# zotya701/OpenCL_Path_tracer

Hardware: AMD Instinct MI355X
Metric: Msamples/s (whole node) at 1920x1080, 8-bounce Cornell box (higher is better)
Workload: dtype f32

## Files before the change

### opencl_path_tracer_amd/csrc/pt_context.hpp

```cpp
#pragma once

#include "pt_internal.hpp"

#include <algorithm>
#include <atomic>
#include <chrono>
#include <cmath>
#include <condition_variable>
#include <functional>
#include <mutex>
#include <cstdio>
#include <cstring>
#include <limits>
#include <memory>
#include <numeric>
#include <queue>
#include <thread>

using namespace ptamd;

namespace ptamd {
struct EventPair {
    hipEvent_t a = nullptr, b = nullptr;
};
}

struct pt_context {
    int device = -1;
    bool has_device = false;
    int32_t W = 0, H = 0;
    int32_t rank = 0, world = 1, rows_per_block = 8;
    int32_t local_rows = 0;
    int64_t npix = 0;
    int64_t slab_pix = 0;

    void* comm = nullptr;
    float4* d_gathered = nullptr;
    float4* d_frame = nullptr;
    uint64_t render_epoch = 0;
    uint64_t frame_epoch = ~0ull;

    std::vector<pt_triangle> tris;
    std::vector<int32_t> obj_begin;
    int32_t tri_shift = 0;
    std::vector<pt_material> mats;
    std::vector<int32_t> enc_rank;
    int32_t next_rank = 0;
    bool tris_uploaded = false, mats_uploaded = false;

    std::vector<Node64> nodes;
    std::vector<Node4q> nodes4;
    int wide_pending = 0;
    std::vector<TriPacket> packets;
    bool host_packets_stale = false;
    std::vector<TriMeta> meta;
    std::vector<int32_t> orig;
    int bvh_depth = 0;
    int interior_depth = 0;
    int n_flat = 0;
    int n_fbox = 0;
    uint8_t fbox_rep[32] = {};
    uint32_t fbox_mask[32] = {};

    float4* d_nodes = nullptr;
    float4* d_nodes4 = nullptr;
    uint32_t* d_stack_ovf = nullptr;
    size_t stack_ovf_lanes = 0;
    float4* d_tris = nullptr;
    TriMeta* d_meta = nullptr;
    pt_material* d_mats = nullptr;
    int32_t* d_rnds = nullptr;
    float4* d_colors = nullptr;
    pt_ray* d_rays = nullptr;
    float4* d_ldr = nullptr;
    unsigned long long* d_stats = nullptr;
    float4* d_wf_state = nullptr;
    int32_t* d_wf_queues = nullptr;
    std::vector<float> cost_boxes;
    uint32_t* d_wf_counters = nullptr;
    hipStream_t wf_stream[kWfMaxChains] = {};
    hipEvent_t wf_event[kWfMaxChains] = {};
    int poll_timeout_ms = 10000;
    int debug_stall_tile = -1;
    bool counters_suspect = false;
    bool launched_since_check = false;
    int wf_streams = -1;
    bool own_rnds = true, own_colors = true;
    hipStream_t stream = nullptr;

    int32_t current_sample = 0;

    int variant = 0;
    int lds_scene = 2;
    int treelet = 0;
    int treelet_nodes = 0;
    int timing = 0;
    int count_work = 0;
    int bvh_on_device = 0;
    double bvh_build_ms = 0.0;
    int cu_count = 256;
    int persistent = 1;
    uint32_t* d_tile_counter = nullptr;
    uint32_t* d_tile_done = nullptr;
    uint32_t* d_tile_cost = nullptr;
    float4* d_adapt_snap = nullptr;
    int32_t* d_adapt_spp = nullptr;
    float* d_adapt_err = nullptr;
    uint8_t* d_adapt_active = nullptr;
    int32_t* d_adapt_list = nullptr;
    int32_t* h_adapt_count = nullptr;
    bool adaptive_frame = false;
    float4* d_aov = nullptr;
    float4* d_dn = nullptr;
    float4* d_denoised = nullptr;
    bool aov_valid = false;
    int moments = 0;
    bool moments_valid = false;
    float* d_variance = nullptr;
    uint64_t frame_serial = 0;
    pt_camera frame_cam = {};
    bool frame_cam_same = false;
    uint64_t aov_serial = 0;
    pt_camera aov_cam = {};
    float4* d_temporal = nullptr;
    float* d_temporal_var = nullptr;
    int temporal_out = -1;
    bool temporal_history = false;
    pt_camera temporal_cam = {};
    uint64_t temporal_frame = ~0ull;
    uint64_t temporal_aov = ~0ull;
    std::vector<int32_t> nee_tri;
    std::vector<float> nee_cdf;
    std::vector<float> nee_pdf_area;
    bool nee_valid = false;
    int32_t* d_nee_tri = nullptr;
    float* d_nee_cdf = nullptr;
    float* d_nee_pdf_area = nullptr;
    bool nee_uploaded = false;
    int chunk_taper = -1;
    int chunk_spp = -1;
    int sah_visit_cost = 10;
    int flat_list = 16;
    int schedule = -1;
    int suspend_lanes = -1;
    int migrate_lanes = -1;
    int node_min_lanes = -1, leaf_min_lanes = -1;
    int lbvh_ploc = 16;
    int lbvh_cluster = 64;
    int build_threads = 0;
    int wide_nodes = 1;
    int wide_lds_entries = kWideLdsEntries;
    int lds_block = -1;
    int waves_per_simd = -1;
    int debug_repeat = 0;
    int cost_binning = 1;
    int bvh_policy = 0;
    int sah_grain = 256;
    int wide_on_device = 1;
    int bvh_device = -1;

    std::vector<EventPair> events;
    size_t events_used = 0;
    double kernel_ms_acc = 0.0;
    int64_t kernel_launches = 0;
    size_t last_lds_bytes = 0;
    int last_waves_per_simd = 4;

    std::string err;
    char info[256] = {0};
};

namespace ptamd {

constexpr size_t kLdsPerCu = 160 * 1024;
constexpr size_t kLdsSlack = 32 * 100 + 4096 + 1024 + 256;

int fail(pt_context* ctx, int code, const std::string& msg);
int host_threads(const pt_context* ctx);

#define PT_HIP(ctx, call)                                                                   \
    do {                                                                                    \
        hipError_t e_ = (call);                                                             \
        if (e_ != hipSuccess)                                                               \
            return fail(ctx, PT_EHIP, std::string(#call) + ": " + hipGetErrorString(e_));   \
    } while (0)

inline void note_frame(pt_context* ctx, int32_t first_sample, const pt_camera* cam) {
    ctx->moments_valid = (first_sample == 0 || ctx->moments_valid) && ctx->moments != 0;
    if (first_sample == 0) {
        ++ctx->frame_serial;
        ctx->frame_cam = *cam;
        ctx->frame_cam_same = true;
    } else if (std::memcmp(cam, &ctx->frame_cam, sizeof(pt_camera)) != 0) {
        ctx->frame_cam_same = false;
    }
}

#define PT_NEED_DEVICE(ctx)                                                                 \
    do {                                                                                    \
        if (!(ctx)) return PT_EINVAL;                                                       \
        if (!(ctx)->has_device)                                                             \
            return fail(ctx, PT_ENODEVICE, "context was created without a HIP device (host-only); no CPU render path exists"); \
    } while (0)
class HostPool {
public:
    static HostPool& get() { static HostPool p; return p; }
    template <class F>
    void run(size_t chunks, int threads, F fn) {
        if (chunks == 0) return;
        if (threads <= 1 || chunks == 1) { for (size_t k = 0; k < chunks; ++k) fn(k); return; }
        std::unique_lock<std::mutex> region(region_mu_, std::try_to_lock);
        if (!region.owns_lock()) {
            std::atomic<size_t> next(0);
            auto work = [&]() { for (size_t k = next.fetch_add(1); k < chunks; k = next.fetch_add(1)) fn(k); };
            std::vector<std::thread> th;
            for (int t = 1; t < std::min<int>(threads, (int)chunks); ++t) th.emplace_back(work);
            work();
            for (std::thread& t : th) t.join();
            return;
        }
        grow(std::min<int>(threads, (int)chunks) - 1);
        std::function<void(size_t)> f = fn;
        {
            std::lock_guard<std::mutex> lk(mu_);
            job_ = &f;
            chunks_ = chunks;
            next_.store(0);
            helpers_wanted_ = std::min<int>(threads, (int)chunks) - 1;
            helpers_in_ = 0;
            helpers_done_ = 0;
            ++generation_;
        }
        cv_.notify_all();
        for (size_t k = next_.fetch_add(1); k < chunks; k = next_.fetch_add(1)) fn(k);
        std::unique_lock<std::mutex> lk(mu_);
        job_ = nullptr;
        done_cv_.wait(lk, [&]() { return helpers_done_ == helpers_in_; });
    }
    ~HostPool() {
        {
            std::lock_guard<std::mutex> lk(mu_);
            stop_ = true;
        }
        cv_.notify_all();
        for (std::thread& t : workers_) t.join();
    }

private:
    void grow(int n) {
        while ((int)workers_.size() < n) workers_.emplace_back([this]() { loop(); });
    }
    void loop() {
        unsigned long long seen = 0;
        for (;;) {
            std::function<void(size_t)>* job = nullptr;
            size_t chunks = 0;
            {
                std::unique_lock<std::mutex> lk(mu_);
                cv_.wait(lk, [&]() { return stop_ || (generation_ != seen && job_ != nullptr && helpers_in_ < helpers_wanted_); });
                if (stop_) return;
                seen = generation_;
                job = job_;
                chunks = chunks_;
                ++helpers_in_;
            }
            for (size_t k = next_.fetch_add(1); k < chunks; k = next_.fetch_add(1)) (*job)(k);
            {
                std::lock_guard<std::mutex> lk(mu_);
                ++helpers_done_;
            }
            done_cv_.notify_all();
        }
    }
    std::mutex region_mu_, mu_;
    std::condition_variable cv_, done_cv_;
    std::vector<std::thread> workers_;
    std::function<void(size_t)>* job_ = nullptr;
    size_t chunks_ = 0;
    std::atomic<size_t> next_{0};
    int helpers_wanted_ = 0, helpers_in_ = 0, helpers_done_ = 0;
    unsigned long long generation_ = 0;
    bool stop_ = false;
};

template <class F>
void parallel_for(size_t n, size_t grain, int threads, F fn) {
    const size_t nt = std::min<size_t>((size_t)std::max(threads, 1), (n + grain - 1) / std::max<size_t>(grain, 1));
    if (nt <= 1) { fn((size_t)0, n); return; }
    const size_t per = (n + nt - 1) / nt;
    HostPool::get().run(nt, (int)nt, [&](size_t k) {
        const size_t b = k * per, e = std::min(n, b + per);
        if (b < e) fn(b, e);
    });
}
int deepest_interior_node(const std::vector<Node64>& nodes);
int reindex_treelet(std::vector<Node64>& nodes, int interior_depth, int want);

int32_t count_local_rows(int32_t H, int32_t rank, int32_t world, int32_t rb);
int wide_stack_entries(int pending);
int stack_entries_for(int interior_depth);
bool whole_tree_fits_lds(size_t n_nodes, size_t n_tris, int interior_depth, int n_flat);
int plan_node_placement(pt_context* ctx, const float4* d_bvh2 = nullptr, bool* wide_on_device = nullptr);
int alloc_stack_overflow(pt_context* ctx);
int seed_upload(pt_context* ctx, const int32_t* global_seeds);
void fill_params(const pt_context* ctx, const pt_camera* cam, RenderParams* p);
int check_ready(pt_context* ctx, const pt_camera* cam);
int time_begin(pt_context* ctx, EventPair** ep);
int time_end(pt_context* ctx, EventPair* ep);
int time_collect(pt_context* ctx);
int sync_and_check(pt_context* ctx);
inline int32_t local_tiles(const pt_context* c) { return ((c->W + 7) / 8) * ((c->local_rows + 7) / 8); }
template <class T>
int upload_vec(pt_context* ctx, T** dptr, const void* src, size_t bytes) {
    if (*dptr) { PT_HIP(ctx, hipFree(*dptr)); *dptr = nullptr; }
    PT_HIP(ctx, hipMalloc((void**)dptr, std::max<size_t>(bytes, 64)));
    if (bytes < 64) PT_HIP(ctx, hipMemset(*dptr, 0, 64));
    if (bytes) PT_HIP(ctx, hipMemcpy(*dptr, src, bytes, hipMemcpyHostToDevice));
    return PT_OK;
}


}
```

### opencl_path_tracer_amd/csrc/pt_host.cpp

```cpp
#include "pt_context.hpp"

namespace {
thread_local std::string g_create_error;
}

namespace ptamd {

int fail(pt_context* ctx, int code, const std::string& msg) {
    if (ctx) ctx->err = msg; else g_create_error = msg;
    return code;
}

int host_threads(const pt_context* ctx) {
    const unsigned hw = std::thread::hardware_concurrency();
    return ctx->build_threads > 0 ? ctx->build_threads : (int)std::min(16u, std::max(1u, hw));
}

int fail_ctx(pt_context* ctx, int code, const std::string& msg) { return fail(ctx, code, msg); }
int append_triangles(pt_context* ctx, int64_t n, pt_triangle** tail) {
    if (!ctx || n < 0 || !tail) return PT_EINVAL;
    if ((int64_t)ctx->tris.size() + n > kMaxTriangles) return fail(ctx, PT_EINVAL, "more than 2^26 triangles");
    const size_t old = ctx->tris.size();
    ctx->tris.resize(old + (size_t)n);
    ctx->tris_uploaded = false;
    *tail = ctx->tris.data() + old;
    return PT_OK;
}
hipError_t launch_deinterleave(const float4* gathered, float4* frame, int W, int H, int world, int rb, long long slab_stride, hipStream_t stream);
void gather_source_index(int W, int H, int world, int rb, long long slab_stride, int64_t* out);
int comm_available(std::string* err);
int comm_unique_id(void* id128, std::string* err);
int comm_init(const void* id128, int rank, int world, void** comm_out, std::string* err);
void comm_destroy(void* comm);
int comm_all_gather(void* comm, const void* send, void* recv, size_t floats_per_rank, hipStream_t stream, std::string* err);

}

extern "C" {

void pt_material_init(pt_material* m, const float kd[3], const float ks[3], const float emission[3],
                      const float N[3], const float K[3], float shininess, int32_t type) {
    std::memset(m, 0, sizeof *m);
    for (int i = 0; i < 3; ++i) { m->kd.s[i] = kd[i]; m->ks.s[i] = ks[i]; m->emission.s[i] = emission[i]; }
    m->shininess = shininess;
    m->type = type;
    m->n = (N[0] + N[1] + N[2]) / 3.0f;
    for (int i = 0; i < 3; ++i) {
        float a = (N[i] - 1) * (N[i] - 1);
        float b = (N[i] + 1) * (N[i] + 1);
        m->F0.s[i] = (K[i] * K[i] + a) / (K[i] * K[i] + b);
    }
}

void pt_triangle_init(pt_triangle* t, const float r1[3], const float r2[3], const float r3[3], uint16_t mati) {
    std::memset(t, 0, sizeof *t);
    float v1[3], v2[3], n[3];
    for (int i = 0; i < 3; ++i) {
        t->r1.s[i] = r1[i]; t->r2.s[i] = r2[i]; t->r3.s[i] = r3[i];
        v1[i] = r2[i] - r1[i];
        v2[i] = r3[i] - r1[i];
    }
    t->mati = mati;
    n[0] = v1[1] * v2[2] - v1[2] * v2[1];
    n[1] = v1[2] * v2[0] - v1[0] * v2[2];
    n[2] = v1[0] * v2[1] - v1[1] * v2[0];
    float length = (float)std::sqrt((double)(n[0] * n[0] + n[1] * n[1] + n[2] * n[2]));
    for (int i = 0; i < 3; ++i) t->N.s[i] = n[i] / length;
}

void pt_triangles_init(pt_triangle* out, const float* verts, const uint16_t* mati, int64_t n) {
    for (int64_t i = 0; i < n; ++i) pt_triangle_init(&out[i], verts + 9 * i, verts + 9 * i + 3, verts + 9 * i + 6, mati[i]);
}

static void rotate_x_ref(float v[3], float gamma) {
    gamma = gamma / 180.0f * 3.141593f;
    const double c = std::cos((double)gamma), s = std::sin((double)gamma);
    const float r1 = (float)((double)v[1] * c - (double)v[2] * s);
    const float r2 = (float)((double)v[1] * s + (double)v[2] * c);
    v[1] = r1;
    v[2] = r2;
}
static void rotate_y_ref(float v[3], float beta) {
    beta = beta / 180.0f * 3.141593f;
    const double c = std::cos((double)beta), s = std::sin((double)beta);
    const float r0 = (float)((double)v[0] * c + (double)v[2] * s);
    const float r2 = (float)(-(double)v[0] * s + (double)v[2] * c);
    v[0] = r0;
    v[2] = r2;
}

void pt_camera_init(pt_camera* c, float fov, float yaw, float pitch, const float shift[3], int32_t width, int32_t height) {
    std::memset(c, 0, sizeof *c);
    c->XM = (float)width;
    c->YM = (float)height;
    const float up_length = c->YM / 2.0f;
    const float right_length = c->XM / 2.0f;
    const float ahead_length = (float)((double)right_length / std::tan((double)(fov / 2.0f / 180.0f * 3.141593f)));
    float up[3] = {0.0f, 1.0f, 0.0f}, right[3] = {1.0f, 0.0f, 0.0f}, ahead[3] = {0.0f, 0.0f, 1.0f};
    rotate_x_ref(up, pitch); rotate_y_ref(up, yaw);
    rotate_x_ref(right, pitch); rotate_y_ref(right, yaw);
    rotate_x_ref(ahead, pitch); rotate_y_ref(ahead, yaw);
    for (int i = 0; i < 3; ++i) { up[i] *= up_length; right[i] *= right_length; ahead[i] *= ahead_length; }
    c->eye.s[0] = 500.0f + shift[0];
    c->eye.s[1] = 500.0f + shift[1];
    c->eye.s[2] = -1299.037842f + shift[2];
    for (int i = 0; i < 3; ++i) { c->up.s[i] = up[i]; c->right.s[i] = right[i]; c->lookat.s[i] = c->eye.s[i] + ahead[i]; }
}

void pt_camera_move(float shift[3], float yaw, float pitch, float forward, float rightward, float upward) {
    float up[3] = {0.0f, 1.0f, 0.0f}, right[3] = {1.0f, 0.0f, 0.0f}, ahead[3] = {0.0f, 0.0f, 1.0f};
    rotate_x_ref(up, pitch); rotate_y_ref(up, yaw);
    rotate_x_ref(right, pitch); rotate_y_ref(right, yaw);
    rotate_x_ref(ahead, pitch); rotate_y_ref(ahead, yaw);
    for (int i = 0; i < 3; ++i) {
        const float a = ahead[i] * forward, r = right[i] * rightward, u = up[i] * upward;
        shift[i] = ((shift[i] + a) + r) + u;
    }
}

int pt_create_tiled(int device, int32_t width, int32_t height, int32_t rank, int32_t world, int32_t rows_per_block, pt_context** out) {
    if (!out) return fail(nullptr, PT_EINVAL, "out is NULL");
    *out = nullptr;
    if (width <= 0 || height <= 0 || (int64_t)width * height > (int64_t)1 << 30) return fail(nullptr, PT_EINVAL, "bad frame size");
    if (width > 65535 || height > 65535) return fail(nullptr, PT_EINVAL, "bad frame size: at most 65,535 pixels per side (the kernels pack a pixel's coordinates into 2 x 16 bits)");
    if (world < 1 || rank < 0 || rank >= world || rows_per_block < 1) return fail(nullptr, PT_EINVAL, "bad rank/world/rows_per_block");
    pt_context* ctx = new pt_context();
    ctx->W = width;
    ctx->H = height;
    ctx->rank = rank;
    ctx->world = world;
    ctx->rows_per_block = rows_per_block;
    ctx->local_rows = count_local_rows(height, rank, world, rows_per_block);
    ctx->npix = (int64_t)ctx->local_rows * width;
    for (int32_t r = 0; r < world; ++r) ctx->slab_pix = std::max(ctx->slab_pix, (int64_t)count_local_rows(height, r, world, rows_per_block) * width);
    ctx->device = device;
    if (device < 0) {
        std::snprintf(ctx->info, sizeof ctx->info, "host-only context (no device)");
        *out = ctx;
        return PT_OK;
    }
    int count = 0;
    hipError_t e = hipGetDeviceCount(&count);
    if (e != hipSuccess || count <= 0 || device >= count) {
        delete ctx;
        return fail(nullptr, PT_ENODEVICE, std::string("no usable HIP device: ") + (e != hipSuccess ? hipGetErrorString(e) : "device index out of range"));
    }
    auto bail = [&](const char* what, hipError_t err) {
        std::string msg = std::string(what) + ": " + hipGetErrorString(err);
        pt_destroy(ctx);
        return fail(nullptr, PT_EHIP, msg);
    };
    if ((e = hipSetDevice(device)) != hipSuccess) return bail("hipSetDevice", e);
    hipDeviceProp_t prop;
    if ((e = hipGetDeviceProperties(&prop, device)) != hipSuccess) return bail("hipGetDeviceProperties", e);
    ctx->cu_count = prop.multiProcessorCount;
    std::snprintf(ctx->info, sizeof ctx->info, "%s (%s), %d CUs, %.1f GiB, wave %d", prop.name, prop.gcnArchName,
                  prop.multiProcessorCount, (double)prop.totalGlobalMem / (1024.0 * 1024.0 * 1024.0), prop.warpSize);
    if (std::strncmp(prop.gcnArchName, "gfx950", 6) != 0) {
        std::string msg = std::string("device is ") + prop.gcnArchName + ", this library carries gfx950 code only";
        pt_destroy(ctx);
        return fail(nullptr, PT_ENODEVICE, msg);
    }
    ctx->has_device = true;
    const size_t np = (size_t)std::max<int64_t>(ctx->npix, 1);
    const size_t nslab = (size_t)std::max<int64_t>(ctx->slab_pix, 1);
    if ((e = hipMalloc((void**)&ctx->d_rays, sizeof(pt_ray) * np)) != hipSuccess) return bail("hipMalloc(rays)", e);
    if ((e = hipMalloc((void**)&ctx->d_rnds, sizeof(int32_t) * np)) != hipSuccess) return bail("hipMalloc(rnds)", e);
    if ((e = hipMalloc((void**)&ctx->d_colors, sizeof(float4) * nslab)) != hipSuccess) return bail("hipMalloc(colors)", e);
    if ((e = hipMalloc((void**)&ctx->d_stats, sizeof(unsigned long long) * kStatCols * kStatRows)) != hipSuccess) return bail("hipMalloc(stats)", e);
    if ((e = hipMalloc((void**)&ctx->d_tile_counter, sizeof(uint32_t) * kTileCounterWords)) != hipSuccess) return bail("hipMalloc(tile counter)", e);
    if ((e = hipMemset(ctx->d_tile_counter, 0, sizeof(uint32_t) * kTileCounterWords)) != hipSuccess) return bail("hipMemset", e);
    if ((e = hipMemset(ctx->d_rays, 0, sizeof(pt_ray) * np)) != hipSuccess) return bail("hipMemset", e);
    if ((e = hipMemset(ctx->d_colors, 0, sizeof(float4) * nslab)) != hipSuccess) return bail("hipMemset", e);
    if ((e = hipMemset(ctx->d_stats, 0, sizeof(unsigned long long) * kStatCols * kStatRows)) != hipSuccess) return bail("hipMemset", e);
    int rc = pt_seed_default(ctx);
    if (rc != PT_OK) {
        std::string msg = ctx->err;
        pt_destroy(ctx);
        return fail(nullptr, rc, msg);
    }
    *out = ctx;
    return PT_OK;
}

int pt_create(int device, int32_t width, int32_t height, pt_context** out) {
    return pt_create_tiled(device, width, height, 0, 1, 8, out);
}

void pt_destroy(pt_context* ctx) {
    if (!ctx) return;
    if (ctx->has_device) {
        (void)hipSetDevice(ctx->device);
        (void)hipDeviceSynchronize();
        for (auto& e : ctx->events) { if (e.a) (void)hipEventDestroy(e.a); if (e.b) (void)hipEventDestroy(e.b); }
        if (ctx->d_nodes) (void)hipFree(ctx->d_nodes);
        if (ctx->d_nodes4) (void)hipFree(ctx->d_nodes4);
        if (ctx->d_stack_ovf) (void)hipFree(ctx->d_stack_ovf);
        if (ctx->d_tris) (void)hipFree(ctx->d_tris);
        if (ctx->d_meta) (void)hipFree(ctx->d_meta);
        if (ctx->d_mats) (void)hipFree(ctx->d_mats);
        if (ctx->d_rays) (void)hipFree(ctx->d_rays);
        if (ctx->d_ldr) (void)hipFree(ctx->d_ldr);
        if (ctx->d_stats) (void)hipFree(ctx->d_stats);
        if (ctx->d_tile_counter) (void)hipFree(ctx->d_tile_counter);
        if (ctx->d_tile_done) (void)hipFree(ctx->d_tile_done);
        if (ctx->d_tile_cost) (void)hipFree(ctx->d_tile_cost);
        if (ctx->d_adapt_snap) (void)hipFree(ctx->d_adapt_snap);
        if (ctx->d_adapt_spp) (void)hipFree(ctx->d_adapt_spp);
        if (ctx->d_adapt_err) (void)hipFree(ctx->d_adapt_err);
        if (ctx->d_adapt_active) (void)hipFree(ctx->d_adapt_active);
        if (ctx->d_adapt_list) (void)hipFree(ctx->d_adapt_list);
        if (ctx->h_adapt_count) (void)hipHostFree(ctx->h_adapt_count);
        if (ctx->d_aov) (void)hipFree(ctx->d_aov);
        if (ctx->d_dn) (void)hipFree(ctx->d_dn);
        if (ctx->d_variance) (void)hipFree(ctx->d_variance);
        if (ctx->d_temporal) (void)hipFree(ctx->d_temporal);
        if (ctx->d_temporal_var) (void)hipFree(ctx->d_temporal_var);
        if (ctx->d_nee_tri) (void)hipFree(ctx->d_nee_tri);
        if (ctx->d_nee_cdf) (void)hipFree(ctx->d_nee_cdf);
        if (ctx->d_nee_pdf_area) (void)hipFree(ctx->d_nee_pdf_area);
        if (ctx->d_wf_state) (void)hipFree(ctx->d_wf_state);
        if (ctx->d_wf_queues) (void)hipFree(ctx->d_wf_queues);
        if (ctx->d_wf_counters) (void)hipFree(ctx->d_wf_counters);
        for (int c = 0; c < kWfMaxChains; ++c) {
            if (ctx->wf_stream[c]) (void)hipStreamDestroy(ctx->wf_stream[c]);
            if (ctx->wf_event[c]) (void)hipEventDestroy(ctx->wf_event[c]);
        }
        if (ctx->comm) comm_destroy(ctx->comm);
        if (ctx->d_gathered) (void)hipFree(ctx->d_gathered);
        if (ctx->d_frame) (void)hipFree(ctx->d_frame);
        if (ctx->own_rnds && ctx->d_rnds) (void)hipFree(ctx->d_rnds);
        if (ctx->own_colors && ctx->d_colors) (void)hipFree(ctx->d_colors);
    }
    delete ctx;
}

const char* pt_last_error(const pt_context* ctx) { return ctx ? ctx->err.c_str() : g_create_error.c_str(); }

int pt_device_info(const pt_context* ctx, char* buf, int32_t buflen) {
    if (!ctx || !buf || buflen <= 0) return PT_EINVAL;
    std::snprintf(buf, (size_t)buflen, "%s", ctx->info);
    return PT_OK;
}

int pt_add_material(pt_context* ctx, const pt_material* m) {
    if (!ctx || !m) return PT_EINVAL;
    if (ctx->mats.size() >= 65536) return fail(ctx, PT_EINVAL, "more than 65536 materials (mati is a ushort, prog.cl:20)");
    ctx->mats.push_back(*m);
    ctx->mats_uploaded = false;
    return (int)ctx->mats.size() - 1;
}

int pt_add_triangle(pt_context* ctx, const pt_triangle* t) { return pt_add_triangles(ctx, t, 1); }

int pt_add_triangles(pt_context* ctx, const pt_triangle* t, int64_t n) {
    if (!ctx || (!t && n) || n < 0) return PT_EINVAL;
    if ((int64_t)ctx->tris.size() + n > kMaxTriangles)
        return fail(ctx, PT_EINVAL, "more than 2^26 triangles");
    ctx->tris.insert(ctx->tris.end(), t, t + n);
    ctx->tris_uploaded = false;
    return PT_OK;
}

int pt_upload_materials(pt_context* ctx) {
    if (!ctx) return PT_EINVAL;
    ctx->aov_valid = false;
    ctx->nee_valid = false;
    for (const pt_triangle& t : ctx->tris)
        if (t.mati >= ctx->mats.size()) return fail(ctx, PT_EINVAL, "a triangle references a material index that was never added");
    if (ctx->has_device) {
        PT_HIP(ctx, hipSetDevice(ctx->device));
        std::vector<pt_material> dm(ctx->mats);
        for (pt_material& m : dm)
            m._pad = (m.ks.s[0] == 0.0f && m.ks.s[1] == 0.0f && m.ks.s[2] == 0.0f && std::isfinite(m.shininess) && m.shininess >= 0.0f) ? 1 : 0;
        int rc = upload_vec(ctx, &ctx->d_mats, dm.data(), sizeof(pt_material) * dm.size());
        if (rc != PT_OK) return rc;
    }
    ctx->mats_uploaded = true;
    return PT_OK;
}

int pt_seed_default(pt_context* ctx) {
    PT_NEED_DEVICE(ctx);
    const size_t n = (size_t)ctx->W * (size_t)ctx->H;
    std::vector<int32_t> g(n);
    uint64_t x = 1;
    for (size_t i = 0; i < n; ++i) {
        x = (x * 16807ull) % 2147483647ull;
        g[i] = (int32_t)x;
    }
    return seed_upload(ctx, g.data());
}

int pt_upload_seeds(pt_context* ctx, const int32_t* seeds, int64_t n) {
    PT_NEED_DEVICE(ctx);
    if (!seeds || n != (int64_t)ctx->W * ctx->H) return fail(ctx, PT_EINVAL, "seeds must hold width*height ints (global frame)");
    return seed_upload(ctx, seeds);
}

int pt_local_pixel_count(const pt_context* ctx, int64_t* out) {
    if (!ctx || !out) return PT_EINVAL;
    *out = ctx->npix;
    return PT_OK;
}

int pt_slab_pixel_count(const pt_context* ctx, int64_t* out) {
    if (!ctx || !out) return PT_EINVAL;
    *out = ctx->slab_pix;
    return PT_OK;
}

int pt_frame_size(const pt_context* ctx, int32_t* width, int32_t* height, int64_t* npix) {
    if (!ctx) return PT_EINVAL;
    if (width) *width = ctx->W;
    if (height) *height = ctx->H;
    if (npix) *npix = (int64_t)ctx->W * ctx->H;
    return PT_OK;
}

int pt_comm_available(void) {
    std::string err;
    const int rc = comm_available(&err);
    return rc == PT_OK ? rc : fail(nullptr, rc, err);
}

int pt_comm_unique_id(void* id128) {
    if (!id128) return PT_EINVAL;
    std::string err;
    const int rc = comm_unique_id(id128, &err);
    return rc == PT_OK ? rc : fail(nullptr, rc, err);
}

int pt_comm_init(pt_context* ctx, const void* id128) {
    PT_NEED_DEVICE(ctx);
    if (!id128) return fail(ctx, PT_EINVAL, "id is NULL");
    if (ctx->comm) return fail(ctx, PT_EINVAL, "the context already has a communicator");
    PT_HIP(ctx, hipSetDevice(ctx->device));
    std::string err;
    const int rc = comm_init(id128, ctx->rank, ctx->world, &ctx->comm, &err);
    return rc == PT_OK ? rc : fail(ctx, rc, err);
}

int pt_gather_frame(pt_context* ctx) {
    PT_NEED_DEVICE(ctx);
    if (!ctx->comm) {
        if (ctx->world == 1) return PT_OK;
        return fail(ctx, PT_EINVAL, "pt_comm_init has not been called on this tiled context");
    }
    PT_HIP(ctx, hipSetDevice(ctx->device));
    const size_t slab = (size_t)ctx->slab_pix;
    if (!ctx->d_gathered) PT_HIP(ctx, hipMalloc((void**)&ctx->d_gathered, sizeof(float4) * slab * (size_t)ctx->world));
    if (!ctx->d_frame) PT_HIP(ctx, hipMalloc((void**)&ctx->d_frame, sizeof(float4) * (size_t)ctx->W * (size_t)ctx->H));
    std::string err;
    const int rc = comm_all_gather(ctx->comm, ctx->d_colors, ctx->d_gathered, slab * 4, ctx->stream, &err);
    if (rc != PT_OK) return fail(ctx, rc, err);
    PT_HIP(ctx, launch_deinterleave(ctx->d_gathered, ctx->d_frame, ctx->W, ctx->H, ctx->world, ctx->rows_per_block, (long long)slab, ctx->stream));
    ctx->frame_epoch = ctx->render_epoch;
    return PT_OK;
}

static const float4* current_frame(const pt_context* ctx) {
    if (ctx->d_frame && ctx->frame_epoch == ctx->render_epoch) return ctx->d_frame;
    return ctx->world == 1 ? ctx->d_colors : nullptr;
}

void* pt_device_frame(pt_context* ctx) { return !ctx ? nullptr : (void*)current_frame(ctx); }

int pt_read_frame(pt_context* ctx, float* out, int64_t npix) {
    PT_NEED_DEVICE(ctx);
    if (!out || npix != (int64_t)ctx->W * ctx->H) return fail(ctx, PT_EINVAL, "npix must equal width * height of the global frame");
    const float4* src = current_frame(ctx);
    if (!src) return fail(ctx, PT_EINVAL, ctx->d_frame ? "the gathered frame is older than colors: call pt_gather_frame again" : "pt_gather_frame has not been called");
    PT_HIP(ctx, hipSetDevice(ctx->device));
    PT_HIP(ctx, hipStreamSynchronize(ctx->stream));
    PT_HIP(ctx, hipMemcpy(out, src, sizeof(float4) * (size_t)npix, hipMemcpyDeviceToHost));
    return PT_OK;
}

int pt_debug_gather_index(int32_t width, int32_t height, int32_t world, int32_t rows_per_block, int64_t slab_stride, int64_t* out) {
    if (width <= 0 || height <= 0 || world < 1 || rows_per_block < 1 || !out) return PT_EINVAL;
    gather_source_index(width, height, world, rows_per_block, (long long)slab_stride, out);
    return PT_OK;
}

int pt_local_pixel_ids(const pt_context* ctx, int32_t* out, int64_t n) {
    if (!ctx || !out || n != ctx->npix) return PT_EINVAL;
    for (int32_t lr = 0; lr < ctx->local_rows; ++lr) {
        const int32_t gr = global_row(*ctx, lr);
        for (int32_t x = 0; x < ctx->W; ++x) out[(size_t)lr * ctx->W + x] = gr * ctx->W + x;
    }
    return PT_OK;
}

static int read_back(pt_context* ctx, void* dst, const void* src, size_t bytes) {
    const int rc = sync_and_check(ctx);
    if (rc != PT_OK) return rc;
    if (bytes) PT_HIP(ctx, hipMemcpy(dst, src, bytes, hipMemcpyDeviceToHost));
    return PT_OK;
}

int pt_read_colors(pt_context* ctx, float* out, int64_t npix) {
    PT_NEED_DEVICE(ctx);
    if (!out || npix != ctx->npix) return fail(ctx, PT_EINVAL, "npix must equal the local pixel count");
    return read_back(ctx, out, ctx->d_colors, sizeof(float4) * (size_t)npix);
}
int pt_read_rnds(pt_context* ctx, int32_t* out, int64_t npix) {
    PT_NEED_DEVICE(ctx);
    if (!out || npix != ctx->npix) return fail(ctx, PT_EINVAL, "npix must equal the local pixel count");
    return read_back(ctx, out, ctx->d_rnds, sizeof(int32_t) * (size_t)npix);
}
int pt_read_sample_counts(pt_context* ctx, int32_t* out, int64_t npix) {
    PT_NEED_DEVICE(ctx);
    if (!out || npix != ctx->npix) return fail(ctx, PT_EINVAL, "npix must equal the local pixel count");
    if (!ctx->adaptive_frame) {
        std::fill(out, out + npix, ctx->current_sample);
        return PT_OK;
    }
    std::vector<int32_t> spp((size_t)local_tiles(ctx));
    const int rc = read_back(ctx, spp.data(), ctx->d_adapt_spp, sizeof(int32_t) * spp.size());
    if (rc != PT_OK) return rc;
    const int32_t tiles_x = (ctx->W + 7) / 8;
    for (int64_t i = 0; i < npix; ++i) {
        const int32_t y = (int32_t)(i / ctx->W), x = (int32_t)(i % ctx->W);
        out[i] = spp[(size_t)(y / 8) * tiles_x + x / 8];
    }
    return PT_OK;
}
int pt_read_tile_state(pt_context* ctx, int32_t* spp, float* err, int64_t n_tiles) {
    PT_NEED_DEVICE(ctx);
    if (n_tiles != local_tiles(ctx)) return fail(ctx, PT_EINVAL, "pt_read_tile_state: n_tiles must be the number of 8x8 tiles of the local frame");
    if (!ctx->adaptive_frame) {
        if (spp) std::fill(spp, spp + n_tiles, ctx->current_sample);
        if (err) std::fill(err, err + n_tiles, std::numeric_limits<float>::infinity());
        return PT_OK;
    }
    int rc = PT_OK;
    if (spp && (rc = read_back(ctx, spp, ctx->d_adapt_spp, sizeof(int32_t) * (size_t)n_tiles)) != PT_OK) return rc;
    if (err && (rc = read_back(ctx, err, ctx->d_adapt_err, sizeof(float) * (size_t)n_tiles)) != PT_OK) return rc;
    return PT_OK;
}
int pt_render_aovs(pt_context* ctx, const pt_camera* cam, int32_t subpixels, int32_t specular_depth) {
    if (!ctx) return PT_EINVAL;
    if (subpixels < 1 || subpixels > 8) return fail(ctx, PT_EINVAL, "pt_render_aovs: subpixels must be 1..8");
    if (specular_depth < 0 || specular_depth > 16) return fail(ctx, PT_EINVAL, "pt_render_aovs: specular_depth must be 0..16");
    PT_NEED_DEVICE(ctx);
    int rc = check_ready(ctx, cam);
    if (rc != PT_OK) return rc;
    PT_HIP(ctx, hipSetDevice(ctx->device));
    if (!ctx->d_aov) PT_HIP(ctx, hipMalloc((void**)&ctx->d_aov, 2 * sizeof(float4) * (size_t)std::max<int64_t>(ctx->npix, 1)));
    RenderParams p;
    fill_params(ctx, cam, &p);
    PT_HIP(ctx, launch_aovs(p, subpixels, specular_depth, ctx->npix, ctx->d_aov, ctx->d_aov + ctx->npix, ctx->cu_count, ctx->stream));
    if (!ctx->aov_valid) ctx->temporal_history = false;
    ctx->aov_valid = true;
    ctx->aov_cam = *cam;
    ++ctx->aov_serial;
    return PT_OK;
}
int pt_read_aovs(pt_context* ctx, float* albedo_rgbm, float* normal_depth, int64_t npix) {
    PT_NEED_DEVICE(ctx);
    if (npix != ctx->npix) return fail(ctx, PT_EINVAL, "npix must equal the local pixel count");
    if (!ctx->d_aov) return fail(ctx, PT_EINVAL, "pt_read_aovs: pt_render_aovs has not run");
    int rc = PT_OK;
    if (albedo_rgbm && (rc = read_back(ctx, albedo_rgbm, ctx->d_aov, sizeof(float4) * (size_t)npix)) != PT_OK) return rc;
    if (normal_depth && (rc = read_back(ctx, normal_depth, ctx->d_aov + npix, sizeof(float4) * (size_t)npix)) != PT_OK) return rc;
    return PT_OK;
}
void pt_denoise_defaults(pt_denoise_params* p) {
    if (!p) return;
    p->iterations = 3;
    p->sigma_color = 0.125f;
    p->sigma_normal = 8.0f;
    p->sigma_depth = 0.05f;
    p->demodulate = 1;
}
int pt_denoise(pt_context* ctx, const pt_denoise_params* dp) {
    if (!ctx) return PT_EINVAL;
    if (!dp) return fail(ctx, PT_EINVAL, "pt_denoise: params is NULL");
    if (dp->iterations < 1 || dp->iterations > 10) return fail(ctx, PT_EINVAL, "pt_denoise: iterations must be 1..10");
    if (!(dp->sigma_color >= 0.0f) || !(dp->sigma_normal >= 0.0f) || !(dp->sigma_depth >= 0.0f))
        return fail(ctx, PT_EINVAL, "pt_denoise: sigmas must be >= 0 (and not NaN)");
    if (ctx->world != 1) return fail(ctx, PT_EINVAL, "pt_denoise: contexts of one rank (world == 1) only");
    if (!ctx->aov_valid)
        return fail(ctx, PT_EINVAL, "pt_denoise: no guides (pt_render_aovs has not run since the scene was last uploaded)");
    PT_NEED_DEVICE(ctx);
    PT_HIP(ctx, hipSetDevice(ctx->device));
    const size_t npix = (size_t)ctx->npix;
    if (!ctx->d_dn) PT_HIP(ctx, hipMalloc((void**)&ctx->d_dn, 2 * sizeof(float4) * std::max<size_t>(npix, 1)));
    for (int i = 0; i < dp->iterations; ++i) {
        AtrousStep s;
        s.step = 1 << i;
        s.demodulate = dp->demodulate ? 1 : 0;
        s.color_on = std::isfinite(dp->sigma_color) ? 1 : 0;
        s.normal_on = std::isfinite(dp->sigma_normal) && dp->sigma_normal > 0.0f ? 1 : 0;
        s.depth_on = std::isfinite(dp->sigma_depth) ? 1 : 0;
        s.color_scale = (float)(1 << (2 * i));
        s.sigma_color2 = dp->sigma_color * dp->sigma_color;
        s.sigma_normal = dp->sigma_normal;
        s.sigma_depth = dp->sigma_depth;
        const float4* in = i == 0 ? ctx->d_colors : ctx->d_dn + ((i - 1) & 1) * npix;
        float4* out = ctx->d_dn + (i & 1) * npix;
        PT_HIP(ctx, launch_atrous(in, out, ctx->d_aov, ctx->d_aov + npix, ctx->W, ctx->local_rows, s, i == 0, i == dp->iterations - 1, ctx->stream));
    }
    ctx->d_denoised = ctx->d_dn + ((dp->iterations - 1) & 1) * npix;
    return PT_OK;
}
int pt_read_denoised(pt_context* ctx, float* out, int64_t npix) {
    PT_NEED_DEVICE(ctx);
    if (!out || npix != ctx->npix) return fail(ctx, PT_EINVAL, "npix must equal the local pixel count");
    if (!ctx->d_denoised) return fail(ctx, PT_EINVAL, "pt_read_denoised: pt_denoise has not run");
    return read_back(ctx, out, ctx->d_denoised, sizeof(float4) * (size_t)npix);
}
void* pt_device_denoised(pt_context* ctx) { return ctx ? (void*)ctx->d_denoised : nullptr; }

static int compute_variance(pt_context* ctx, const char* who) {
    if (!ctx->moments_valid) return fail(ctx, PT_EINVAL, std::string(who) + ": the frame was not rendered with option moments = 1 from its first sample");
    if (ctx->current_sample <= 0) return fail(ctx, PT_EINVAL, std::string(who) + ": the frame has no samples");
    PT_HIP(ctx, hipSetDevice(ctx->device));
    if (!ctx->d_variance) PT_HIP(ctx, hipMalloc((void**)&ctx->d_variance, sizeof(float) * (size_t)std::max<int64_t>(ctx->npix, 1)));
    PT_HIP(ctx, launch_variance(ctx->d_colors, ctx->adaptive_frame ? ctx->d_adapt_spp : nullptr, ctx->current_sample, ctx->W, ctx->npix,
                                ctx->d_variance, ctx->stream));
    return PT_OK;
}
int pt_read_variance(pt_context* ctx, float* out, int64_t npix) {
    PT_NEED_DEVICE(ctx);
    if (!out || npix != ctx->npix) return fail(ctx, PT_EINVAL, "npix must equal the local pixel count");
    const int rc = compute_variance(ctx, "pt_read_variance");
    if (rc != PT_OK) return rc;
    return read_back(ctx, out, ctx->d_variance, sizeof(float) * (size_t)npix);
}
void* pt_device_variance(pt_context* ctx) {
    if (!ctx || !ctx->has_device) {
        if (ctx) (void)fail(ctx, PT_ENODEVICE, "context was created without a HIP device (host-only); no CPU render path exists");
        return nullptr;
    }
    return compute_variance(ctx, "pt_device_variance") == PT_OK ? (void*)ctx->d_variance : nullptr;
}

void pt_denoise_variance_defaults(pt_denoise_variance_params* p) {
    if (!p) return;
    p->iterations = 2;
    p->sigma_luminance = 4.0f;
    p->sigma_normal = 8.0f;
    p->sigma_depth = 0.05f;
    p->demodulate = 0;
}
static std::string variance_params_error(const pt_denoise_variance_params* dp) {
    if (!dp) return "params is NULL";
    if (dp->iterations < 1 || dp->iterations > 10) return "iterations must be 1..10";
    if (!(dp->sigma_luminance >= 0.0f) || !(dp->sigma_normal >= 0.0f) || !(dp->sigma_depth >= 0.0f)) return "sigmas must be >= 0 (and not NaN)";
    return "";
}
static int atrous_var_iterations(pt_context* ctx, const pt_denoise_variance_params* dp, const float4* in0, const float* var) {
    const size_t npix = (size_t)ctx->npix;
    if (!ctx->d_dn) PT_HIP(ctx, hipMalloc((void**)&ctx->d_dn, 2 * sizeof(float4) * std::max<size_t>(npix, 1)));
    for (int i = 0; i < dp->iterations; ++i) {
        AtrousVarStep s;
        s.step = 1 << i;
        s.demodulate = dp->demodulate ? 1 : 0;
        s.lum_on = std::isfinite(dp->sigma_luminance) ? 1 : 0;
        s.normal_on = std::isfinite(dp->sigma_normal) && dp->sigma_normal > 0.0f ? 1 : 0;
        s.depth_on = std::isfinite(dp->sigma_depth) ? 1 : 0;
        s.sigma_luminance = dp->sigma_luminance;
        s.sigma_normal = dp->sigma_normal;
        s.sigma_depth = dp->sigma_depth;
        const float4* in = i == 0 ? in0 : ctx->d_dn + ((i - 1) & 1) * npix;
        float4* out = ctx->d_dn + (i & 1) * npix;
        PT_HIP(ctx, launch_atrous_var(in, var, out, ctx->d_aov, ctx->d_aov + npix, ctx->W, ctx->local_rows, s, i == 0,
                                      i == dp->iterations - 1, ctx->stream));
    }
    ctx->d_denoised = ctx->d_dn + ((dp->iterations - 1) & 1) * npix;
    return PT_OK;
}
int pt_denoise_variance(pt_context* ctx, const pt_denoise_variance_params* dp) {
    if (!ctx) return PT_EINVAL;
    const std::string why = variance_params_error(dp);
    if (!why.empty()) return fail(ctx, PT_EINVAL, "pt_denoise_variance: " + why);
    if (ctx->world != 1) return fail(ctx, PT_EINVAL, "pt_denoise_variance: contexts of one rank (world == 1) only");
    if (!ctx->aov_valid)
        return fail(ctx, PT_EINVAL, "pt_denoise_variance: no guides (pt_render_aovs has not run since the scene was last uploaded)");
    PT_NEED_DEVICE(ctx);
    const int rc = compute_variance(ctx, "pt_denoise_variance");
    if (rc != PT_OK) return rc;
    return atrous_var_iterations(ctx, dp, ctx->d_colors, ctx->d_variance);
}

void pt_temporal_defaults(pt_temporal_params* p) {
    if (!p) return;
    p->max_history = 64;
    p->normal_cos = 0.9f;
    p->depth_tolerance = 0.02f;
}
static float4* temporal_colour(const pt_context* ctx, int s) { return ctx->d_temporal + (size_t)s * (size_t)std::max<int64_t>(ctx->npix, 1); }
static float4* temporal_guides(const pt_context* ctx, int s) { return ctx->d_temporal + (size_t)(2 + s) * (size_t)std::max<int64_t>(ctx->npix, 1); }
static float2* temporal_nm(const pt_context* ctx, int s) {
    const size_t np = (size_t)std::max<int64_t>(ctx->npix, 1);
    return reinterpret_cast<float2*>(ctx->d_temporal + 4 * np) + (size_t)s * np;
}
int pt_temporal_accumulate(pt_context* ctx, const pt_temporal_params* tp) {
    if (!ctx) return PT_EINVAL;
    if (!tp) return fail(ctx, PT_EINVAL, "pt_temporal_accumulate: params is NULL");
    if (tp->max_history < 0) return fail(ctx, PT_EINVAL, "pt_temporal_accumulate: max_history must be >= 0");
    if (!(tp->normal_cos >= -1.0f && tp->normal_cos <= 1.0f)) return fail(ctx, PT_EINVAL, "pt_temporal_accumulate: normal_cos must be in [-1, 1]");
    if (!(tp->depth_tolerance >= 0.0f)) return fail(ctx, PT_EINVAL, "pt_temporal_accumulate: depth_tolerance must be >= 0 (and not NaN)");
    if (ctx->world != 1) return fail(ctx, PT_EINVAL, "pt_temporal_accumulate: contexts of one rank (world == 1) only");
    PT_NEED_DEVICE(ctx);
    if (!ctx->aov_valid)
        return fail(ctx, PT_EINVAL, "pt_temporal_accumulate: no guides (pt_render_aovs has not run since the scene was last uploaded)");
    if (!ctx->moments_valid)
        return fail(ctx, PT_EINVAL, "pt_temporal_accumulate: the frame was not rendered with option moments = 1 from its first sample");
    if (ctx->current_sample <= 0) return fail(ctx, PT_EINVAL, "pt_temporal_accumulate: the frame has no samples");
    if (!ctx->frame_cam_same) return fail(ctx, PT_EINVAL, "pt_temporal_accumulate: the launches of the frame used different cameras");
    if (std::memcmp(&ctx->aov_cam, &ctx->frame_cam, sizeof(pt_camera)) != 0)
        return fail(ctx, PT_EINVAL, "pt_temporal_accumulate: the guides were rendered with a different camera from the frame");
    if (ctx->temporal_frame == ctx->frame_serial) return fail(ctx, PT_EINVAL, "pt_temporal_accumulate: this frame was already accumulated");
    PT_HIP(ctx, hipSetDevice(ctx->device));
    const size_t np = (size_t)std::max<int64_t>(ctx->npix, 1);
    if (!ctx->d_temporal) {
        PT_HIP(ctx, hipMalloc((void**)&ctx->d_temporal, (4 * sizeof(float4) + 2 * sizeof(float2)) * np));
        PT_HIP(ctx, hipMalloc((void**)&ctx->d_temporal_var, sizeof(float) * np));
    }
    const int out = ctx->temporal_out == 0 ? 1 : 0, prev = 1 - out;
    TemporalArgs a;
    a.cur = ctx->frame_cam;
    a.prev = ctx->temporal_cam;
    a.colors = ctx->d_colors;
    a.tile_spp = ctx->adaptive_frame ? ctx->d_adapt_spp : nullptr;
    a.n_all = ctx->current_sample;
    a.albedo = ctx->d_aov;
    a.nd = ctx->d_aov + ctx->npix;
    a.prev_c = temporal_colour(ctx, prev);
    a.prev_g = temporal_guides(ctx, prev);
    a.prev_nm = temporal_nm(ctx, prev);
    a.out_c = temporal_colour(ctx, out);
    a.out_g = temporal_guides(ctx, out);
    a.out_nm = temporal_nm(ctx, out);
    a.out_v = ctx->d_temporal_var;
    a.W = ctx->W;
    a.H = ctx->local_rows;
    a.has_prev = ctx->temporal_history ? 1 : 0;
    a.max_history = (float)tp->max_history;
    a.normal_cos = tp->normal_cos;
    a.depth_tolerance = tp->depth_tolerance;
    PT_HIP(ctx, launch_temporal(a, ctx->stream));
    ctx->temporal_out = out;
    ctx->temporal_history = true;
    ctx->temporal_cam = ctx->frame_cam;
    ctx->temporal_frame = ctx->frame_serial;
    ctx->temporal_aov = ctx->aov_serial;
    return PT_OK;
}
int pt_read_temporal(pt_context* ctx, float* rgbv, float* n, int64_t npix) {
    PT_NEED_DEVICE(ctx);
    if (npix != ctx->npix) return fail(ctx, PT_EINVAL, "npix must equal the local pixel count");
    if (ctx->temporal_out < 0) return fail(ctx, PT_EINVAL, "pt_read_temporal: pt_temporal_accumulate has not run");
    int rc = PT_OK;
    if (rgbv) {
        std::vector<float> v((size_t)npix);
        if ((rc = read_back(ctx, rgbv, temporal_colour(ctx, ctx->temporal_out), sizeof(float4) * (size_t)npix)) != PT_OK) return rc;
        if ((rc = read_back(ctx, v.data(), ctx->d_temporal_var, sizeof(float) * (size_t)npix)) != PT_OK) return rc;
        for (int64_t i = 0; i < npix; ++i) rgbv[4 * i + 3] = v[(size_t)i];
    }
    if (n) {
        std::vector<float2> nm((size_t)npix);
        if ((rc = read_back(ctx, nm.data(), temporal_nm(ctx, ctx->temporal_out), sizeof(float2) * (size_t)npix)) != PT_OK) return rc;
        for (int64_t i = 0; i < npix; ++i) n[i] = nm[(size_t)i].x;
    }
    return PT_OK;
}
void* pt_device_temporal(pt_context* ctx) { return ctx && ctx->temporal_out >= 0 ? (void*)temporal_colour(ctx, ctx->temporal_out) : nullptr; }
int pt_denoise_temporal(pt_context* ctx, const pt_denoise_variance_params* dp) {
    if (!ctx) return PT_EINVAL;
    const std::string why = variance_params_error(dp);
    if (!why.empty()) return fail(ctx, PT_EINVAL, "pt_denoise_temporal: " + why);
    if (ctx->world != 1) return fail(ctx, PT_EINVAL, "pt_denoise_temporal: contexts of one rank (world == 1) only");
    PT_NEED_DEVICE(ctx);
    if (!ctx->aov_valid || ctx->temporal_out < 0 || ctx->temporal_aov != ctx->aov_serial)
        return fail(ctx, PT_EINVAL, "pt_denoise_temporal: pt_temporal_accumulate has not run on the current guides");
    PT_HIP(ctx, hipSetDevice(ctx->device));
    return atrous_var_iterations(ctx, dp, temporal_colour(ctx, ctx->temporal_out), ctx->d_temporal_var);
}
int pt_debug_reproject(const pt_camera* cur, const pt_camera* prev, int32_t x, int32_t y, float depth, float out[3]) {
    if (!cur || !prev || !out) return fail(nullptr, PT_EINVAL, "pt_debug_reproject: NULL argument");
    if (!(cur->XM >= 1.0f && cur->XM <= 65535.0f && cur->YM >= 1.0f && cur->YM <= 65535.0f) || x < 0 || y < 0 || x >= (int32_t)cur->XM || y >= (int32_t)cur->YM)
        return fail(nullptr, PT_EINVAL, "pt_debug_reproject: (x, y) must lie in cur's frame");
    if (!reproject(*cur, *prev, y * (int32_t)cur->XM + x, depth, out))
        return fail(nullptr, PT_EINVAL, "pt_debug_reproject: the point is not in front of prev (a <= 0)");
    return PT_OK;
}

uint32_t pt_nee_rand(uint32_t state, int32_t segment, int32_t dim) { return nee_rand(state, segment, dim); }
static int nee_table(pt_context* ctx) {
    if (!ctx->tris_uploaded) return fail(ctx, PT_EINVAL, "pt_upload_triangles has not been called");
    if (!ctx->mats_uploaded) return fail(ctx, PT_EINVAL, "pt_upload_materials has not been called");
    if (ctx->nee_valid) return PT_OK;
    const size_t m = ctx->orig.size();
    std::vector<double> wgt, area;
    ctx->nee_tri.clear();
    ctx->nee_cdf.clear();
    ctx->nee_pdf_area.assign(std::max<size_t>(m, 1), 0.0f);
    for (size_t k = 0; k < m; ++k) {
        const pt_triangle& t = ctx->tris[(size_t)ctx->orig[k]];
        const pt_material& mt = ctx->mats[t.mati];
        if (mt.type != 3) continue;
        const double esum = ((double)mt.emission.s[0] + (double)mt.emission.s[1]) + (double)mt.emission.s[2];
        const double e1[3] = {(double)t.r2.s[0] - t.r1.s[0], (double)t.r2.s[1] - t.r1.s[1], (double)t.r2.s[2] - t.r1.s[2]};
        const double e2[3] = {(double)t.r3.s[0] - t.r1.s[0], (double)t.r3.s[1] - t.r1.s[1], (double)t.r3.s[2] - t.r1.s[2]};
        const double cx = e1[1] * e2[2] - e1[2] * e2[1], cy = e1[2] * e2[0] - e1[0] * e2[2], cz = e1[0] * e2[1] - e1[1] * e2[0];
        const double a = 0.5 * std::sqrt(cx * cx + cy * cy + cz * cz);
        if (!(esum > 0.0) || !(a > 0.0) || !std::isfinite(a * esum)) continue;
        ctx->nee_tri.push_back((int32_t)k);
        wgt.push_back(a * esum);
        area.push_back(a);
    }
    double total = 0.0;
    for (double w : wgt) total += w;
    double run = 0.0;
    for (size_t j = 0; j < wgt.size(); ++j) {
        run += wgt[j];
        ctx->nee_cdf.push_back(j + 1 == wgt.size() ? 1.0f : (float)(run / total));
    }
    double below = 0.0;
    for (size_t j = 0; j < wgt.size(); ++j) {
        const double upto = std::ceil((double)ctx->nee_cdf[j] * 16777216.0);
        ctx->nee_pdf_area[(size_t)ctx->nee_tri[j]] = (float)((upto - below) / 16777216.0 / area[j]);
        below = upto;
    }
    ctx->nee_valid = true;
    ctx->nee_uploaded = false;
    return PT_OK;
}
int pt_debug_light_table(pt_context* ctx, int32_t* orig_tri, float* cdf, int64_t cap, int64_t* n) {
    if (!ctx) return PT_EINVAL;
    if (!n || cap < 0) return fail(ctx, PT_EINVAL, "pt_debug_light_table: n is NULL or cap < 0");
    int rc = nee_table(ctx);
    if (rc != PT_OK) return rc;
    *n = (int64_t)ctx->nee_tri.size();
    const size_t k = (size_t)std::min<int64_t>(cap, *n);
    for (size_t j = 0; j < k; ++j) {
        if (orig_tri) orig_tri[j] = ctx->orig[(size_t)ctx->nee_tri[j]];
        if (cdf) cdf[j] = ctx->nee_cdf[j];
    }
    return PT_OK;
}
int pt_render_nee(pt_context* ctx, const pt_camera* cam, int32_t iterations, int32_t nsamples, int32_t strategy) {
    if (!ctx) return PT_EINVAL;
    if (iterations < 0 || nsamples < 0) return fail(ctx, PT_EINVAL, "pt_render_nee: iterations/nsamples must be >= 0");
    if (strategy < PT_NEE_BSDF || strategy > PT_NEE_MIS) return fail(ctx, PT_EINVAL, "pt_render_nee: strategy must be PT_NEE_BSDF, PT_NEE_LIGHT or PT_NEE_MIS");
    PT_NEED_DEVICE(ctx);
    int rc = check_ready(ctx, cam);
    if (rc != PT_OK) return rc;
    if (ctx->adaptive_frame) return fail(ctx, PT_EINVAL, "pt_render_nee: an adaptive frame is held: pt_set_current_sample(ctx, 0) starts a new frame");
    if ((int64_t)ctx->current_sample + nsamples > INT32_MAX) return fail(ctx, PT_EINVAL, "pt_render_nee: current_sample + nsamples overflows");
    if (nsamples == 0) return PT_OK;
    if ((rc = nee_table(ctx)) != PT_OK) return rc;
    PT_HIP(ctx, hipSetDevice(ctx->device));
    if (!ctx->nee_uploaded) {
        if (ctx->d_nee_tri) PT_HIP(ctx, hipFree(ctx->d_nee_tri));
        if (ctx->d_nee_cdf) PT_HIP(ctx, hipFree(ctx->d_nee_cdf));
        if (ctx->d_nee_pdf_area) PT_HIP(ctx, hipFree(ctx->d_nee_pdf_area));
        ctx->d_nee_tri = nullptr;
        ctx->d_nee_cdf = nullptr;
        ctx->d_nee_pdf_area = nullptr;
        const size_t nl = std::max<size_t>(ctx->nee_tri.size(), 1);
        PT_HIP(ctx, hipMalloc((void**)&ctx->d_nee_tri, sizeof(int32_t) * nl));
        PT_HIP(ctx, hipMalloc((void**)&ctx->d_nee_cdf, sizeof(float) * nl));
        PT_HIP(ctx, hipMalloc((void**)&ctx->d_nee_pdf_area, sizeof(float) * ctx->nee_pdf_area.size()));
        if (!ctx->nee_tri.empty()) {
            PT_HIP(ctx, hipMemcpy(ctx->d_nee_tri, ctx->nee_tri.data(), sizeof(int32_t) * ctx->nee_tri.size(), hipMemcpyHostToDevice));
            PT_HIP(ctx, hipMemcpy(ctx->d_nee_cdf, ctx->nee_cdf.data(), sizeof(float) * ctx->nee_cdf.size(), hipMemcpyHostToDevice));
        }
        PT_HIP(ctx, hipMemcpy(ctx->d_nee_pdf_area, ctx->nee_pdf_area.data(), sizeof(float) * ctx->nee_pdf_area.size(), hipMemcpyHostToDevice));
        ctx->nee_uploaded = true;
    }
    RenderParams p;
    fill_params(ctx, cam, &p);
    p.iterations = iterations;
    p.first_sample = ctx->current_sample;
    p.nsamples = nsamples;
    NeeTable lt;
    lt.tri = ctx->d_nee_tri;
    lt.cdf = ctx->d_nee_cdf;
    lt.pdf_area = ctx->d_nee_pdf_area;
    lt.n = (int32_t)ctx->nee_tri.size();
    lt.strategy = strategy;
    ctx->render_epoch++;
    note_frame(ctx, p.first_sample, cam);
    EventPair* ep;
    if ((rc = time_begin(ctx, &ep)) != PT_OK) return rc;
    PT_HIP(ctx, launch_nee(p, lt, ctx->npix, ctx->cu_count, ctx->stream));
    if ((rc = time_end(ctx, ep)) != PT_OK) return rc;
    ctx->current_sample += nsamples;
    return PT_OK;
}

int pt_read_rays(pt_context* ctx, pt_ray* out, int64_t npix) {
    PT_NEED_DEVICE(ctx);
    if (!out || npix != ctx->npix) return fail(ctx, PT_EINVAL, "npix must equal the local pixel count");
    return read_back(ctx, out, ctx->d_rays, sizeof(pt_ray) * (size_t)npix);
}

int pt_resolve_ldr(pt_context* ctx, int32_t which, float* out, int64_t npix) {
    PT_NEED_DEVICE(ctx);
    if (!out || npix != ctx->npix) return fail(ctx, PT_EINVAL, "npix must equal the local pixel count");
    if (which != 0 && which != 1) return fail(ctx, PT_EINVAL, "which must be 0 (Reinhard) or 1 (filt_im)");
    if (which == 1 && ctx->world != 1) return fail(ctx, PT_EINVAL, "filt_im needs the whole frame on one context (3x3 stencil)");
    PT_HIP(ctx, hipSetDevice(ctx->device));
    if (!ctx->d_ldr) PT_HIP(ctx, hipMalloc((void**)&ctx->d_ldr, sizeof(float4) * (size_t)std::max<int64_t>(npix, 1)));
    if (which == 0) {
        PT_HIP(ctx, launch_resolve_reinhard(ctx->d_colors, ctx->d_ldr, npix, ctx->stream));
    } else {
        PT_HIP(ctx, hipMemsetAsync(ctx->d_ldr, 0, sizeof(float4) * (size_t)npix, ctx->stream));
        PT_HIP(ctx, launch_filt_im(ctx->d_colors, ctx->d_ldr, ctx->W, ctx->H, ctx->stream));
    }
    return read_back(ctx, out, ctx->d_ldr, sizeof(float4) * (size_t)npix);
}

int pt_bind_framebuffer(pt_context* ctx, void* d_colors, void* d_rnds) {
    PT_NEED_DEVICE(ctx);
    PT_HIP(ctx, hipSetDevice(ctx->device));
    PT_HIP(ctx, hipStreamSynchronize(ctx->stream));
    if (d_colors && d_colors != ctx->d_colors) {
        PT_HIP(ctx, hipMemcpy(d_colors, ctx->d_colors, sizeof(float4) * (size_t)ctx->npix, hipMemcpyDeviceToDevice));
        if (ctx->own_colors) PT_HIP(ctx, hipFree(ctx->d_colors));
        ctx->d_colors = (float4*)d_colors;
        ctx->own_colors = false;
    }
    if (d_rnds && d_rnds != ctx->d_rnds) {
        PT_HIP(ctx, hipMemcpy(d_rnds, ctx->d_rnds, sizeof(int32_t) * (size_t)ctx->npix, hipMemcpyDeviceToDevice));
        if (ctx->own_rnds) PT_HIP(ctx, hipFree(ctx->d_rnds));
        ctx->d_rnds = (int32_t*)d_rnds;
        ctx->own_rnds = false;
    }
    return PT_OK;
}

void* pt_device_colors(pt_context* ctx) { return ctx ? (void*)ctx->d_colors : nullptr; }
void* pt_device_rnds(pt_context* ctx) { return ctx ? (void*)ctx->d_rnds : nullptr; }

int pt_set_stream(pt_context* ctx, void* s) {
    PT_NEED_DEVICE(ctx);
    PT_HIP(ctx, hipSetDevice(ctx->device));
    PT_HIP(ctx, hipStreamSynchronize(ctx->stream));
    ctx->stream = (hipStream_t)s;
    return PT_OK;
}

int pt_set_option(pt_context* ctx, const char* key, int64_t value) {
    if (!ctx || !key) return PT_EINVAL;
    std::string k(key);
    if (k == "variant") {
        if (value != 0 && value != 1) return fail(ctx, PT_EINVAL, "variant must be 0 (megakernel) or 1 (wavefront)");
        ctx->variant = (int)value;
    } else if (k == "lds_scene") {
        if (value != 0 && value != 2) return fail(ctx, PT_EINVAL, "lds_scene: 0 every node through L1/L2, 2 stage the tree (or its top) in LDS");
        ctx->lds_scene = (int)value;
    } else if (k == "treelet") {
        if (value < -1 || value > 2048) return fail(ctx, PT_EINVAL, "treelet: 0 off, -1 as many nodes as fit, 2..2048 nodes");
        ctx->treelet = (int)value;
        ctx->tris_uploaded = false;
    } else if (k == "lbvh_cluster") {
        if (value < 0 || value > (1 << 20)) return fail(ctx, PT_EINVAL, "lbvh_cluster: 0 off, 1..2^20 triangles");
        ctx->lbvh_cluster = (int)value;
        ctx->tris_uploaded = false;
    } else if (k == "build_threads") {
        if (value < 0 || value > 256) return fail(ctx, PT_EINVAL, "build_threads: 0 automatic, 1..256");
        ctx->build_threads = (int)value;
    } else if (k == "wide_nodes") {
        if (value < 0 || value > 2) return fail(ctx, PT_EINVAL, "wide_nodes: 0 never, 1 for trees that do not fit LDS, 2 always");
        ctx->wide_nodes = (int)value;
        ctx->tris_uploaded = false;
    } else if (k == "wide_lds_entries") {
        if (value < 4 || value > kWideLdsEntries || (value & 1)) return fail(ctx, PT_EINVAL, "wide_lds_entries: even, 4..20");
        ctx->wide_lds_entries = (int)value;
        ctx->tris_uploaded = false;
    } else if (k == "moments") {
        if (value != 0 && value != 1) return fail(ctx, PT_EINVAL, "moments must be 0 (off) or 1 (second moment of the luminance in colors[].w)");
        ctx->moments = (int)value;
    } else if (k == "timing") {
        ctx->timing = value ? 1 : 0;
    } else if (k == "count_work") {
        ctx->count_work = value ? 1 : 0;
    } else if (k == "chunk_taper") {
        if (value < -1 || value > 1 << 15) return fail(ctx, PT_EINVAL, "chunk_taper: -1 default, 0 off, else the shortest pass");
        ctx->chunk_taper = (int)value;
    } else if (k == "chunk_spp") {
        if (value < -1 || value > 1 << 20) return fail(ctx, PT_EINVAL, "chunk_spp out of range");
        ctx->chunk_spp = (int)value;
    } else if (k == "persistent") {
        ctx->persistent = value ? 1 : 0;
    } else if (k == "sah_visit_cost") {
        if (value < 0 || value > 1000) return fail(ctx, PT_EINVAL, "sah_visit_cost: tenths of a triangle test, 0..1000");
        ctx->sah_visit_cost = (int)value;
    } else if (k == "schedule") {
        if (value < -1 || value > 2) return fail(ctx, PT_EINVAL, "schedule: -1 automatic, 0 lockstep per sample, 1 restart + tail suspension, 2 the same with lanes moving on to the wave's next work item");
        ctx->schedule = (int)value;
    } else if (k == "flat_list") {
        if (value < 0 || value > 32) return fail(ctx, PT_EINVAL, "flat_list: 0..32 big triangles tested before the tree (a 32-bit candidate mask per lane)");
        ctx->flat_list = (int)value;
        ctx->tris_uploaded = false;
    } else if (k == "poll_timeout_ms") {
        if (value < 1 || value > 40000) return fail(ctx, PT_EINVAL, "poll_timeout_ms: 1..40000");
        ctx->poll_timeout_ms = (int)value;
    } else if (k == "debug_stall_tile") {
        if (value < -1 || value > 0x7fffffff) return fail(ctx, PT_EINVAL, "debug_stall_tile: -1 none, or a tile index");
        ctx->debug_stall_tile = (int)value;
    } else if (k == "wf_streams") {
        if (value < -1 || value == 0 || value > kWfMaxChains) return fail(ctx, PT_EINVAL, "wf_streams: -1 default, 1..8");
        ctx->wf_streams = (int)value;
    } else if (k == "node_min_lanes" || k == "leaf_min_lanes") {
        if (value < -1 || value > 63) return fail(ctx, PT_EINVAL, k + ": -1 default, 0..63");
        (k == "node_min_lanes" ? ctx->node_min_lanes : ctx->leaf_min_lanes) = (int)value;
    } else if (k == "migrate_lanes") {
        if (value != -1 && (value < 1 || value > 64)) return fail(ctx, PT_EINVAL, "migrate_lanes: -1 default, 1..64");
        ctx->migrate_lanes = (int)value;
    } else if (k == "suspend_lanes") {
        if (value < -1 || value > 63) return fail(ctx, PT_EINVAL, "suspend_lanes: -1 default, 0..63");
        ctx->suspend_lanes = (int)value;
    } else if (k == "waves_per_simd") {
        if (value != -1 && (value < 4 || value > 8)) return fail(ctx, PT_EINVAL, "waves_per_simd: -1 automatic (at most 7), 4..8 (kernels that read nodes from global memory)");
        ctx->waves_per_simd = (int)value;
    } else if (k == "bvh_device") {
        if (value < -1 || value > 1) return fail(ctx, PT_EINVAL, "bvh_device: -1 (by scene size), 0 (host) or 1 (device)");
        ctx->bvh_device = (int)value;
    } else if (k == "wide_on_device") {
        if (value != 0 && value != 1) return fail(ctx, PT_EINVAL, "wide_on_device: 0 or 1");
        ctx->wide_on_device = (int)value;
    } else if (k == "sah_grain") {
        if (value < 8 || value > (1 << 16)) return fail(ctx, PT_EINVAL, "sah_grain: 8..65536 triangles");
        ctx->sah_grain = (int)value;
    } else if (k == "lbvh_ploc") {
        if (value != 0 && value != 8 && value != 16 && value != 32) return fail(ctx, PT_EINVAL, "lbvh_ploc: 0 (radix tree), 8, 16 or 32 (PLOC search radius)");
        ctx->lbvh_ploc = (int)value;
    } else if (k == "lds_block") {
        if (value != -1 && value != kLdsBlockBase && value != kLdsBlockWide) return fail(ctx, PT_EINVAL, "lds_block: -1 automatic, 512 or 768");
        ctx->lds_block = (int)value;
    } else if (k == "debug_repeat") {
        if (value < 0 || value > 1000) return fail(ctx, PT_EINVAL, "debug_repeat: 0..1000 extra timed launches");
        ctx->debug_repeat = (int)value;
    } else if (k == "cost_binning") {
        ctx->cost_binning = value ? 1 : 0;
    } else if (k == "bvh_policy") {
        if (value < 0 || value > 5) return fail(ctx, PT_EINVAL, "bvh_policy must be 0..5 (4 = device LBVH, 5 = the SAH tree built on the device)");
        ctx->bvh_policy = (int)value;
        ctx->tris_uploaded = false;
    } else if (k == "reset_stats") {
        if (ctx->has_device) {
            PT_HIP(ctx, hipSetDevice(ctx->device));
            PT_HIP(ctx, hipStreamSynchronize(ctx->stream));
            PT_HIP(ctx, hipMemset(ctx->d_stats, 0, sizeof(unsigned long long) * kStatCols * kStatRows));
        }
        int rc = time_collect(ctx);
        if (rc != PT_OK) return rc;
        ctx->kernel_ms_acc = 0.0;
        ctx->kernel_launches = 0;
    } else {
        return fail(ctx, PT_EINVAL, "unknown option: " + k);
    }
    return PT_OK;
}

int pt_get_stat(pt_context* ctx, const char* key, double* out) {
    if (!ctx || !key || !out) return PT_EINVAL;
    std::string k(key);
    if (k == "bvh_nodes") { *out = (double)ctx->nodes.size(); return PT_OK; }
    if (k == "bvh_depth") { *out = (double)ctx->bvh_depth; return PT_OK; }
    if (k == "stack_entries") { *out = (double)stack_entries_for(ctx->interior_depth); return PT_OK; }
    if (k == "bvh_build_ms") { *out = ctx->bvh_build_ms; return PT_OK; }
    if (k == "bvh_on_device") { *out = (double)ctx->bvh_on_device; return PT_OK; }
    if (k == "triangles") { *out = (double)ctx->orig.size(); return PT_OK; }
    if (k == "lds_bytes") { *out = (double)ctx->last_lds_bytes; return PT_OK; }
    if (k == "waves_per_simd") { *out = (double)ctx->last_waves_per_simd; return PT_OK; }
    if (k == "treelet_nodes") { *out = (double)ctx->treelet_nodes; return PT_OK; }
    if (k == "wide_nodes") { *out = (double)ctx->nodes4.size(); return PT_OK; }
    if (k == "wide_pending") { *out = (double)ctx->wide_pending; return PT_OK; }
    if (k == "flat_triangles") { *out = (double)ctx->n_flat; return PT_OK; }
    if (k == "flat_boxes") { *out = (double)ctx->n_fbox; return PT_OK; }
    if (k == "node_mode") {
        pt_camera cam;
        std::memset(&cam, 0, sizeof cam);
        RenderParams p;
        fill_params(ctx, &cam, &p);
        *out = (double)p.node_mode;
        return PT_OK;
    }
    if (k == "kernel_launches") { *out = (double)ctx->kernel_launches; return PT_OK; }
    PT_NEED_DEVICE(ctx);
    PT_HIP(ctx, hipSetDevice(ctx->device));
    if (k == "kernel_ms") {
        int rc = time_collect(ctx);
        if (rc != PT_OK) return rc;
        *out = ctx->kernel_ms_acc;
        return PT_OK;
    }
    if (k == "segments" || k == "samples" || k == "node_visits" || k == "tri_tests" || k == "wave_node_steps" || k == "wave_tri_steps" || k == "tile_lane_steps" ||
        k == "wave_shade_steps" || k == "wave_trips" || k == "wave_rounds" || k.rfind("low_", 0) == 0) {
        std::vector<unsigned long long> rows((size_t)kStatCols * kStatRows);
        unsigned long long h[kStatCols] = {};
        PT_HIP(ctx, hipStreamSynchronize(ctx->stream));
        PT_HIP(ctx, hipMemcpy(rows.data(), ctx->d_stats, sizeof(unsigned long long) * rows.size(), hipMemcpyDeviceToHost));
        for (int r = 0; r < kStatRows; ++r)
            for (int c = 0; c < kStatCols; ++c) h[c] += rows[(size_t)r * kStatCols + c];
        if (k.rfind("low_", 0) == 0 || k == "exact_steps") {
            const int slot = k == "low_node" ? 10 : k == "low_tri" ? 11 : k == "low_exact" ? 12 : k == "low_shade" ? 13 : k == "low_exact_all" ? 15 : -1;
            if (slot < 0) return fail(ctx, PT_EINVAL, "unknown stat " + k);
            *out = (double)h[slot];
            return PT_OK;
        }
        *out = (double)h[k == "segments" ? 0 : k == "samples" ? 1 : k == "node_visits" ? 2 : k == "tri_tests" ? 3 : k == "wave_node_steps" ? 4 : k == "wave_tri_steps" ? 5 : k == "tile_lane_steps" ? 6 : k == "wave_shade_steps" ? 7 : k == "wave_trips" ? 8 : 9];
        return PT_OK;
    }
    return fail(ctx, PT_EINVAL, "unknown stat: " + k);
}

int pt_debug_bvh_sizes(const pt_context* ctx, int64_t* nnodes, int64_t* ntris) {
    if (!ctx) return PT_EINVAL;
    if (nnodes) *nnodes = (int64_t)ctx->nodes.size();
    if (ntris) *ntris = (int64_t)ctx->orig.size();
    return PT_OK;
}

int pt_debug_wide_nodes(const pt_context* ctx, void* out, int64_t capacity, int64_t* count) {
    if (!ctx || !count || capacity < 0) return PT_EINVAL;
    *count = (int64_t)ctx->nodes4.size();
    if (out) std::memcpy(out, ctx->nodes4.data(), sizeof(Node4q) * (size_t)std::min<int64_t>(capacity, *count));
    return PT_OK;
}

int pt_debug_bvh_copy(const pt_context* cctx, float* nodes, float* tris, int32_t* meta, int32_t* orig) {
    if (!cctx || !cctx->tris_uploaded) return PT_EINVAL;
    pt_context* ctx = const_cast<pt_context*>(cctx);
    if (ctx->host_packets_stale && (tris || meta)) {
        const size_t m = ctx->orig.size();
        ctx->packets.resize(m);
        ctx->meta.resize(m);
        PT_HIP(ctx, hipSetDevice(ctx->device));
        PT_HIP(ctx, hipMemcpy(ctx->packets.data(), ctx->d_tris, sizeof(TriPacket) * m, hipMemcpyDeviceToHost));
        PT_HIP(ctx, hipMemcpy(ctx->meta.data(), ctx->d_meta, sizeof(TriMeta) * m, hipMemcpyDeviceToHost));
        ctx->host_packets_stale = false;
    }
    if (nodes) std::memcpy(nodes, ctx->nodes.data(), sizeof(Node64) * ctx->nodes.size());
    if (tris) std::memcpy(tris, ctx->packets.data(), sizeof(TriPacket) * ctx->orig.size());
    if (meta) std::memcpy(meta, ctx->meta.data(), sizeof(TriMeta) * ctx->orig.size());
    if (orig) std::memcpy(orig, ctx->orig.data(), sizeof(int32_t) * ctx->orig.size());
    return PT_OK;
}

namespace {
struct DeviceBuf {
    void* p = nullptr;
    ~DeviceBuf() { if (p) (void)hipFree(p); }
    hipError_t alloc(size_t bytes) { return hipMalloc(&p, std::max<size_t>(bytes, 16)); }
};
struct EventOwner {
    hipEvent_t e = nullptr;
    ~EventOwner() { if (e) (void)hipEventDestroy(e); }
};
}

int pt_debug_math(pt_context* ctx, int32_t fn, int64_t first, int64_t n, int64_t out[3], uint32_t* bad, int64_t bad_cap) {
    PT_NEED_DEVICE(ctx);
    if (fn < PT_MATH_SQRT || fn > PT_MATH_DIV_NORMAL || first < 0 || n < 0 || !out || bad_cap < 0 || (bad_cap > 0 && !bad))
        return fail(ctx, PT_EINVAL, "pt_debug_math: bad arguments");
    PT_HIP(ctx, hipSetDevice(ctx->device));
    DeviceBuf d_out, d_bad;
    PT_HIP(ctx, d_out.alloc(3 * sizeof(unsigned long long)));
    PT_HIP(ctx, d_bad.alloc(2 * sizeof(uint32_t) * (size_t)std::max<int64_t>(bad_cap, 1)));
    PT_HIP(ctx, hipMemsetAsync(d_out.p, 0, 3 * sizeof(unsigned long long), ctx->stream));
    PT_HIP(ctx, launch_debug_math(fn, (unsigned long long)first, (unsigned long long)n, (unsigned long long*)d_out.p, (uint32_t*)d_bad.p, (long long)bad_cap,
                                  ctx->cu_count, ctx->stream));
    PT_HIP(ctx, hipStreamSynchronize(ctx->stream));
    unsigned long long h[3];
    PT_HIP(ctx, hipMemcpy(h, d_out.p, sizeof h, hipMemcpyDeviceToHost));
    for (int i = 0; i < 3; ++i) out[i] = (int64_t)h[i];
    const int64_t k = std::min<int64_t>(out[2], bad_cap);
    if (k > 0) PT_HIP(ctx, hipMemcpy(bad, d_bad.p, 2 * sizeof(uint32_t) * (size_t)k, hipMemcpyDeviceToHost));
    return PT_OK;
}

int pt_debug_closest_hit(pt_context* ctx, const pt_ray* rays, int64_t n, float* out_t, int32_t* out_tri) {
    PT_NEED_DEVICE(ctx);
    if (!rays || !out_t || !out_tri || n < 0) return fail(ctx, PT_EINVAL, "bad arguments");
    if (!ctx->tris_uploaded) return fail(ctx, PT_EINVAL, "pt_upload_triangles has not been called");
    PT_HIP(ctx, hipSetDevice(ctx->device));
    pt_camera cam;
    std::memset(&cam, 0, sizeof cam);
    RenderParams p;
    fill_params(ctx, &cam, &p);
    DeviceBuf d_rays, d_t, d_tri;
    PT_HIP(ctx, d_rays.alloc(sizeof(pt_ray) * (size_t)n));
    PT_HIP(ctx, d_t.alloc(sizeof(float) * (size_t)n));
    PT_HIP(ctx, d_tri.alloc(sizeof(int32_t) * (size_t)n));
    if (n) PT_HIP(ctx, hipMemcpy(d_rays.p, rays, sizeof(pt_ray) * (size_t)n, hipMemcpyHostToDevice));
    ctx->last_lds_bytes = traversal_lds_bytes(p, traversal_block(p.node_mode, false));
    PT_HIP(ctx, launch_debug_closest_hit(p, (const pt_ray*)d_rays.p, n, (float*)d_t.p, (int32_t*)d_tri.p, ctx->cu_count, ctx->stream));
    PT_HIP(ctx, hipStreamSynchronize(ctx->stream));
    if (ctx->debug_repeat > 0) {
        EventOwner e0, e1;
        PT_HIP(ctx, hipEventCreate(&e0.e));
        PT_HIP(ctx, hipEventCreate(&e1.e));
        PT_HIP(ctx, hipEventRecord(e0.e, ctx->stream));
        for (int r = 0; r < ctx->debug_repeat; ++r)
            PT_HIP(ctx, launch_debug_closest_hit(p, (const pt_ray*)d_rays.p, n, (float*)d_t.p, (int32_t*)d_tri.p, ctx->cu_count, ctx->stream));
        PT_HIP(ctx, hipEventRecord(e1.e, ctx->stream));
        PT_HIP(ctx, hipEventSynchronize(e1.e));
        float ms = 0.f;
        PT_HIP(ctx, hipEventElapsedTime(&ms, e0.e, e1.e));
        ctx->kernel_ms_acc += ms;
        ctx->kernel_launches += ctx->debug_repeat;
    }
    if (n) {
        PT_HIP(ctx, hipMemcpy(out_t, d_t.p, sizeof(float) * (size_t)n, hipMemcpyDeviceToHost));
        PT_HIP(ctx, hipMemcpy(out_tri, d_tri.p, sizeof(int32_t) * (size_t)n, hipMemcpyDeviceToHost));
    }
    for (int64_t i = 0; i < n; ++i)
        if (out_tri[i] >= 0) out_tri[i] = ctx->orig[(size_t)out_tri[i]];
    return PT_OK;
}

int pt_debug_deinterleave(pt_context* ctx, const float* gathered, int64_t n_pixels, float* out_frame) {
    PT_NEED_DEVICE(ctx);
    if (!gathered || !out_frame || n_pixels != ctx->slab_pix * ctx->world) return fail(ctx, PT_EINVAL, "gathered must hold world x slab pixels");
    PT_HIP(ctx, hipSetDevice(ctx->device));
    DeviceBuf d_g, d_f;
    const size_t nf = (size_t)ctx->W * (size_t)ctx->H;
    PT_HIP(ctx, d_g.alloc(sizeof(float4) * (size_t)n_pixels));
    PT_HIP(ctx, d_f.alloc(sizeof(float4) * nf));
    PT_HIP(ctx, hipMemcpy(d_g.p, gathered, sizeof(float4) * (size_t)n_pixels, hipMemcpyHostToDevice));
    PT_HIP(ctx, launch_deinterleave((const float4*)d_g.p, (float4*)d_f.p, ctx->W, ctx->H, ctx->world, ctx->rows_per_block, (long long)ctx->slab_pix, ctx->stream));
    PT_HIP(ctx, hipStreamSynchronize(ctx->stream));
    PT_HIP(ctx, hipMemcpy(out_frame, d_f.p, sizeof(float4) * nf, hipMemcpyDeviceToHost));
    return PT_OK;
}

int pt_debug_scene_sizes(const pt_context* ctx, int64_t* ntris, int64_t* nmats, int64_t* nobjs) {
    if (!ctx) return PT_EINVAL;
    if (ntris) *ntris = (int64_t)ctx->tris.size();
    if (nmats) *nmats = (int64_t)ctx->mats.size();
    if (nobjs) *nobjs = (int64_t)ctx->obj_begin.size();
    return PT_OK;
}

int pt_debug_scene_copy(const pt_context* ctx, pt_triangle* tris, pt_material* mats, int32_t* obj_begin) {
    if (!ctx) return PT_EINVAL;
    if (tris && !ctx->tris.empty()) std::memcpy(tris, ctx->tris.data(), sizeof(pt_triangle) * ctx->tris.size());
    if (mats && !ctx->mats.empty()) std::memcpy(mats, ctx->mats.data(), sizeof(pt_material) * ctx->mats.size());
    if (obj_begin && !ctx->obj_begin.empty()) std::memcpy(obj_begin, ctx->obj_begin.data(), sizeof(int32_t) * ctx->obj_begin.size());
    return PT_OK;
}

int pt_debug_tile_cost(pt_context* ctx, uint32_t* out, int64_t n) {
    PT_NEED_DEVICE(ctx);
    const int64_t n_tiles = (int64_t)((ctx->W + 7) / 8) * ((ctx->local_rows + 7) / 8);
    if (!out || n != n_tiles) return fail(ctx, PT_EINVAL, "pt_debug_tile_cost: n must be the number of 8x8 tiles of the local frame");
    if (!ctx->d_tile_cost) return fail(ctx, PT_EINVAL, "pt_debug_tile_cost: no counting launch yet (option count_work, then pt_render)");
    PT_HIP(ctx, hipSetDevice(ctx->device));
    PT_HIP(ctx, hipStreamSynchronize(ctx->stream));
    PT_HIP(ctx, hipMemcpy(out, ctx->d_tile_cost, sizeof(uint32_t) * (size_t)n, hipMemcpyDeviceToHost));
    return PT_OK;
}

int pt_debug_encounter_rank(const pt_context* ctx, int32_t* out, int64_t n) {
    if (!ctx || !out || n != (int64_t)ctx->enc_rank.size()) return PT_EINVAL;
    std::memcpy(out, ctx->enc_rank.data(), sizeof(int32_t) * (size_t)n);
    return PT_OK;
}

}
```

### opencl_path_tracer_amd/csrc/pt_internal.hpp

```cpp
#pragma once

#include <hip/hip_runtime.h>

#include <atomic>
#include <chrono>
#include <cstdint>
#include <cstdio>
#include <cstdlib>
#include <string>
#include <vector>

#include "pt_api.h"

namespace ptamd {

struct Node64 {
    float q[3][4];
    int32_t left, right;
    int32_t pad[2];
};
static_assert(sizeof(Node64) == 64, "Node64 must be 64 B");

struct TriPacket {
    float v[12];
};
static_assert(sizeof(TriPacket) == 48, "TriPacket must be 48 B");

struct TriMeta {
    int32_t rank;
    int32_t mati;
};

struct Node4q {
    float origin[3];
    uint8_t exp[3];
    uint8_t nchild;
    uint32_t qlo_x, qhi_x, qlo_y, qhi_y;
    uint32_t qlo_z, qhi_z;
    uint32_t spare[2];
    int32_t ref[4];
};
static_assert(sizeof(Node4q) == 64, "Node4q must be 64 B");
constexpr int32_t kWideNoChild = ~0;
constexpr int kWideLdsEntries = 20;
bool build_wide_nodes(const std::vector<Node64>& bvh2, std::vector<Node4q>* out, int* max_pending, int threads);

enum : int { kNodesLds = 0, kNodesGlobal = 1, kNodesTreelet = 2, kNodesWide = 3 };

constexpr int64_t kMaxTriangles = (int64_t)1 << 26;

constexpr int64_t kDeviceBuildFrom = 16384;
constexpr int kMaxLeaf = 4;
constexpr int kMaxDepth = 30;
constexpr int kTileCounterError = 16;
constexpr int kMaxTaperPasses = 30;
constexpr int kTileCounterWords = 32;
constexpr int kStatRows = 256;
constexpr int kStatCols = 16;
#ifndef PT_LEAN_FROM_WPS
#define PT_LEAN_FROM_WPS 6
#endif
constexpr int kLeanFromWps = PT_LEAN_FROM_WPS;
constexpr int kLdsBlockWide = 768, kLdsWpsWide = 6;
constexpr int kLdsBlockBase = 512, kLdsWpsBase = 4;
#ifndef PT_LDS_NODE_BYTES
#define PT_LDS_NODE_BYTES 56
#endif
constexpr int kLdsNodeBytes = PT_LDS_NODE_BYTES;
constexpr int kStackEntries = 36;

struct RenderParams {
    const float4* nodes;
    const float4* tris;
    const TriMeta* meta;
    const pt_material* mats;
    int32_t* rnds;
    float4* colors;
    pt_ray* rays;
    unsigned long long* stats;
    pt_camera cam;
    int32_t width, height;
    int32_t local_rows;
    int32_t rank, world, rows_per_block;
    int32_t iterations, first_sample, nsamples;
    int32_t n_nodes, n_tris;
    int32_t n_flat;
    int32_t n_fbox;
    uint8_t fbox_rep[32];
    uint32_t fbox_mask[32];
    int32_t node_mode;
    int32_t treelet_nodes;
    int32_t stack_entries;
    uint32_t* stack_ovf;
    int32_t stack_ovf_lanes;
    uint32_t* tile_counter;
    uint32_t poll_ticks;
    int32_t debug_stall_tile;
    int32_t n_tiles;
    int32_t n_taper;
    uint16_t taper_end[kMaxTaperPasses];
    int32_t chunk_spp;
    uint32_t* tile_done;
    int32_t suspend_lanes;
    int32_t node_min_lanes;
    int32_t leaf_min_lanes;
    int32_t migrate_lanes;
    uint32_t* tile_cost;
    const int32_t* tile_list;
    int32_t moments;
};

template <class P>
__host__ __device__ __forceinline__ int global_row(const P& p, int lrow) {
    return ((lrow / p.rows_per_block) * p.world + p.rank) * p.rows_per_block + lrow % p.rows_per_block;
}

constexpr int kWfCounterStride = 8;
constexpr int kWfMaxBounces = 1023;
constexpr int kWfGenRow = 0;
__host__ __device__ inline int wf_row(int bounce) { return bounce == 0 ? kWfGenRow : bounce + 1; }
constexpr int kWfMaxCostBoxes = 8;
constexpr int kWfMaxChains = 8;
constexpr int kWfDefaultChains = 4;
enum : int { kWfL = 0, kWfB = 1, kWfS = 2, kWfR = 3, kWfC = 4, kWfFields = 5, kWfInsideBit = 1 << 5, kWfBZeroBit = 1 << 6 };
struct WfParams {
    RenderParams rp;
    float* sP;
    float4* rsA[2][2];
    float4* rsB[2][2];
    float4* rsC[2][2];
    float2* hit[2];
    int32_t* q_cls[3];
    uint32_t* counters;
    float cbox[kWfMaxCostBoxes][6];
    int32_t n_cbox;
    int32_t npix;
    int32_t pix0;
    int32_t npix_all;
    int32_t sample;
};

struct LbvhResult {
    float4* d_nodes = nullptr;
    int n_nodes = 0;
    float4* d_tris = nullptr;
    TriMeta* d_meta = nullptr;
    int32_t* d_orig = nullptr;
    int depth = 0;
};
struct DeviceStage {
    char* base = nullptr;
    pt_triangle* d_tris = nullptr;
    int32_t* d_rank = nullptr;
    int32_t* d_sel = nullptr;
    float* d_area = nullptr;
    int* d_misc = nullptr;
    int n = 0;
};
hipError_t stage_upload(const pt_triangle* h_tris, const int32_t* h_rank, int n, hipStream_t stream, DeviceStage* st, float* h_area, int* nonfinite);
hipError_t stage_rest_box(const DeviceStage& st, const int32_t* h_top, int cand, hipStream_t stream, float box[6]);
hipError_t stage_select(const DeviceStage& st, const int32_t* h_flat, int nf, hipStream_t stream);
void stage_free(DeviceStage* st);
hipError_t lbvh_build(const pt_triangle* d_tris, const int32_t* d_rank, int n_all, const int32_t* d_sel, int n, int ploc_radius, hipStream_t stream, LbvhResult* out);
hipError_t sah_device_build(const pt_triangle* d_tris, const int32_t* d_rank, int n_all, const int32_t* d_sel, int n, int max_leaf, bool force_leaf, float visit_cost, int grain,
                            hipStream_t stream, LbvhResult* out, bool* unsupported);

hipError_t wide_device_build(const float4* d_bvh2, int n_nodes, hipStream_t stream, float4** d_out, int* n_out, int* max_pending, bool* failed);

struct LaunchConfig {
    int block = 256;
    size_t lds_bytes = 0;
    int persistent_blocks = 1 << 30;
    int cu_count = 0;
    bool count_work = false;
    int schedule = 0;
    int waves_per_simd = 4;
};

constexpr int kMaxDevicesPerProcess = 16;
struct LdsMark {
    std::atomic<size_t> bytes[kMaxDevicesPerProcess];
};
inline hipError_t ensure_dynamic_lds(const void* kern, LdsMark& mark, size_t lds_bytes) {
    if (lds_bytes <= 64 * 1024) return hipSuccess;
    int dev = 0;
    hipError_t e = hipGetDevice(&dev);
    if (e != hipSuccess) return e;
    if (dev < 0 || dev >= kMaxDevicesPerProcess) return hipFuncSetAttribute(kern, hipFuncAttributeMaxDynamicSharedMemorySize, (int)lds_bytes);
    if (mark.bytes[dev].load(std::memory_order_acquire) >= lds_bytes) return hipSuccess;
    e = hipFuncSetAttribute(kern, hipFuncAttributeMaxDynamicSharedMemorySize, (int)lds_bytes);
    if (e != hipSuccess) return e;
    size_t seen = mark.bytes[dev].load(std::memory_order_relaxed);
    while (seen < lds_bytes && !mark.bytes[dev].compare_exchange_weak(seen, lds_bytes, std::memory_order_release)) {}
    return hipSuccess;
}

struct OccMark {
    std::atomic<long long> key[kMaxDevicesPerProcess];
};
inline int resident_blocks_per_cu(const void* kern, OccMark& mark, int block, size_t lds_bytes) {
    int dev = 0;
    if (hipGetDevice(&dev) != hipSuccess || dev < 0 || dev >= kMaxDevicesPerProcess) return 0;
    const long long seen = mark.key[dev].load(std::memory_order_acquire);
    if (seen != 0 && (size_t)(seen >> 8) == lds_bytes) return (int)(seen & 0xff);
    int n = 0;
    if (hipOccupancyMaxActiveBlocksPerMultiprocessor(&n, kern, block, lds_bytes) != hipSuccess || n <= 0) return 0;
    mark.key[dev].store(((long long)lds_bytes << 8) | (long long)std::min(n, 255), std::memory_order_release);
    return n;
}

struct PhaseClock {
    const char* who;
    const bool on = std::getenv("PTAMD_TRACE") != nullptr;
    std::chrono::steady_clock::time_point t0 = std::chrono::steady_clock::now();
    explicit PhaseClock(const char* w) : who(w) {}
    void lap(const char* what) {
        if (!on) return;
        const auto t1 = std::chrono::steady_clock::now();
        std::fprintf(stderr, "[%s] %-32s %8.1f ms\n", who, what, std::chrono::duration<double, std::milli>(t1 - t0).count());
        t0 = t1;
    }
};

int traversal_block(int node_mode, bool wide_lds_block);
size_t traversal_lds_bytes(const RenderParams& p, int block);
hipError_t launch_gen_ray(const RenderParams& p, hipStream_t stream);
hipError_t launch_trace_ray(const RenderParams& p, const LaunchConfig& lc, hipStream_t stream);
hipError_t launch_render_mega(const RenderParams& p, const LaunchConfig& lc, hipStream_t stream);
hipError_t launch_resolve_reinhard(const float4* colors, float4* out, int64_t n, hipStream_t stream);
hipError_t launch_filt_im(const float4* colors, float4* out, int32_t width, int32_t height, hipStream_t stream);
hipError_t launch_wf_generate(const WfParams& p, hipStream_t stream);
hipError_t launch_wf_intersect(const WfParams& p, int bounce, int cu_count, hipStream_t stream);
hipError_t launch_wf_shade(const WfParams& p, int bounce, hipStream_t stream);
hipError_t launch_adaptive_tiles(const float4* colors, float4* snap, const int32_t* list, int32_t n_list, int32_t width, int32_t rows, int mode,
                                 float threshold, int32_t spp, float* tile_err, int32_t* tile_spp, uint8_t* active, hipStream_t stream);
hipError_t launch_compact_tiles(const uint8_t* active, int32_t n, int32_t* list, int32_t* count, hipStream_t stream);
hipError_t launch_debug_closest_hit(const RenderParams& p, const pt_ray* rays, int64_t n, float* out_t, int32_t* out_tri, int cu_count, hipStream_t stream);
hipError_t launch_debug_math(int fn, unsigned long long first, unsigned long long n, unsigned long long* out, uint32_t* bad, long long bad_cap, int cu_count,
                             hipStream_t stream);
hipError_t launch_aovs(const RenderParams& p, int32_t subpixels, int32_t specular_depth, int64_t npix, float4* albedo_rgbm, float4* normal_depth,
                       int cu_count, hipStream_t stream);
struct AtrousStep {
    int32_t step;
    int32_t demodulate;
    int32_t color_on, normal_on, depth_on;
    float color_scale;
    float sigma_color2, sigma_normal, sigma_depth;
};
hipError_t launch_atrous(const float4* in, float4* out, const float4* albedo, const float4* nd, int32_t W, int32_t H, const AtrousStep& s,
                         bool first, bool last, hipStream_t stream);
struct AtrousVarStep {
    int32_t step;
    int32_t demodulate;
    int32_t lum_on, normal_on, depth_on;
    float sigma_luminance, sigma_normal, sigma_depth;
};
hipError_t launch_atrous_var(const float4* in, const float* var, float4* out, const float4* albedo, const float4* nd, int32_t W, int32_t H,
                             const AtrousVarStep& s, bool first, bool last, hipStream_t stream);
hipError_t launch_variance(const float4* colors, const int32_t* tile_spp, int32_t n_all, int32_t W, int64_t npix, float* out, hipStream_t stream);
struct NeeTable {
    const int32_t* tri;
    const float* cdf;
    const float* pdf_area;
    int32_t n;
    int32_t strategy;
};
hipError_t launch_nee(const RenderParams& p, const NeeTable& lt, int64_t npix, int cu_count, hipStream_t stream);
__host__ __device__ __forceinline__ uint32_t lowbias32(uint32_t x) {
    x ^= x >> 16;
    x *= 0x7feb352du;
    x ^= x >> 15;
    x *= 0x846ca68bu;
    x ^= x >> 16;
    return x;
}
__host__ __device__ __forceinline__ uint32_t nee_rand(uint32_t state, int segment, int dim) {
    return lowbias32(lowbias32(state) + 0x9e3779b9u * (uint32_t)(3 * segment + dim + 1));
}

struct TemporalArgs {
    pt_camera cur, prev;
    const float4* colors;
    const int32_t* tile_spp;
    int32_t n_all;
    const float4* albedo;
    const float4* nd;
    const float4* prev_c;
    const float4* prev_g;
    const float2* prev_nm;
    float4* out_c;
    float4* out_g;
    float2* out_nm;
    float* out_v;
    int32_t W, H;
    int32_t has_prev;
    float max_history, normal_cos, depth_tolerance;
};
hipError_t launch_temporal(const TemporalArgs& a, hipStream_t stream);
__host__ __device__ __forceinline__ float rp_dot(const float* a, const float* b) { return __builtin_fmaf(a[2], b[2], __builtin_fmaf(a[1], b[1], a[0] * b[0])); }
__host__ __device__ __forceinline__ void rp_cross(const float* a, const float* b, float* r) {
    r[0] = __builtin_fmaf(a[1], b[2], -(a[2] * b[1]));
    r[1] = __builtin_fmaf(a[2], b[0], -(a[0] * b[2]));
    r[2] = __builtin_fmaf(a[0], b[1], -(a[1] * b[0]));
}
__host__ __device__ inline bool reproject(const pt_camera& cur, const pt_camera& prev, int gid, float depth, float out[3]) {
    const int X = (int)cur.XM, Y = (int)cur.YM;
    const float sx = (2.0f * ((float)(gid % X) + 0.5f)) / (float)X - 1.0f;
    const float sy = (2.0f * ((float)(gid / X) + 0.5f)) / (float)Y - 1.0f;
    float d[3], v[3], ahead[3];
    for (int i = 0; i < 3; ++i) d[i] = ((cur.lookat.s[i] + cur.right.s[i] * sx) + cur.up.s[i] * sy) - cur.eye.s[i];
    const float inv = 1.0f / __builtin_sqrtf(rp_dot(d, d));
    for (int i = 0; i < 3; ++i) {
        v[i] = __builtin_fmaf(depth, d[i] * inv, cur.eye.s[i]) - prev.eye.s[i];
        ahead[i] = prev.lookat.s[i] - prev.eye.s[i];
    }
    float ru[3], vu[3], rv[3];
    rp_cross(prev.right.s, prev.up.s, ru);
    rp_cross(v, prev.up.s, vu);
    rp_cross(prev.right.s, v, rv);
    const float det = rp_dot(ahead, ru);
    const float a = rp_dot(v, ru) / det;
    if (!(a > 0.0f && a < __builtin_inff())) return false;
    const float u = (rp_dot(ahead, vu) / det) / a, w = (rp_dot(ahead, rv) / det) / a;
    out[0] = ((u + 1.0f) * prev.XM) * 0.5f - 0.5f;
    out[1] = ((w + 1.0f) * prev.YM) * 0.5f - 0.5f;
    out[2] = __builtin_sqrtf(rp_dot(v, v));
    return true;
}

}
```

### opencl_path_tracer_amd/csrc/pt_kernels.hip

```cpp
#include "pt_device.hpp"


#include <algorithm>

namespace ptamd {

__global__ void __launch_bounds__(256) k_gen_ray(RenderParams p) {
    const PixelId px = pixel_of_thread(p);
    if (px.li < 0) return;
    int seed = p.rnds[px.li];
    const float rnd1 = lcg_rand(seed), rnd2 = lcg_rand(seed);
    f3 P, D;
    camera_get_ray(px.gid, p.cam, rnd1, rnd2, &P, &D);
    p.rnds[px.li] = seed;
    float4* r = reinterpret_cast<float4*>(&p.rays[px.li]);
    r[0] = make_float4(P.x, P.y, P.z, 0.0f);
    r[1] = make_float4(D.x, D.y, D.z, 0.0f);
}

enum : int { kSchedLockstep = 0, kSchedSuspend = 1, kSchedMigrate = 2 };


PT_DEV void fold_sample(const RenderParams& p, int li, f3 color, int s) {
    f3 acc = mk(0.0f, 0.0f, 0.0f);
    float m2 = 0.0f;
    if (s != 0) {
        const float4 c = p.colors[li];
        acc = mk(c.x, c.y, c.z);
        m2 = c.w;
    }
    acc = running_mean(acc, color, s);
    m2 = p.moments ? running_moment(m2, color, s) : 0.0f;
    p.colors[li] = make_float4(acc.x, acc.y, acc.z, m2);
}

template <bool SPLIT, int MODE, bool COUNT, bool LEAN, bool SK>
PT_DEV void render_pixel_lockstep(const RenderParams& p, const SceneView& sv, const LaneStack<typename StackOf<MODE>::type> stk, const PixelId px,
                                  int s_begin, int s_end, unsigned* segs, WorkCount* wc) {
    int seed = p.rnds[px.li];
    f3 acc = mk(0.0f, 0.0f, 0.0f);
    float m2 = 0.0f;
    if (!LEAN && s_begin != 0) {
        const float4 c = p.colors[px.li];
        acc = mk(c.x, c.y, c.z);
        if (p.moments) m2 = c.w;
    }
    const int camX = (int)p.cam.XM;
    const int gx = px.gid % camX, gy = px.gid / camX;
    const unsigned pxy = (unsigned)gx | ((unsigned)gy << 16);
    const float pix_x0 = (float)gx, pix_y0 = (float)gy;
    f3 rP = mk(0.f, 0.f, 0.f), rD = mk(0.f, 0.f, 1.f);
    PathRegs st;
    st.reset();
    for (int s = s_begin; s < s_end; ++s) {
        const float pix_x = LEAN ? (float)(pxy & 0xffffu) : pix_x0, pix_y = LEAN ? (float)(pxy >> 16) : pix_y0;
        st.reset();
        bool inside = false;
        if (SPLIT) {
            const float4* r = reinterpret_cast<const float4*>(&p.rays[px.li]);
            const float4 a = r[0], b = r[1];
            rP = mk(a.x, a.y, a.z);
            rD = mk(b.x, b.y, b.z);
        } else {
            const float rnd1 = lcg_rand(seed), rnd2 = lcg_rand(seed);
            camera_get_ray_xy(pix_x, pix_y, p.cam, rnd1, rnd2, &rP, &rD);
        }
        for (int bounce = 0; bounce < p.iterations; ++bounce) {
            if (COUNT && first_active_lane()) wc->wtrips++;
            float t;
            const int ti = closest_hit<MODE, COUNT>(sv, rP, rD, stk, &t, wc);
            ++*segs;
            if (ti < 0) break;
            if (COUNT) { if (first_active_lane()) wc->wshade++; count_low(wc, 3); }
            shade_hit<SK>(rP, rD, st, seed, inside, p, sv.tris, sv.meta, ti, t);
        }
        if (LEAN) fold_sample(p, px.li, st.C(), s);
        else {
            acc = running_mean(acc, st.C(), s);
            if (p.moments) m2 = running_moment(m2, st.C(), s);
        }
    }
    if (!LEAN) p.colors[px.li] = make_float4(acc.x, acc.y, acc.z, m2);
    p.rnds[px.li] = seed;
    if (SPLIT) {
        float4* r = reinterpret_cast<float4*>(&p.rays[px.li]);
        r[0] = make_float4(rP.x, rP.y, rP.z, 0.0f);
        r[1] = make_float4(rD.x, rD.y, rD.z, 0.0f);
    }
}

template <bool SPLIT, int MODE, bool COUNT, bool LEAN, bool SK>
PT_DEV void render_pixel_suspend(const RenderParams& p, const SceneView& sv, const LaneStack<typename StackOf<MODE>::type> stk, const PixelId px,
                                 int s_begin, int s_end, unsigned* segs, WorkCount* wc) {
    f3 rP = mk(0.f, 0.f, 0.f), rD = mk(0.f, 0.f, 1.f);
    PathRegs st;
    st.reset();
    bool inside = false;
    int seed = p.rnds[px.li];
    f3 acc = mk(0.0f, 0.0f, 0.0f);
    float m2 = 0.0f;
    if (!LEAN && s_begin != 0) {
        const float4 c = p.colors[px.li];
        acc = mk(c.x, c.y, c.z);
        if (p.moments) m2 = c.w;
    }
    int s = s_begin;
    int bounce = 0;
    bool fresh = true;
    bool traversing = false;
    Trav<MODE> tr;
    tr.setup(rP, rD);
    tr.restart(stk);
    tr.idle();
    const int camX = (int)p.cam.XM;
    const int gx = px.gid % camX, gy = px.gid / camX;
    const unsigned pxy = (unsigned)gx | ((unsigned)gy << 16);
    const float pix_x0 = (float)gx, pix_y0 = (float)gy;
    for (;;) {
        if (COUNT && first_active_lane()) wc->wtrips++;
        if (fresh && !traversing) {
            if (s == s_end) break;
            st.reset();
            inside = false;
            if (SPLIT) {
                const float4* r = reinterpret_cast<const float4*>(&p.rays[px.li]);
                const float4 a = r[0], b = r[1];
                rP = mk(a.x, a.y, a.z);
                rD = mk(b.x, b.y, b.z);
            } else {
                const float rnd1 = lcg_rand(seed), rnd2 = lcg_rand(seed);
                const float pix_x = LEAN ? (float)(pxy & 0xffffu) : pix_x0, pix_y = LEAN ? (float)(pxy >> 16) : pix_y0;
                camera_get_ray_xy(pix_x, pix_y, p.cam, rnd1, rnd2, &rP, &rD);
            }
            bounce = 0;
            fresh = false;
        }
        bool finished = true;
        if (traversing || bounce < p.iterations) {
            tr.setup(rP, rD);
            if (!traversing) {
                tr.restart(stk);
                tr.template flat_pass<COUNT>(sv, wc);
            }
            for (;;) {
                if (COUNT && first_active_lane()) wc->wrounds++;
                tr.template round<COUNT>(sv, wc);
                const unsigned long long unfinished = __ballot(!tr.done());
                if (unfinished == 0) break;
                if (__popcll(unfinished) <= p.suspend_lanes && __ballot(tr.done()) != 0) break;
            }
            traversing = !tr.done();
            if (traversing) {
                finished = false;
            } else {
                ++*segs;
                if (tr.best >= 0) {
                    if (COUNT) { if (first_active_lane()) wc->wshade++; count_low(wc, 3); }
                    shade_hit<SK>(rP, rD, st, seed, inside, p, sv.tris, sv.meta, tr.best, tr.best_t);
                    ++bounce;
                    finished = (bounce >= p.iterations);
                }
            }
        }
        if (finished) {
            if (LEAN) fold_sample(p, px.li, st.C(), s);
            else {
                acc = running_mean(acc, st.C(), s);
                if (p.moments) m2 = running_moment(m2, st.C(), s);
            }
            ++s;
                fresh = true;
        }
    }
    if (!LEAN) p.colors[px.li] = make_float4(acc.x, acc.y, acc.z, m2);
    p.rnds[px.li] = seed;
    if (SPLIT) {
        float4* r = reinterpret_cast<float4*>(&p.rays[px.li]);
        r[0] = make_float4(rP.x, rP.y, rP.z, 0.0f);
        r[1] = make_float4(rD.x, rD.y, rD.z, 0.0f);
    }
}

PT_DEV int wait_tile_pass(const RenderParams& p, int tile, int pass, bool lane0) {
    unsigned seen = 0, lost = 0, polls = 0;
    const unsigned long long w0 = __builtin_amdgcn_s_memrealtime();
    for (;;) {
        if (lane0) seen = __hip_atomic_load(&p.tile_done[tile], __ATOMIC_RELAXED, __HIP_MEMORY_SCOPE_AGENT);
        seen = (unsigned)__builtin_amdgcn_readfirstlane((int)seen);
        if (seen >= (unsigned)pass) break;
        if ((++polls & 63u) == 0) {
            if (lane0) lost = __hip_atomic_load(&p.tile_counter[kTileCounterError], __ATOMIC_RELAXED, __HIP_MEMORY_SCOPE_AGENT);
            lost = (unsigned)__builtin_amdgcn_readfirstlane((int)lost);
            if (lost != 0) break;
            if (__builtin_amdgcn_s_memrealtime() - w0 > (unsigned long long)p.poll_ticks) {
                const unsigned long long mine = ((unsigned long long)(unsigned)pass << 32) | (unsigned long long)((unsigned)tile + 1u);
                unsigned long long was = 0;
                if (lane0) was = atomicCAS(reinterpret_cast<unsigned long long*>(&p.tile_counter[kTileCounterError]), 0ull, mine);
                (void)__builtin_amdgcn_readfirstlane((int)(unsigned)was);
                break;
            }
        }
        __builtin_amdgcn_s_sleep(8);
    }
    return __builtin_amdgcn_readfirstlane((int)(seen >= (unsigned)pass));
}

template <int MODE, bool COUNT, bool LEAN, bool SK>
PT_DEV void render_items_migrating(const RenderParams& p, const SceneView& sv, const LaneStack<typename StackOf<MODE>::type> stk, WorkCount* wc,
                                   unsigned long long* segs_tot, unsigned long long* samples_tot, unsigned long long* lane_steps) {
    const bool lane0 = (threadIdx.x & 63) == 0;
    const bool chained = p.chunk_spp > 0;
    const int n_pass = chained ? (p.n_taper > 0 ? p.n_taper : (p.nsamples + p.chunk_spp - 1) / p.chunk_spp) : 1;
    const int s_last = p.first_sample + p.nsamples;
    const int camX = (int)p.cam.XM;
    f3 rP = mk(0.f, 0.f, 0.f), rD = mk(0.f, 0.f, 1.f);
    PathRegs st;
    st.reset();
    bool inside = false;
    int seed = 0;
    f3 acc = mk(0.0f, 0.0f, 0.0f);
    float m2 = 0.0f;
    int s = 0, bounce = 0;
    bool fresh = true, traversing = false;
    bool parked = true, on_next = false;
    int li = 0;
    unsigned pxy = 0;
    unsigned my_segs = 0;
    Trav<MODE> tr;
    tr.setup(rP, rD);
    tr.restart(stk);
    tr.idle();
    int cur_item = -1, nxt_item = -1;
    int cur_end = 0, nxt_end = 0;
    int nxt_ready = 0, no_more = 0;
    unsigned long long samples = 0;
    auto pass_of = [&](int item) { return chained ? item / p.n_tiles : 0; };
    auto tile_of = [&](int item) { return chained ? item - (item / p.n_tiles) * p.n_tiles : item; };

    auto fetch = [&]() {
        int t = 0;
        if (lane0) t = (int)atomicAdd(p.tile_counter, 1u);
        t = __builtin_amdgcn_readfirstlane(t);
        const bool ok = chained ? t / p.n_tiles < n_pass : t < p.n_tiles;
        return __builtin_amdgcn_readfirstlane(ok ? t : -1);
    };
    auto released = [&](int item) {
        const int pass = pass_of(item);
        if (pass == 0) return 1;
        unsigned seen = 0;
        if (lane0) seen = __hip_atomic_load(&p.tile_done[tile_of(item)], __ATOMIC_RELAXED, __HIP_MEMORY_SCOPE_AGENT);
        seen = (unsigned)__builtin_amdgcn_readfirstlane((int)seen);
        return __builtin_amdgcn_readfirstlane((int)(seen >= (unsigned)pass));
    };
    auto wait_released = [&](int item) {
        const int pass = pass_of(item);
        return pass == 0 ? 1 : wait_tile_pass(p, tile_of(item), pass, lane0);
    };
    auto begin_of = [&](int item) { const int ps = pass_of(item); return p.first_sample + (p.n_taper > 0 ? (ps > 0 ? (int)p.taper_end[ps - 1] : 0) : ps * p.chunk_spp); };
    auto end_of = [&](int item) { return !chained ? s_last : p.n_taper > 0 ? p.first_sample + (int)p.taper_end[pass_of(item)] : min(p.first_sample + (pass_of(item) + 1) * p.chunk_spp, s_last); };
    const int lane = threadIdx.x & 63;
    const int tiles_x = (p.width + 7) >> 3;
    const bool rows_aligned = (p.rows_per_block & 7) == 0;
    auto take_pixel = [&](int item) {
        const int tile = frame_tile(p, tile_of(item));
        const int ty = tile / tiles_x, tx = tile - ty * tiles_x;
        const int x = tx * 8 + (lane & 7), lrow = ty * 8 + (lane >> 3);
        if (x >= p.width || lrow >= p.local_rows) return;
        int grow;
        if (p.world == 1) grow = lrow;
        else if (rows_aligned) { const int r0 = ty * 8; grow = ((r0 / p.rows_per_block) * p.world + p.rank) * p.rows_per_block + (r0 % p.rows_per_block) + (lane >> 3); }
        else grow = global_row(p, lrow);
        li = lrow * p.width + x;
        int gx = x, gy = grow;
        if (camX != p.width) { const int gid = grow * p.width + x; gx = gid % camX; gy = gid / camX; }
        pxy = (unsigned)gx | ((unsigned)gy << 16);
        seed = p.rnds[li];
        s = begin_of(item);
        if (!LEAN) {
            acc = mk(0.0f, 0.0f, 0.0f);
            m2 = 0.0f;
            if (s != 0) {
                const float4 c = p.colors[li];
                acc = mk(c.x, c.y, c.z);
                if (p.moments) m2 = c.w;
            }
        }
        fresh = true;
        traversing = false;
        bounce = 0;
        parked = false;
    };

    for (;;) {
        if (COUNT && first_active_lane()) wc->wtrips++;
        if (!parked && fresh && !traversing && s == (on_next ? nxt_end : cur_end)) {
            if (!LEAN) p.colors[li] = make_float4(acc.x, acc.y, acc.z, m2);
            p.rnds[li] = seed;
            parked = true;
        }
        if (__ballot(!parked && !on_next) == 0) {
            if (cur_item >= 0 && chained) {
                __builtin_amdgcn_fence(__ATOMIC_RELEASE, "agent");
                asm volatile("s_waitcnt vmcnt(0)" ::: "memory");
                const int tile = tile_of(cur_item), pass = pass_of(cur_item);
                if (lane0 && !(tile == p.debug_stall_tile && pass == 0)) {
                    unsigned handed;
                    asm volatile("v_mov_b32 %0, %1" : "=v"(handed) : "s"(__builtin_amdgcn_readfirstlane(pass + 1)));
                    __hip_atomic_store(&p.tile_done[tile], handed, __ATOMIC_RELAXED, __HIP_MEMORY_SCOPE_AGENT);
                }
            }
            cur_item = -1;
            if (nxt_item < 0 && !no_more) {
                nxt_item = fetch();
                no_more = __builtin_amdgcn_readfirstlane((int)(nxt_item < 0));
                nxt_ready = 0;
            }
            if (nxt_item < 0) break;
            if (!nxt_ready) {
                if (!wait_released(nxt_item)) break;
                if (pass_of(nxt_item) > 0) __builtin_amdgcn_fence(__ATOMIC_ACQUIRE, "agent");
            }
            cur_item = __builtin_amdgcn_readfirstlane(nxt_item);
            cur_end = __builtin_amdgcn_readfirstlane(end_of(nxt_item));
            nxt_item = -1;
            nxt_ready = 0;
            if (on_next) on_next = false;
            else take_pixel(cur_item);
        } else if (__popcll(__ballot(parked && !on_next)) >= p.migrate_lanes) {
            if (nxt_item < 0 && !no_more) {
                nxt_item = fetch();
                no_more = __builtin_amdgcn_readfirstlane((int)(nxt_item < 0));
                nxt_ready = 0;
                nxt_end = __builtin_amdgcn_readfirstlane(end_of(nxt_item));
            }
            if (nxt_item >= 0 && !nxt_ready && released(nxt_item)) {
                if (pass_of(nxt_item) > 0) __builtin_amdgcn_fence(__ATOMIC_ACQUIRE, "agent");
                nxt_ready = 1;
            }
            if (nxt_item >= 0 && nxt_ready && parked && !on_next) {
                on_next = true;
                take_pixel(nxt_item);
            }
        }
        if (!parked && fresh && !traversing) {
            st.reset();
            inside = false;
            const float rnd1 = lcg_rand(seed), rnd2 = lcg_rand(seed);
            camera_get_ray_xy((float)(pxy & 0xffffu), (float)(pxy >> 16), p.cam, rnd1, rnd2, &rP, &rD);
            bounce = 0;
            fresh = false;
        }
        bool finished = !parked;
        if (!parked && (traversing || bounce < p.iterations)) {
            tr.setup(rP, rD);
            if (!traversing) {
                tr.restart(stk);
                tr.template flat_pass<COUNT>(sv, wc);
            }
            for (;;) {
                if (COUNT && first_active_lane()) wc->wrounds++;
                tr.template round<COUNT>(sv, wc);
                const unsigned long long unfinished = __ballot(!tr.done());
                if (unfinished == 0) break;
                if (__popcll(unfinished) <= p.suspend_lanes && __ballot(tr.done()) != 0) break;
            }
            traversing = !tr.done();
            if (traversing) {
                finished = false;
            } else {
                ++my_segs;
                if (tr.best >= 0) {
                    if (COUNT) { if (first_active_lane()) wc->wshade++; count_low(wc, 3); }
                    shade_hit<SK>(rP, rD, st, seed, inside, p, sv.tris, sv.meta, tr.best, tr.best_t);
                    ++bounce;
                    finished = (bounce >= p.iterations);
                }
            }
        }
        samples += (unsigned long long)__popcll(__ballot(finished));
        if (finished) {
            if (LEAN) fold_sample(p, li, st.C(), s);
            else {
                acc = running_mean(acc, st.C(), s);
                if (p.moments) m2 = running_moment(m2, st.C(), s);
            }
            ++s;
            fresh = true;
        }
    }
    {
        unsigned v = my_segs;
        for (int off = 32; off > 0; off >>= 1) v += __shfl_down(v, off, 64);
        *segs_tot += (unsigned)__builtin_amdgcn_readfirstlane((int)v);
        *samples_tot += samples;
    }
    if (COUNT) {
        unsigned mx = my_segs;
        for (int off = 32; off > 0; off >>= 1) mx = max(mx, (unsigned)__shfl_down(mx, off, 64));
        *lane_steps += (unsigned long long)(unsigned)__builtin_amdgcn_readfirstlane((int)mx) * 64ull;
    }
}

template <bool SPLIT, int MODE, int BLOCK, bool COUNT, int SCHED, int WPS>
__global__ void __launch_bounds__(BLOCK, WPS) k_render(RenderParams p) {
    constexpr bool kLean = WPS >= kLeanFromWps;
    constexpr bool kScalarK = WPS >= 5;
    LaneStack<typename StackOf<MODE>::type> stk;
    SceneView sv;
    setup_traversal<MODE, BLOCK>(p, &sv, &stk);
    WorkCount wc;
    wc.nodes = 0;
    wc.tris = 0;
    wc.wnodes = 0;
    wc.wtris = 0;
    wc.wshade = 0;
    wc.wtrips = 0;
    wc.wrounds = 0;
    for (int i = 0; i < 6; ++i) wc.low[i] = 0;
    const bool lane0 = (threadIdx.x & 63) == 0;
    const bool chained = p.tile_counter != nullptr && p.chunk_spp > 0;
    const int n_pass = chained ? (p.n_taper > 0 ? p.n_taper : (p.nsamples + p.chunk_spp - 1) / p.chunk_spp) : 1;
    unsigned long long segs_tot = 0, samples_tot = 0, item_lane_steps = 0;
    int tile = __builtin_amdgcn_readfirstlane((int)((blockIdx.x * blockDim.x + threadIdx.x) >> 6));
    int pass = 0;
    if (SCHED == kSchedMigrate) {
        if (p.tile_counter) render_items_migrating<MODE, COUNT, kLean, kScalarK>(p, sv, stk, &wc, &segs_tot, &samples_tot, &item_lane_steps);
    } else
    for (;;) {
        if (p.tile_counter) {
            int t = 0;
            if (lane0) t = (int)atomicAdd(p.tile_counter, 1u);
#ifdef PT_TEST_WORK_ITEM_IN_VGPR
            t = __shfl(t, 0, 64);
#else
            t = __builtin_amdgcn_readfirstlane(t);
#endif
            pass = chained ? t / p.n_tiles : 0;
            tile = t - pass * p.n_tiles;
            if (chained ? pass >= n_pass : tile >= p.n_tiles) break;
            if (pass > 0) {
                if (!wait_tile_pass(p, tile, pass, lane0)) break;
                __builtin_amdgcn_fence(__ATOMIC_ACQUIRE, "agent");
            }
        }
        const bool tabled = chained && p.n_taper > 0;
        const int s_begin = p.first_sample + (tabled ? (pass > 0 ? (int)p.taper_end[pass - 1] : 0) : chained ? pass * p.chunk_spp : 0);
        const int s_end = tabled ? p.first_sample + (int)p.taper_end[pass] : chained ? min(s_begin + p.chunk_spp, p.first_sample + p.nsamples) : p.first_sample + p.nsamples;
        const int ftile = frame_tile(p, tile);
        const PixelId px = pixel_of_wave(p, ftile);
        unsigned item_segs = 0;
        const unsigned long long item_t0 = COUNT ? __builtin_amdgcn_s_memtime() : 0ull;
        if (px.li >= 0) {
            if (SCHED == kSchedLockstep) render_pixel_lockstep<SPLIT, MODE, COUNT, kLean, kScalarK>(p, sv, stk, px, s_begin, s_end, &item_segs, &wc);
            else render_pixel_suspend<SPLIT, MODE, COUNT, kLean, kScalarK>(p, sv, stk, px, s_begin, s_end, &item_segs, &wc);
        }
        {
            unsigned v = item_segs;
            for (int off = 32; off > 0; off >>= 1) v += __shfl_down(v, off, 64);
            segs_tot += (unsigned)__builtin_amdgcn_readfirstlane((int)v);
            samples_tot += (unsigned long long)__popcll(__ballot(px.li >= 0)) * (unsigned)(s_end - s_begin);
        }
        if (COUNT) {
            unsigned mx = item_segs;
            for (int off = 32; off > 0; off >>= 1) mx = max(mx, (unsigned)__shfl_down(mx, off, 64));
            const unsigned mxs = (unsigned)__builtin_amdgcn_readfirstlane((int)mx);
            item_lane_steps += (unsigned long long)mxs * 64ull;
            if (p.tile_cost && lane0) atomicAdd(&p.tile_cost[ftile], (unsigned)((__builtin_amdgcn_s_memtime() - item_t0) >> 6));
        }
        if (chained) {
            __builtin_amdgcn_fence(__ATOMIC_RELEASE, "agent");
            asm volatile("s_waitcnt vmcnt(0)" ::: "memory");
            if (lane0 && !(tile == p.debug_stall_tile && pass == 0))
                __hip_atomic_store(&p.tile_done[tile], (unsigned)(pass + 1), __ATOMIC_RELAXED, __HIP_MEMORY_SCOPE_AGENT);
        }
        if (!p.tile_counter) break;
    }
    if (p.tile_counter) {
        unsigned gone = 0;
        if (lane0) gone = atomicAdd(p.tile_counter + 1, 1u);
        gone = (unsigned)__builtin_amdgcn_readfirstlane((int)gone);
        if (lane0 && gone + 1u == gridDim.x * (BLOCK / 64)) {
            __hip_atomic_store(p.tile_counter, 0u, __ATOMIC_RELAXED, __HIP_MEMORY_SCOPE_AGENT);
            __hip_atomic_store(p.tile_counter + 1, 0u, __ATOMIC_RELAXED, __HIP_MEMORY_SCOPE_AGENT);
        }
    }
    if (COUNT) {
        const unsigned long long wn = wave_sum((unsigned long long)wc.nodes), wt = wave_sum((unsigned long long)wc.tris);
        const unsigned long long wwn = wave_sum((unsigned long long)wc.wnodes), wwt = wave_sum((unsigned long long)wc.wtris);
        const unsigned long long wsh = wave_sum((unsigned long long)wc.wshade), wtr = wave_sum((unsigned long long)wc.wtrips), wro = wave_sum((unsigned long long)wc.wrounds);
        if (lane0 && p.stats) {
            stat_add(p, 2, wn);
            stat_add(p, 3, wt);
            stat_add(p, 4, wwn);
            stat_add(p, 5, wwt);
            stat_add(p, 6, item_lane_steps);
            stat_add(p, 7, wsh);
            stat_add(p, 8, wtr);
            stat_add(p, 9, wro);
        }
        for (int i = 0; i < 6; ++i) {
            const unsigned long long v = wave_sum((unsigned long long)wc.low[i]);
            if (lane0 && p.stats) stat_add(p, 10 + i, v);
        }
    }
    if (lane0 && p.stats) {
        stat_add(p, 0, segs_tot);
        stat_add(p, 1, samples_tot);
    }
}

PT_DEV float srgb1(float a) {
    if (a <= 0.00304f) return 12.92f * a;
    return fmaf_(1.055f, spec_pow<false>(a, 0.4167f), -0.055f);
}
__global__ void __launch_bounds__(256) k_resolve_reinhard(const float4* colors, float4* out, long long n) {
    const long long i = (long long)blockIdx.x * blockDim.x + threadIdx.x;
    if (i >= n) return;
    const float4 c = colors[i];
    const float L = fmaf_(0.0722f, c.z, fmaf_(0.7152f, c.y, 0.2126f * c.x));
    const float L2 = L / (1.0f + L);
    out[i] = make_float4(srgb1(c.x * L2 / L), srgb1(c.y * L2 / L), srgb1(c.z * L2 / L), 1.0f);
}

PT_DEV float filmic1(float cin) {
    float c = cin - 0.004f;
    c = c > 0.0f ? c : 0.0f;
    return (c * fmaf_(c, 6.2f, 0.5f)) / fmaf_(c, fmaf_(c, 6.2f, 1.7f), 0.06f);
}
__global__ void __launch_bounds__(256) k_filt_im(const float4* colors, float4* out, int W, int H) {
    const int x = blockIdx.x * 32 + (threadIdx.x & 31);
    const int y = blockIdx.y * 8 + (threadIdx.x >> 5);
    if (x <= 0 || y <= 0 || x >= W - 1 || y >= H - 1) return;
    float4 arr[9];
    float grey[9];
#pragma unroll
    for (int i = 0; i < 3; ++i)
#pragma unroll
        for (int j = 0; j < 3; ++j) {
            const float4 c = colors[(size_t)(y - 1 + i) * W + (x - 1 + j)];
            arr[i * 3 + j] = c;
            grey[i * 3 + j] = ((c.x + c.y) + c.z) / 3.0f;
        }
#pragma unroll
    for (int jn = 9; jn > 1; --jn) {
        int maxi = 0;
#pragma unroll
        for (int i = 1; i < jn; ++i)
            if (grey[i] > grey[maxi]) maxi = i;
#pragma unroll
        for (int i = 0; i < 9; ++i) {
            if (i == maxi) {
                const float tg = grey[jn - 1];
                const float4 tv = arr[jn - 1];
                grey[jn - 1] = grey[i];
                arr[jn - 1] = arr[i];
                grey[i] = tg;
                arr[i] = tv;
            }
        }
    }
    out[(size_t)y * W + x] = make_float4(filmic1(arr[4].x), filmic1(arr[4].y), filmic1(arr[4].z), 1.0f);
}

static inline int n_waves(const RenderParams& p) {
    const int tiles_x = (p.width + 7) >> 3, tiles_y = (p.local_rows + 7) >> 3;
    return tiles_x * tiles_y;
}

int traversal_block(int node_mode, bool wide_lds_block) { return node_mode == kNodesLds ? (wide_lds_block ? kLdsBlockWide : kLdsBlockBase) : node_mode == kNodesTreelet ? 1024 : 256; }

size_t traversal_lds_bytes(const RenderParams& p, int block) {
    size_t b = (size_t)p.stack_entries * (p.node_mode == kNodesLds ? 2 : 4) * (size_t)block;
    b = (b + 15) & ~(size_t)15;
    if (p.node_mode == kNodesLds) b += ((size_t)p.n_nodes * kLdsNodeBytes + 15) & ~(size_t)15;
    if (p.node_mode == kNodesTreelet) b += (size_t)p.treelet_nodes * 64;
    return b + (size_t)p.n_flat * 100;
}

hipError_t launch_gen_ray(const RenderParams& p, hipStream_t stream) {
    const int waves = n_waves(p);
    if (waves == 0) return hipSuccess;
    const int blocks = (waves + 3) / 4;
    hipLaunchKernelGGL(k_gen_ray, dim3(blocks), dim3(256), 0, stream, p);
    return hipGetLastError();
}

template <bool SPLIT, int MODE, int BLOCK, bool COUNT, int SCHED, int WPS>
static hipError_t launch_one(const RenderParams& p, const LaunchConfig& lc, hipStream_t stream) {
    const int waves = p.tile_list ? p.n_tiles : n_waves(p);
    if (waves == 0) return hipSuccess;
    constexpr int wpb = BLOCK / 64;
    int blocks = (waves + wpb - 1) / wpb;
    if (p.tile_counter) blocks = std::min(blocks, lc.persistent_blocks);
    if (p.stack_ovf && (long long)blocks * BLOCK > (long long)p.stack_ovf_lanes) return hipErrorInvalidValue;
    auto kern = k_render<SPLIT, MODE, BLOCK, COUNT, SCHED, WPS>;
    static LdsMark mark;
    const hipError_t e = ensure_dynamic_lds((const void*)kern, mark, lc.lds_bytes);
    if (e != hipSuccess) return e;
    if (p.tile_counter && lc.cu_count > 0) {
        static OccMark occ;
        const int per_cu = resident_blocks_per_cu((const void*)kern, occ, BLOCK, lc.lds_bytes);
        if (per_cu > 0) blocks = std::min(blocks, per_cu * lc.cu_count);
    }
    hipLaunchKernelGGL(kern, dim3(blocks), dim3(BLOCK), lc.lds_bytes, stream, p);
    return hipGetLastError();
}

template <bool SPLIT, bool COUNT, int SCHED>
static hipError_t launch_render_t(const RenderParams& p, const LaunchConfig& lc, hipStream_t stream) {
    if (lc.block != traversal_block(p.node_mode, lc.block == kLdsBlockWide)) return hipErrorInvalidValue;
    switch (p.node_mode) {
    case kNodesLds:
        if (lc.block == kLdsBlockWide) return launch_one<SPLIT, kNodesLds, kLdsBlockWide, COUNT, SCHED, kLdsWpsWide>(p, lc, stream);
        return launch_one<SPLIT, kNodesLds, kLdsBlockBase, COUNT, SCHED, kLdsWpsBase>(p, lc, stream);
    case kNodesGlobal:
        if (lc.waves_per_simd == 8) return launch_one<SPLIT, kNodesGlobal, 256, COUNT, SCHED, 8>(p, lc, stream);
        if (lc.waves_per_simd == 7) return launch_one<SPLIT, kNodesGlobal, 256, COUNT, SCHED, 7>(p, lc, stream);
        if (lc.waves_per_simd == 6) return launch_one<SPLIT, kNodesGlobal, 256, COUNT, SCHED, 6>(p, lc, stream);
        if (lc.waves_per_simd == 5) return launch_one<SPLIT, kNodesGlobal, 256, COUNT, SCHED, 5>(p, lc, stream);
        return launch_one<SPLIT, kNodesGlobal, 256, COUNT, SCHED, 4>(p, lc, stream);
    case kNodesWide:
        if (lc.waves_per_simd == 8) return launch_one<SPLIT, kNodesWide, 256, COUNT, SCHED, 8>(p, lc, stream);
        if (lc.waves_per_simd == 7) return launch_one<SPLIT, kNodesWide, 256, COUNT, SCHED, 7>(p, lc, stream);
        if (lc.waves_per_simd == 6) return launch_one<SPLIT, kNodesWide, 256, COUNT, SCHED, 6>(p, lc, stream);
        if (lc.waves_per_simd == 5) return launch_one<SPLIT, kNodesWide, 256, COUNT, SCHED, 5>(p, lc, stream);
        return launch_one<SPLIT, kNodesWide, 256, COUNT, SCHED, 4>(p, lc, stream);
    case kNodesTreelet: return launch_one<SPLIT, kNodesTreelet, 1024, COUNT, SCHED, 4>(p, lc, stream);
    }
    return hipErrorInvalidValue;
}

hipError_t launch_trace_ray(const RenderParams& p, const LaunchConfig& lc, hipStream_t stream) { return launch_render_t<true, false, kSchedLockstep>(p, lc, stream); }
hipError_t launch_render_mega(const RenderParams& p, const LaunchConfig& lc, hipStream_t stream) {
    if (lc.schedule == kSchedLockstep)
        return lc.count_work ? launch_render_t<false, true, kSchedLockstep>(p, lc, stream) : launch_render_t<false, false, kSchedLockstep>(p, lc, stream);
    if (lc.schedule == kSchedMigrate && p.tile_counter)
        return lc.count_work ? launch_render_t<false, true, kSchedMigrate>(p, lc, stream) : launch_render_t<false, false, kSchedMigrate>(p, lc, stream);
    return lc.count_work ? launch_render_t<false, true, kSchedSuspend>(p, lc, stream) : launch_render_t<false, false, kSchedSuspend>(p, lc, stream);
}

hipError_t launch_resolve_reinhard(const float4* colors, float4* out, int64_t n, hipStream_t stream) {
    if (n == 0) return hipSuccess;
    hipLaunchKernelGGL(k_resolve_reinhard, dim3((unsigned)((n + 255) / 256)), dim3(256), 0, stream, colors, out, (long long)n);
    return hipGetLastError();
}

hipError_t launch_filt_im(const float4* colors, float4* out, int32_t W, int32_t H, hipStream_t stream) {
    hipLaunchKernelGGL(k_filt_im, dim3((W + 31) / 32, (H + 7) / 8), dim3(256), 0, stream, colors, out, W, H);
    return hipGetLastError();
}

}
```

### opencl_path_tracer_amd/csrc/pt_launch.cpp

```cpp
#include "pt_context.hpp"

namespace ptamd {

int32_t count_local_rows(int32_t H, int32_t rank, int32_t world, int32_t rb) {
    int32_t n = 0;
    for (int32_t r = 0; r < H; ++r)
        if ((r / rb) % world == rank) ++n;
    return n;
}

int wide_stack_entries(int pending) { return ((pending + 4) + 1) & ~1; }
int stack_entries_for(int interior_depth) { return std::min(kStackEntries, ((interior_depth + 2) + 1) & ~1); }


bool whole_tree_fits_lds(size_t n_nodes, size_t n_tris, int interior_depth, int n_flat) {
    const bool s16 = n_nodes <= 32767 && n_tris <= 4096;
    const size_t block = (size_t)kLdsBlockBase;
    return s16 && (size_t)kLdsNodeBytes * n_nodes + 16 + (size_t)stack_entries_for(interior_depth) * 2 * block + (size_t)n_flat * 100 + 64 <= kLdsPerCu / 2;
}

static void group_flat_boxes(pt_context* ctx) {
    ctx->n_fbox = 0;
    float ext[32][6];
    for (int k = 0; k < ctx->n_flat; ++k) {
        const float* v = ctx->packets[(size_t)k].v;
        float e[6];
        for (int a = 0; a < 3; ++a) {
            e[a] = std::min(std::min(v[a], v[3 + a]), v[6 + a]);
            e[3 + a] = std::max(std::max(v[a], v[3 + a]), v[6 + a]);
        }
        int b = 0;
        for (; b < ctx->n_fbox; ++b)
            if (std::memcmp(ext[b], e, sizeof e) == 0) break;
        if (b == ctx->n_fbox) {
            std::memcpy(ext[b], e, sizeof e);
            ctx->fbox_rep[b] = (uint8_t)k;
            ctx->fbox_mask[b] = 0;
            ctx->n_fbox++;
        }
        ctx->fbox_mask[b] |= 1u << k;
    }
}

int plan_node_placement(pt_context* ctx, const float4* d_bvh2, bool* wide_on_device) {
    PhaseClock clk("node placement");
    if (wide_on_device) *wide_on_device = false;
    ctx->treelet_nodes = 0;
    group_flat_boxes(ctx);
    ctx->interior_depth = deepest_interior_node(ctx->nodes);
    clk.lap("list boxes + interior depth");
    if (ctx->interior_depth + 2 > kStackEntries) return fail(ctx, PT_ESCENE, "internal: BVH deeper than the traversal stack");
    const bool fits = whole_tree_fits_lds(ctx->nodes.size(), ctx->orig.size(), ctx->interior_depth, ctx->n_flat);
    if (ctx->treelet != 0 && !fits) ctx->treelet_nodes = reindex_treelet(ctx->nodes, ctx->interior_depth, ctx->treelet);
    ctx->nodes4.clear();
    ctx->wide_pending = 0;
    if (ctx->wide_nodes == 2 || (ctx->wide_nodes == 1 && !fits && ctx->treelet_nodes == 0)) {
        if (d_bvh2 && ctx->treelet_nodes == 0 && ctx->wide_on_device != 0) {
            float4* d4 = nullptr;
            int n4 = 0, pending = 0;
            bool failed = false;
            PT_HIP(ctx, wide_device_build(d_bvh2, (int)ctx->nodes.size(), ctx->stream, &d4, &n4, &pending, &failed));
            if (!failed) {
                if (ctx->d_nodes4) (void)hipFree(ctx->d_nodes4);
                ctx->d_nodes4 = d4;
                ctx->nodes4.resize((size_t)n4);
                ctx->wide_pending = pending;
                PT_HIP(ctx, hipMemcpy(ctx->nodes4.data(), d4, sizeof(Node4q) * (size_t)n4, hipMemcpyDeviceToHost));
                if (wide_on_device) *wide_on_device = true;
            }
            clk.lap("4-wide nodes (device)");
            return PT_OK;
        }
        const unsigned hw = std::thread::hardware_concurrency();
        const int threads = ctx->build_threads > 0 ? ctx->build_threads : (int)std::min(16u, std::max(1u, hw));
        if (!build_wide_nodes(ctx->nodes, &ctx->nodes4, &ctx->wide_pending, threads)) ctx->nodes4.clear();
        clk.lap("4-wide nodes (host)");
    }
    return PT_OK;
}

int alloc_stack_overflow(pt_context* ctx) {
    if (ctx->d_stack_ovf) { PT_HIP(ctx, hipFree(ctx->d_stack_ovf)); ctx->d_stack_ovf = nullptr; }
    ctx->stack_ovf_lanes = 0;
    const int extra = ctx->nodes4.empty() ? 0 : wide_stack_entries(ctx->wide_pending) - ctx->wide_lds_entries;
    if (extra <= 0) return PT_OK;
    const size_t n_tiles = (size_t)((ctx->W + 7) / 8) * (size_t)((ctx->local_rows + 7) / 8);
    const size_t lanes = 256 * std::max<size_t>((size_t)ctx->cu_count * 12 * kWfDefaultChains, (n_tiles + 3) / 4);
    PT_HIP(ctx, hipMalloc((void**)&ctx->d_stack_ovf, lanes * (size_t)extra * sizeof(uint32_t)));
    ctx->stack_ovf_lanes = lanes;
    return PT_OK;
}

int seed_upload(pt_context* ctx, const int32_t* global_seeds) {
    std::vector<int32_t> local((size_t)ctx->npix);
    for (int32_t lr = 0; lr < ctx->local_rows; ++lr) {
        const int32_t gr = global_row(*ctx, lr);
        std::memcpy(&local[(size_t)lr * ctx->W], &global_seeds[(size_t)gr * ctx->W], sizeof(int32_t) * (size_t)ctx->W);
    }
    if (ctx->npix) PT_HIP(ctx, hipMemcpyAsync(ctx->d_rnds, local.data(), sizeof(int32_t) * local.size(), hipMemcpyHostToDevice, ctx->stream));
    PT_HIP(ctx, hipStreamSynchronize(ctx->stream));
    return PT_OK;
}

void fill_params(const pt_context* ctx, const pt_camera* cam, RenderParams* p) {
    std::memset(p, 0, sizeof *p);
    p->nodes = ctx->d_nodes;
    p->tris = ctx->d_tris;
    p->meta = ctx->d_meta;
    p->mats = ctx->d_mats;
    p->rnds = ctx->d_rnds;
    p->colors = ctx->d_colors;
    p->rays = ctx->d_rays;
    p->stats = ctx->d_stats;
    p->moments = ctx->moments;
    p->cam = *cam;
    p->width = ctx->W;
    p->height = ctx->H;
    p->local_rows = ctx->local_rows;
    p->rank = ctx->rank;
    p->world = ctx->world;
    p->rows_per_block = ctx->rows_per_block;
    p->n_nodes = (int32_t)ctx->nodes.size();
    p->n_tris = (int32_t)ctx->orig.size();
    p->n_flat = ctx->n_flat;
    p->n_fbox = ctx->n_fbox;
    std::memcpy(p->fbox_rep, ctx->fbox_rep, sizeof p->fbox_rep);
    std::memcpy(p->fbox_mask, ctx->fbox_mask, sizeof p->fbox_mask);
    p->stack_entries = stack_entries_for(ctx->interior_depth);
    p->stack_ovf = nullptr;
    p->stack_ovf_lanes = 0;
    p->node_mode = kNodesGlobal;
    p->treelet_nodes = 0;
    if (ctx->lds_scene) {
        if (whole_tree_fits_lds(ctx->nodes.size(), ctx->orig.size(), ctx->interior_depth, ctx->n_flat)) {
            p->node_mode = kNodesLds;
        } else if (ctx->treelet_nodes > 0) {
            p->node_mode = kNodesTreelet;
            p->treelet_nodes = ctx->treelet_nodes;
        }
    }
    if (!ctx->nodes4.empty() && (p->node_mode == kNodesGlobal || ctx->wide_nodes == 2)) {
        p->node_mode = kNodesWide;
        p->treelet_nodes = 0;
        p->nodes = ctx->d_nodes4;
        p->stack_entries = std::min(ctx->wide_lds_entries, wide_stack_entries(ctx->wide_pending));
        p->stack_ovf = ctx->d_stack_ovf;
        p->stack_ovf_lanes = (int32_t)ctx->stack_ovf_lanes;
    }
    p->tile_counter = nullptr;
    p->poll_ticks = (uint32_t)std::min<int64_t>((int64_t)ctx->poll_timeout_ms * 100000, 0xffffffffll);
    p->debug_stall_tile = ctx->debug_stall_tile;
    p->chunk_spp = 0;
    p->n_taper = 0;
    p->tile_done = nullptr;
    p->n_tiles = ((ctx->W + 7) / 8) * ((ctx->local_rows + 7) / 8);
    p->suspend_lanes = ctx->suspend_lanes >= 0 ? ctx->suspend_lanes : (p->node_mode == kNodesLds ? 16 : 24);
    p->node_min_lanes = ctx->node_min_lanes >= 0 ? ctx->node_min_lanes : (p->node_mode == kNodesLds ? 3 : 6);
    p->leaf_min_lanes = ctx->leaf_min_lanes >= 0 ? ctx->leaf_min_lanes : 4;
    p->migrate_lanes = ctx->migrate_lanes > 0 ? ctx->migrate_lanes : 1;
}

int check_ready(pt_context* ctx, const pt_camera* cam) {
    if (!cam) return fail(ctx, PT_EINVAL, "camera is NULL");
    if (!ctx->tris_uploaded) return fail(ctx, PT_EINVAL, "pt_upload_triangles has not been called");
    if (!ctx->mats_uploaded) return fail(ctx, PT_EINVAL, "pt_upload_materials has not been called");
    if ((int32_t)cam->XM != ctx->W || (int32_t)cam->YM != ctx->H)
        return fail(ctx, PT_EINVAL, "camera XM/YM do not match the context's frame size");
    return PT_OK;
}

int time_begin(pt_context* ctx, EventPair** ep) {
    *ep = nullptr;
    if (!ctx->timing) return PT_OK;
    if (ctx->events_used == ctx->events.size()) {
        EventPair e;
        PT_HIP(ctx, hipEventCreate(&e.a));
        PT_HIP(ctx, hipEventCreate(&e.b));
        ctx->events.push_back(e);
    }
    *ep = &ctx->events[ctx->events_used++];
    PT_HIP(ctx, hipEventRecord((*ep)->a, ctx->stream));
    return PT_OK;
}
int time_end(pt_context* ctx, EventPair* ep) {
    ctx->kernel_launches++;
    if (ep) PT_HIP(ctx, hipEventRecord(ep->b, ctx->stream));
    return PT_OK;
}
int time_collect(pt_context* ctx) {
    for (size_t i = 0; i < ctx->events_used; ++i) {
        float ms = 0.f;
        PT_HIP(ctx, hipEventSynchronize(ctx->events[i].b));
        PT_HIP(ctx, hipEventElapsedTime(&ms, ctx->events[i].a, ctx->events[i].b));
        ctx->kernel_ms_acc += ms;
    }
    ctx->events_used = 0;
    return PT_OK;
}


int sync_and_check(pt_context* ctx) {
    PT_HIP(ctx, hipSetDevice(ctx->device));
    const hipError_t e = hipStreamSynchronize(ctx->stream);
    if (e != hipSuccess) {
        ctx->counters_suspect = true;
        return fail(ctx, PT_EHIP, std::string("hipStreamSynchronize: ") + hipGetErrorString(e));
    }
    if (!ctx->launched_since_check || !ctx->d_tile_counter) return PT_OK;
    ctx->launched_since_check = false;
    uint32_t words[kTileCounterWords] = {};
    PT_HIP(ctx, hipMemcpy(words, ctx->d_tile_counter, sizeof words, hipMemcpyDeviceToHost));
    if (words[kTileCounterError] != 0) {
        ctx->counters_suspect = true;
        PT_HIP(ctx, hipMemset(ctx->d_tile_counter, 0, sizeof words));
        ctx->counters_suspect = false;
        char msg[256];
        std::snprintf(msg, sizeof msg, "k_render: pass %u of tile %u waited more than %d ms for the tile's previous pass to be handed over (the "
                      "wave rendering it was lost); the launch was wound down, the frame is incomplete", words[kTileCounterError + 1],
                      words[kTileCounterError] - 1, ctx->poll_timeout_ms);
        return fail(ctx, PT_EHIP, msg);
    }
    return PT_OK;
}

}

extern "C" {

static int prepare_work_counter(pt_context* ctx) {
    if (ctx->counters_suspect) {
        PT_HIP(ctx, hipMemsetAsync(ctx->d_tile_counter, 0, sizeof(uint32_t) * kTileCounterWords, ctx->stream));
        ctx->counters_suspect = false;
    }
    ctx->launched_since_check = true;
    return PT_OK;
}

static int ptamd_resident_waves(const pt_context*, const LaunchConfig& lc) { return lc.persistent_blocks * (lc.block / 64); }

static int auto_chunk_spp(int n_tiles, int resident_waves, int nsamples, int schedule, int node_mode) {
    if (schedule == 2) return node_mode == kNodesLds ? 32 : nsamples >= 32 ? 16 : nsamples >= 16 ? 8 : nsamples >= 8 ? 4 : 0;
    return n_tiles >= 5 * resident_waves ? (nsamples >= 256 ? 64 : 32)
         : n_tiles >= 3 * resident_waves ? 16
         : n_tiles > resident_waves + resident_waves / 4 ? 8 : 0;
}
static int auto_chunk_taper(int nsamples, int schedule, int node_mode) {
    if (schedule == 0) return nsamples >= 32 ? 2 : 0;
    if (schedule != 2) return 0;
    return node_mode == kNodesLds ? (nsamples >= 64 ? 8 : 0) : (nsamples >= 32 ? 4 : 0);
}

static void launch_cfg(pt_context* ctx, const RenderParams& p, LaunchConfig* lc) {
    const bool wide_fits = p.node_mode == kNodesLds && 2 * (traversal_lds_bytes(p, kLdsBlockWide) + 512) <= kLdsPerCu;
    const bool wide_block = wide_fits && ctx->lds_block != kLdsBlockBase &&
                            (ctx->lds_block == kLdsBlockWide || p.n_tiles >= 2 * ctx->cu_count * 2 * (kLdsBlockWide / 64));
    lc->block = traversal_block(p.node_mode, wide_block);
    lc->lds_bytes = traversal_lds_bytes(p, lc->block);
    lc->count_work = ctx->count_work != 0;
    lc->waves_per_simd = wide_block ? kLdsWpsWide : 4;
    if (p.node_mode == kNodesGlobal || p.node_mode == kNodesWide) {
        const int want = ctx->waves_per_simd > 0 ? ctx->waves_per_simd : 7;
        for (int w = std::min(want, 8); w > 4; --w)
            if ((size_t)w * lc->lds_bytes + 1024 <= kLdsPerCu) { lc->waves_per_simd = w; break; }
    }
    lc->persistent_blocks = ctx->cu_count * std::max(1, 256 * lc->waves_per_simd / lc->block);
    lc->cu_count = ctx->cu_count;
    const bool few_samples = p.nsamples <= (p.node_mode == kNodesLds ? 4 : 1);
    const int restart = (ctx->persistent && (p.node_mode != kNodesLds || p.nsamples >= 64)) ? 2 : 1;
    lc->schedule = ctx->schedule >= 0 ? ctx->schedule : (!few_samples && p.n_tiles >= 3 * ptamd_resident_waves(ctx, *lc) ? restart : 0);
    ctx->last_lds_bytes = lc->lds_bytes;
    ctx->last_waves_per_simd = lc->waves_per_simd;
}

int pt_generate_rays(pt_context* ctx, const pt_camera* cam) {
    PT_NEED_DEVICE(ctx);
    int rc = check_ready(ctx, cam);
    if (rc != PT_OK) return rc;
    PT_HIP(ctx, hipSetDevice(ctx->device));
    RenderParams p;
    fill_params(ctx, cam, &p);
    PT_HIP(ctx, launch_gen_ray(p, ctx->stream));
    return PT_OK;
}

int pt_trace_rays(pt_context* ctx, const pt_camera* cam, int32_t iterations, int32_t current_sample) {
    PT_NEED_DEVICE(ctx);
    int rc = check_ready(ctx, cam);
    if (rc != PT_OK) return rc;
    if (iterations < 0 || current_sample < 0) return fail(ctx, PT_EINVAL, "iterations/current_sample must be >= 0");
    if (ctx->adaptive_frame) return fail(ctx, PT_EINVAL, "an adaptive frame is held: pt_set_current_sample(ctx, 0) starts a new frame");
    PT_HIP(ctx, hipSetDevice(ctx->device));
    RenderParams p;
    fill_params(ctx, cam, &p);
    p.iterations = iterations;
    p.first_sample = current_sample;
    p.nsamples = 1;
    LaunchConfig lc;
    launch_cfg(ctx, p, &lc);
    if (ctx->persistent) {
        if (int rc2 = prepare_work_counter(ctx)) return rc2;
        p.tile_counter = ctx->d_tile_counter;
    }
    EventPair* ep;
    if ((rc = time_begin(ctx, &ep)) != PT_OK) return rc;
    {
        const hipError_t le = launch_trace_ray(p, lc, ctx->stream);
        if (le != hipSuccess) { ctx->counters_suspect = true; return fail(ctx, PT_EHIP, std::string("launch_trace_ray: ") + hipGetErrorString(le)); }
    }
    ctx->render_epoch++;
    note_frame(ctx, current_sample, cam);
    rc = time_end(ctx, ep);
    if (rc != PT_OK) ctx->counters_suspect = true;
    return rc;
}

static int render_wavefront(pt_context* ctx, const RenderParams& rp, int32_t nsamples) {
    if (rp.iterations > kWfMaxBounces) return fail(ctx, PT_EINVAL, "wavefront variant supports at most 1023 iterations");
    const size_t np = (size_t)std::max<int64_t>(ctx->npix, 1);
    constexpr size_t kCounterWords = (size_t)kWfCounterStride * (kWfMaxBounces + 4);
    if (!ctx->d_wf_state) {
        PT_HIP(ctx, hipMalloc((void**)&ctx->d_wf_state, sizeof(float4) * 17 * np));
        PT_HIP(ctx, hipMalloc((void**)&ctx->d_wf_queues, sizeof(int32_t) * 3 * np));
        PT_HIP(ctx, hipMalloc((void**)&ctx->d_wf_counters, sizeof(uint32_t) * kCounterWords * kWfMaxChains));
    }
    if (ctx->npix == 0) return PT_OK;
    const int want = ctx->wf_streams > 0 ? ctx->wf_streams : kWfDefaultChains;
    int chains = (int)std::max<int64_t>(1, std::min<int64_t>(std::min(want, kWfMaxChains), ctx->npix / 65536));
    const size_t chain_lanes = (size_t)2 * 6 * 256 * (size_t)ctx->cu_count;
    if (rp.stack_ovf) chains = (int)std::max<size_t>(1, std::min<size_t>((size_t)chains, (size_t)rp.stack_ovf_lanes / chain_lanes));
    for (int c = 1; c < chains; ++c)
        if (!ctx->wf_stream[c]) {
            PT_HIP(ctx, hipStreamCreateWithFlags(&ctx->wf_stream[c], hipStreamNonBlocking));
            PT_HIP(ctx, hipEventCreateWithFlags(&ctx->wf_event[c], hipEventDisableTiming));
        }
    if (!ctx->wf_event[0]) PT_HIP(ctx, hipEventCreateWithFlags(&ctx->wf_event[0], hipEventDisableTiming));
    WfParams w[kWfMaxChains];
    const int64_t unit = 8192;
    const int64_t per = ((ctx->npix + chains - 1) / chains + unit - 1) / unit * unit;
    for (int c = 0; c < chains; ++c) {
        WfParams& wc = w[c];
        const int64_t p0 = std::min<int64_t>((int64_t)c * per, ctx->npix), count = std::min<int64_t>(p0 + per, ctx->npix) - p0;
        wc.rp = rp;
        if (rp.stack_ovf) wc.rp.stack_ovf = rp.stack_ovf + (size_t)c * chain_lanes;
        wc.sP = reinterpret_cast<float*>(ctx->d_wf_state);
        for (int par = 0; par < 2; ++par)
            for (int k = 0; k < 2; ++k) {
                wc.rsA[par][k] = ctx->d_wf_state + (size_t)(4 + (par * 2 + k) * 2 + 0) * np + p0;
                wc.rsB[par][k] = ctx->d_wf_state + (size_t)(4 + (par * 2 + k) * 2 + 1) * np + p0;
                wc.rsC[par][k] = ctx->d_wf_state + (size_t)(13 + par * 2 + k) * np + p0;
            }
        wc.hit[0] = reinterpret_cast<float2*>(ctx->d_wf_state + 12 * np) + p0;
        wc.hit[1] = reinterpret_cast<float2*>(ctx->d_wf_state + 12 * np) + np + p0;
        for (int k = 0; k < 3; ++k) wc.q_cls[k] = ctx->d_wf_queues + (size_t)k * np + p0;
        wc.counters = ctx->d_wf_counters + (size_t)c * kCounterWords;
        wc.npix = (int32_t)count;
        wc.pix0 = (int32_t)p0;
        wc.npix_all = (int32_t)ctx->npix;
        wc.n_cbox = ctx->cost_binning ? (int32_t)(ctx->cost_boxes.size() / 6) : 0;
        for (int b = 0; b < wc.n_cbox; ++b)
            for (int k = 0; k < 6; ++k) wc.cbox[b][k] = ctx->cost_boxes[(size_t)b * 6 + k];
    }
    PT_HIP(ctx, hipEventRecord(ctx->wf_event[0], ctx->stream));
    for (int c = 1; c < chains; ++c) PT_HIP(ctx, hipStreamWaitEvent(ctx->wf_stream[c], ctx->wf_event[0], 0));
    for (int32_t k = 0; k < nsamples; ++k) {
        for (int c = 0; c < chains; ++c) {
            if (w[c].npix == 0) continue;
            hipStream_t st = c == 0 ? ctx->stream : ctx->wf_stream[c];
            w[c].sample = rp.first_sample + k;
            PT_HIP(ctx, hipMemsetAsync(w[c].counters, 0, sizeof(uint32_t) * kWfCounterStride, st));
            PT_HIP(ctx, launch_wf_generate(w[c], st));
        }
        for (int32_t b = 0; b < rp.iterations; ++b)
            for (int c = 0; c < chains; ++c) {
                if (w[c].npix == 0) continue;
                hipStream_t st = c == 0 ? ctx->stream : ctx->wf_stream[c];
                EventPair* ep = nullptr;
                int rc = PT_OK;
                if (c == 0 && (rc = time_begin(ctx, &ep)) != PT_OK) return rc;
                PT_HIP(ctx, launch_wf_intersect(w[c], b, ctx->cu_count, st));
                if (c == 0 && (rc = time_end(ctx, ep)) != PT_OK) return rc;
                PT_HIP(ctx, launch_wf_shade(w[c], b, st));
            }
        if (ctx->timing && ctx->events_used >= 4096) {
            int rc = time_collect(ctx);
            if (rc != PT_OK) return rc;
        }
    }
    for (int c = 1; c < chains; ++c) {
        PT_HIP(ctx, hipEventRecord(ctx->wf_event[c], ctx->wf_stream[c]));
        PT_HIP(ctx, hipStreamWaitEvent(ctx->stream, ctx->wf_event[c], 0));
    }
    return PT_OK;
}

static int launch_megakernel(pt_context* ctx, RenderParams& p, const int32_t* tile_list, int32_t n_active) {
    int rc = PT_OK;
    const int32_t nsamples = p.nsamples;
    if (tile_list) {
        p.tile_list = tile_list;
        p.n_tiles = n_active;
    }
    const size_t frame_tiles = (size_t)local_tiles(ctx);
    LaunchConfig lc;
    launch_cfg(ctx, p, &lc);
    if (ctx->persistent) {
        if (int rc2 = prepare_work_counter(ctx)) return rc2;
        p.tile_counter = ctx->d_tile_counter;
        const int resident_waves = ptamd_resident_waves(ctx, lc);
        const int auto_chunk = auto_chunk_spp(p.n_tiles, resident_waves, nsamples, lc.schedule, p.node_mode);
        const int chunk = ctx->chunk_spp >= 0 ? ctx->chunk_spp : auto_chunk;
        int n_pass = chunk > 0 ? (int)(((int64_t)nsamples + chunk - 1) / chunk) : 1;
        const int taper = ctx->chunk_taper >= 0 ? ctx->chunk_taper : auto_chunk_taper(nsamples, lc.schedule, p.node_mode);
        if (chunk > 0 && nsamples > chunk && taper > 0 && taper < chunk && nsamples < 65536) {
            std::vector<int> ends;
            int done = 0;
            while (nsamples - done > chunk) { done += chunk; ends.push_back(done); }
            for (int left = nsamples - done; left > 0;) {
                const int take = left >= 2 * taper ? left / 2 : left;
                done += take;
                left -= take;
                ends.push_back(done);
            }
            if ((int)ends.size() <= kMaxTaperPasses) {
                n_pass = p.n_taper = (int)ends.size();
                for (int k = 0; k < n_pass; ++k) p.taper_end[k] = (uint16_t)ends[k];
            }
        }
        const int64_t items = chunk > 0 ? (int64_t)n_pass * p.n_tiles : p.n_tiles;
        if (items + (int64_t)resident_waves + 64 >= ((int64_t)1 << 31))
            return fail(ctx, PT_EINVAL, "nsamples / chunk_spp x tiles does not fit the 31-bit work-item counter of one launch: render in several calls");
        if (chunk > 0 && nsamples > chunk && p.n_tiles > 0) {
            if (!ctx->d_tile_done) PT_HIP(ctx, hipMalloc((void**)&ctx->d_tile_done, sizeof(uint32_t) * frame_tiles));
            PT_HIP(ctx, hipMemsetAsync(ctx->d_tile_done, 0, sizeof(uint32_t) * (size_t)p.n_tiles, ctx->stream));
            p.tile_done = ctx->d_tile_done;
            p.chunk_spp = chunk;
        }
    }
    if (lc.count_work && p.n_tiles > 0) {
        if (!ctx->d_tile_cost) PT_HIP(ctx, hipMalloc((void**)&ctx->d_tile_cost, sizeof(uint32_t) * (frame_tiles + 16)));
        PT_HIP(ctx, hipMemsetAsync(ctx->d_tile_cost, 0, sizeof(uint32_t) * frame_tiles, ctx->stream));
        p.tile_cost = ctx->d_tile_cost;
    }
    EventPair* ep;
    if ((rc = time_begin(ctx, &ep)) != PT_OK) return rc;
    {
        const hipError_t le = launch_render_mega(p, lc, ctx->stream);
        if (le != hipSuccess) { ctx->counters_suspect = true; return fail(ctx, PT_EHIP, std::string("launch_render_mega: ") + hipGetErrorString(le)); }
    }
    if ((rc = time_end(ctx, ep)) != PT_OK) { ctx->counters_suspect = true; return rc; }
    return PT_OK;
}

int pt_render(pt_context* ctx, const pt_camera* cam, int32_t iterations, int32_t nsamples) {
    PT_NEED_DEVICE(ctx);
    int rc = check_ready(ctx, cam);
    if (rc != PT_OK) return rc;
    if (iterations < 0 || nsamples < 0) return fail(ctx, PT_EINVAL, "iterations/nsamples must be >= 0");
    if (ctx->adaptive_frame) return fail(ctx, PT_EINVAL, "an adaptive frame is held: pt_set_current_sample(ctx, 0) starts a new frame");
    if (nsamples == 0) return PT_OK;
    PT_HIP(ctx, hipSetDevice(ctx->device));
    RenderParams p;
    fill_params(ctx, cam, &p);
    p.iterations = iterations;
    p.first_sample = ctx->current_sample;
    p.nsamples = nsamples;
    ctx->render_epoch++;
    note_frame(ctx, p.first_sample, cam);
    if (ctx->variant == 1) {
        if ((rc = render_wavefront(ctx, p, nsamples)) != PT_OK) return rc;
        ctx->current_sample += nsamples;
        return PT_OK;
    }
    if ((rc = launch_megakernel(ctx, p, nullptr, p.n_tiles)) != PT_OK) return rc;
    ctx->current_sample += nsamples;
    return PT_OK;
}

static std::string adaptive_bounds(int32_t min_spp, int32_t max_spp, std::vector<int32_t>* out) {
    if (min_spp < 2 || (min_spp & 1)) return "min_spp must be even and >= 2";
    if (max_spp < min_spp) return "max_spp must be >= min_spp";
    out->clear();
    out->push_back(min_spp / 2);
    for (int64_t b = min_spp;; b = std::min<int64_t>(2 * b, max_spp)) {
        out->push_back((int32_t)b);
        if (b == max_spp) break;
    }
    return "";
}

int pt_render_adaptive(pt_context* ctx, const pt_camera* cam, int32_t iterations, int32_t min_spp, int32_t max_spp, float threshold) {
    if (!ctx) return PT_EINVAL;
    std::vector<int32_t> bounds;
    std::string why = adaptive_bounds(min_spp, max_spp, &bounds);
    if (why.empty() && !(threshold >= 0.0f)) why = "threshold must be >= 0 (and not NaN)";
    if (why.empty() && iterations < 0) why = "iterations must be >= 0";
    if (why.empty()) {
        int64_t longest = bounds[0];
        for (size_t k = 1; k < bounds.size(); ++k) longest = std::max<int64_t>(longest, (int64_t)bounds[k] - bounds[k - 1]);
        if (longest * (int64_t)local_tiles(ctx) + ((int64_t)1 << 20) >= ((int64_t)1 << 31))
            why = "max_spp too large: a round of " + std::to_string(longest) + " samples over " + std::to_string(local_tiles(ctx)) +
                  " tiles does not fit the 31-bit work-item counter of one launch";
    }
    if (!why.empty()) return fail(ctx, PT_EINVAL, "pt_render_adaptive: " + why);
    PT_NEED_DEVICE(ctx);
    int rc = check_ready(ctx, cam);
    if (rc != PT_OK) return rc;
    if (ctx->variant != 0) return fail(ctx, PT_EINVAL, "pt_render_adaptive: the megakernel (variant 0) only");
    if (ctx->world != 1) return fail(ctx, PT_EINVAL, "pt_render_adaptive: contexts of one rank (world == 1) only");
    if (ctx->adaptive_frame) return fail(ctx, PT_EINVAL, "an adaptive frame is held: pt_set_current_sample(ctx, 0) starts a new frame");
    if (ctx->current_sample != 0) return fail(ctx, PT_EINVAL, "pt_render_adaptive starts a frame: current_sample must be 0");
    PT_HIP(ctx, hipSetDevice(ctx->device));
    const int32_t n_frame = local_tiles(ctx);
    if (!ctx->d_adapt_snap) {
        PT_HIP(ctx, hipMalloc((void**)&ctx->d_adapt_snap, sizeof(float4) * (size_t)std::max<int64_t>(ctx->npix, 1)));
        PT_HIP(ctx, hipMalloc((void**)&ctx->d_adapt_spp, sizeof(int32_t) * (size_t)n_frame));
        PT_HIP(ctx, hipMalloc((void**)&ctx->d_adapt_err, sizeof(float) * (size_t)n_frame));
        PT_HIP(ctx, hipMalloc((void**)&ctx->d_adapt_active, (size_t)n_frame));
        PT_HIP(ctx, hipMalloc((void**)&ctx->d_adapt_list, sizeof(int32_t) * ((size_t)n_frame + 1)));
        PT_HIP(ctx, hipHostMalloc((void**)&ctx->h_adapt_count, sizeof(int32_t), hipHostMallocDefault));
    }
    int32_t* d_count = ctx->d_adapt_list + n_frame;
    PT_HIP(ctx, hipMemsetAsync(ctx->d_adapt_active, 1, (size_t)n_frame, ctx->stream));
    PT_HIP(ctx, hipMemsetAsync(d_count, 0, sizeof(int32_t), ctx->stream));
    PT_HIP(ctx, hipMemsetAsync(ctx->d_adapt_spp, 0, sizeof(int32_t) * (size_t)n_frame, ctx->stream));
    PT_HIP(ctx, hipMemsetD32Async((hipDeviceptr_t)ctx->d_adapt_err, 0x7f800000, (size_t)n_frame, ctx->stream));
    ctx->adaptive_frame = true;
    ctx->render_epoch++;
    note_frame(ctx, 0, cam);
    RenderParams p;
    fill_params(ctx, cam, &p);
    p.iterations = iterations;
    const int32_t* list = nullptr;
    int32_t n_active = n_frame;
    for (size_t k = 0; k < bounds.size(); ++k) {
        const int32_t b = bounds[k], prev = k == 0 ? 0 : bounds[k - 1];
        RenderParams pr = p;
        pr.first_sample = prev;
        pr.nsamples = b - prev;
        if ((rc = launch_megakernel(ctx, pr, list, n_active)) != PT_OK) return rc;
        ctx->current_sample = b;
        const int mode = k == 0 ? 1 : b < max_spp ? 2 : 0;
        PT_HIP(ctx, launch_adaptive_tiles(ctx->d_colors, ctx->d_adapt_snap, list, n_active, ctx->W, ctx->local_rows, mode, threshold, b,
                                          ctx->d_adapt_err, ctx->d_adapt_spp, ctx->d_adapt_active, ctx->stream));
        if (mode != 2) continue;
        PT_HIP(ctx, launch_compact_tiles(ctx->d_adapt_active, n_frame, ctx->d_adapt_list, d_count, ctx->stream));
        PT_HIP(ctx, hipMemcpyAsync(ctx->h_adapt_count, d_count, sizeof(int32_t), hipMemcpyDeviceToHost, ctx->stream));
        if ((rc = sync_and_check(ctx)) != PT_OK) return rc;
        n_active = *ctx->h_adapt_count;
        list = ctx->d_adapt_list;
        if (n_active == 0) break;
    }
    return PT_OK;
}

int pt_debug_adaptive_list(pt_context* ctx, int32_t* out, int64_t cap, int64_t* n) {
    PT_NEED_DEVICE(ctx);
    if (!n || cap < 0 || (cap > 0 && !out)) return fail(ctx, PT_EINVAL, "pt_debug_adaptive_list: n non-null, cap >= 0, out non-null when cap > 0");
    *n = 0;
    if (!ctx->adaptive_frame || !ctx->d_adapt_list) return PT_OK;
    int rc = sync_and_check(ctx);
    if (rc != PT_OK) return rc;
    const int32_t n_frame = local_tiles(ctx);
    int32_t count = 0;
    PT_HIP(ctx, hipMemcpy(&count, ctx->d_adapt_list + n_frame, sizeof count, hipMemcpyDeviceToHost));
    *n = count;
    if (cap > 0 && count > 0) PT_HIP(ctx, hipMemcpy(out, ctx->d_adapt_list, sizeof(int32_t) * (size_t)std::min<int64_t>(cap, count), hipMemcpyDeviceToHost));
    return PT_OK;
}

int pt_adaptive_rounds(int32_t min_spp, int32_t max_spp, int32_t* out, int32_t cap, int32_t* count) {
    std::vector<int32_t> bounds;
    std::string why = adaptive_bounds(min_spp, max_spp, &bounds);
    if (why.empty() && (!count || cap < 0 || (cap > 0 && !out))) why = "count must be non-null, cap >= 0, out non-null when cap > 0";
    if (!why.empty()) return fail(nullptr, PT_EINVAL, "pt_adaptive_rounds: " + why);
    *count = (int32_t)bounds.size();
    for (int32_t k = 0; k < std::min<int32_t>(cap, *count); ++k) out[k] = bounds[(size_t)k];
    return PT_OK;
}

int pt_set_current_sample(pt_context* ctx, int32_t s) {
    if (!ctx || s < 0) return PT_EINVAL;
    ctx->current_sample = s;
    if (s == 0) ctx->adaptive_frame = false;
    return PT_OK;
}
int pt_get_current_sample(const pt_context* ctx, int32_t* out) {
    if (!ctx || !out) return PT_EINVAL;
    *out = ctx->current_sample;
    return PT_OK;
}


int pt_sync(pt_context* ctx) {
    PT_NEED_DEVICE(ctx);
    return sync_and_check(ctx);
}

int pt_debug_launch_plan(pt_context* ctx, int32_t nsamples, int32_t cu_count, int64_t out[8]) {
    if (!ctx || !out || nsamples < 1 || cu_count < 0) return PT_EINVAL;
    if (!ctx->tris_uploaded) return fail(ctx, PT_EINVAL, "upload_Triangles first");
    pt_camera cam;
    const float shift[3] = {0.f, 0.f, 0.f};
    pt_camera_init(&cam, 60.0f, 0.0f, 0.0f, shift, ctx->W, ctx->H);
    RenderParams p;
    fill_params(ctx, &cam, &p);
    p.nsamples = nsamples;
    const int saved_cu = ctx->cu_count;
    const size_t saved_lds = ctx->last_lds_bytes;
    const int saved_wps = ctx->last_waves_per_simd;
    if (cu_count > 0) ctx->cu_count = cu_count;
    LaunchConfig lc;
    launch_cfg(ctx, p, &lc);
    const int resident = ptamd_resident_waves(ctx, lc);
    ctx->cu_count = saved_cu;
    ctx->last_lds_bytes = saved_lds;
    ctx->last_waves_per_simd = saved_wps;
    const int chunk = ctx->chunk_spp >= 0 ? ctx->chunk_spp : auto_chunk_spp(p.n_tiles, resident, nsamples, lc.schedule, p.node_mode);
    out[0] = lc.block; out[1] = lc.waves_per_simd; out[2] = lc.schedule; out[3] = (chunk > 0 && nsamples > chunk) ? chunk : 0;
    out[4] = resident; out[5] = p.n_tiles; out[6] = p.node_mode; out[7] = (int64_t)lc.lds_bytes;
    return PT_OK;
}


}
```

Measured before the change: 2787.

## Overlap consecutive persistent megakernel launches via ping-pong streams and dry signals

Adds two alternating streams with separate tile counters and stack-overflow slices, so the next persistent render launch can begin once the previous one's work queue runs dry. The previous launch signals this through a system-scope memory word that the next stream waits on with hipStreamWaitValue32. Tile completion counters now carry an epoch base, so the next launch's pass-0 items wait per tile on the prior launch's results, and the per-launch memset of tile_done is removed. The aim is to hide the tail drain and launch gap between back-to-back renders. In exchange it adds synchronisation complexity, a startup probe, and fallback paths.

```diff
diff --git a/opencl_path_tracer_amd/csrc/pt_context.hpp b/opencl_path_tracer_amd/csrc/pt_context.hpp
--- a/opencl_path_tracer_amd/csrc/pt_context.hpp
+++ b/opencl_path_tracer_amd/csrc/pt_context.hpp
@@ -23,6 +23,23 @@
 struct EventPair {
     hipEvent_t a = nullptr, b = nullptr;
 };
+struct CtxStream {
+    hipStream_t s = nullptr;
+    mutable bool touched = true;
+    operator hipStream_t() const { touched = true; return s; }
+    CtxStream& operator=(hipStream_t v) { s = v; touched = true; return *this; }
+    hipStream_t quiet() const { return s; }
+};
+struct OverlapKey {
+    int block = 0, schedule = 0, waves_per_simd = 0, persistent_blocks = 0, n_tiles = 0;
+    size_t lds_bytes = 0;
+    const void* colors = nullptr;
+    const void* rnds = nullptr;
+    bool operator==(const OverlapKey& o) const {
+        return block == o.block && schedule == o.schedule && waves_per_simd == o.waves_per_simd && persistent_blocks == o.persistent_blocks &&
+               n_tiles == o.n_tiles && lds_bytes == o.lds_bytes && colors == o.colors && rnds == o.rnds;
+    }
+};
 }
 
 struct pt_context {
@@ -66,6 +83,7 @@
     float4* d_nodes4 = nullptr;
     uint32_t* d_stack_ovf = nullptr;
     size_t stack_ovf_lanes = 0;
+    size_t stack_ovf_words = 0;
     float4* d_tris = nullptr;
     TriMeta* d_meta = nullptr;
     pt_material* d_mats = nullptr;
@@ -86,7 +104,21 @@
     bool launched_since_check = false;
     int wf_streams = -1;
     bool own_rnds = true, own_colors = true;
-    hipStream_t stream = nullptr;
+    CtxStream stream;
+
+    int overlap_launches = 1;
+    bool overlap_ok = false;
+    hipStream_t ov_stream[2] = {};
+    hipEvent_t ov_done[2] = {};
+    hipEvent_t ov_entry = nullptr;
+    uint32_t* ov_signal = nullptr;
+    uint32_t ov_serial = 0;
+    int ov_parity = 0;
+    bool ov_chain = false;
+    OverlapKey ov_key;
+    int64_t overlapped_launches = 0;
+    uint32_t done_epoch = 0;
+    hipStream_t time_stream = nullptr;
 
     int32_t current_sample = 0;
 
@@ -309,6 +341,7 @@
 int time_end(pt_context* ctx, EventPair* ep);
 int time_collect(pt_context* ctx);
 int sync_and_check(pt_context* ctx);
+int setup_overlap(pt_context* ctx);
 inline int32_t local_tiles(const pt_context* c) { return ((c->W + 7) / 8) * ((c->local_rows + 7) / 8); }
 template <class T>
 int upload_vec(pt_context* ctx, T** dptr, const void* src, size_t bytes) {
diff --git a/opencl_path_tracer_amd/csrc/pt_host.cpp b/opencl_path_tracer_amd/csrc/pt_host.cpp
--- a/opencl_path_tracer_amd/csrc/pt_host.cpp
+++ b/opencl_path_tracer_amd/csrc/pt_host.cpp
@@ -168,12 +168,16 @@
     if ((e = hipMalloc((void**)&ctx->d_rnds, sizeof(int32_t) * np)) != hipSuccess) return bail("hipMalloc(rnds)", e);
     if ((e = hipMalloc((void**)&ctx->d_colors, sizeof(float4) * nslab)) != hipSuccess) return bail("hipMalloc(colors)", e);
     if ((e = hipMalloc((void**)&ctx->d_stats, sizeof(unsigned long long) * kStatCols * kStatRows)) != hipSuccess) return bail("hipMalloc(stats)", e);
-    if ((e = hipMalloc((void**)&ctx->d_tile_counter, sizeof(uint32_t) * kTileCounterWords)) != hipSuccess) return bail("hipMalloc(tile counter)", e);
-    if ((e = hipMemset(ctx->d_tile_counter, 0, sizeof(uint32_t) * kTileCounterWords)) != hipSuccess) return bail("hipMemset", e);
+    if ((e = hipMalloc((void**)&ctx->d_tile_counter, sizeof(uint32_t) * kTileCounterWords * kTileCounters)) != hipSuccess) return bail("hipMalloc(tile counter)", e);
+    if ((e = hipMemset(ctx->d_tile_counter, 0, sizeof(uint32_t) * kTileCounterWords * kTileCounters)) != hipSuccess) return bail("hipMemset", e);
+    const size_t ntile = (size_t)std::max<int32_t>(local_tiles(ctx), 1);
+    if ((e = hipMalloc((void**)&ctx->d_tile_done, sizeof(uint32_t) * ntile)) != hipSuccess) return bail("hipMalloc(tile done)", e);
+    if ((e = hipMemset(ctx->d_tile_done, 0, sizeof(uint32_t) * ntile)) != hipSuccess) return bail("hipMemset", e);
     if ((e = hipMemset(ctx->d_rays, 0, sizeof(pt_ray) * np)) != hipSuccess) return bail("hipMemset", e);
     if ((e = hipMemset(ctx->d_colors, 0, sizeof(float4) * nslab)) != hipSuccess) return bail("hipMemset", e);
     if ((e = hipMemset(ctx->d_stats, 0, sizeof(unsigned long long) * kStatCols * kStatRows)) != hipSuccess) return bail("hipMemset", e);
     int rc = pt_seed_default(ctx);
+    if (rc == PT_OK) rc = setup_overlap(ctx);
     if (rc != PT_OK) {
         std::string msg = ctx->err;
         pt_destroy(ctx);
@@ -222,6 +226,12 @@
         if (ctx->d_wf_state) (void)hipFree(ctx->d_wf_state);
         if (ctx->d_wf_queues) (void)hipFree(ctx->d_wf_queues);
         if (ctx->d_wf_counters) (void)hipFree(ctx->d_wf_counters);
+        for (int k = 0; k < 2; ++k) {
+            if (ctx->ov_stream[k]) (void)hipStreamDestroy(ctx->ov_stream[k]);
+            if (ctx->ov_done[k]) (void)hipEventDestroy(ctx->ov_done[k]);
+        }
+        if (ctx->ov_entry) (void)hipEventDestroy(ctx->ov_entry);
+        if (ctx->ov_signal) (void)hipFree(ctx->ov_signal);
         for (int c = 0; c < kWfMaxChains; ++c) {
             if (ctx->wf_stream[c]) (void)hipStreamDestroy(ctx->wf_stream[c]);
             if (ctx->wf_event[c]) (void)hipEventDestroy(ctx->wf_event[c]);
@@ -849,7 +859,11 @@
 int pt_set_option(pt_context* ctx, const char* key, int64_t value) {
     if (!ctx || !key) return PT_EINVAL;
     std::string k(key);
-    if (k == "variant") {
+    ctx->stream.touched = true;
+    if (k == "overlap_launches") {
+        if (value != 0 && value != 1) return fail(ctx, PT_EINVAL, "overlap_launches must be 0 (every launch on the context's stream, one after the other) or 1");
+        ctx->overlap_launches = (int)value;
+    } else if (k == "variant") {
         if (value != 0 && value != 1) return fail(ctx, PT_EINVAL, "variant must be 0 (megakernel) or 1 (wavefront)");
         ctx->variant = (int)value;
     } else if (k == "lds_scene") {
@@ -985,6 +999,8 @@
         return PT_OK;
     }
     if (k == "kernel_launches") { *out = (double)ctx->kernel_launches; return PT_OK; }
+    if (k == "overlap_mode") { *out = (ctx->overlap_ok && ctx->overlap_launches != 0) ? 1.0 : 0.0; return PT_OK; }
+    if (k == "overlapped_launches") { *out = (double)ctx->overlapped_launches; return PT_OK; }
     PT_NEED_DEVICE(ctx);
     PT_HIP(ctx, hipSetDevice(ctx->device));
     if (k == "kernel_ms") {
diff --git a/opencl_path_tracer_amd/csrc/pt_internal.hpp b/opencl_path_tracer_amd/csrc/pt_internal.hpp
--- a/opencl_path_tracer_amd/csrc/pt_internal.hpp
+++ b/opencl_path_tracer_amd/csrc/pt_internal.hpp
@@ -55,6 +55,7 @@
 constexpr int kTileCounterError = 16;
 constexpr int kMaxTaperPasses = 30;
 constexpr int kTileCounterWords = 32;
+constexpr int kTileCounters = 2;
 constexpr int kStatRows = 256;
 constexpr int kStatCols = 16;
 #ifndef PT_LEAN_FROM_WPS
@@ -101,6 +102,10 @@
     uint16_t taper_end[kMaxTaperPasses];
     int32_t chunk_spp;
     uint32_t* tile_done;
+    uint32_t done_base;
+    int32_t wait_pass0;
+    uint32_t* dry_word;
+    uint32_t dry_value;
     int32_t suspend_lanes;
     int32_t node_min_lanes;
     int32_t leaf_min_lanes;
@@ -227,6 +232,7 @@
 hipError_t launch_gen_ray(const RenderParams& p, hipStream_t stream);
 hipError_t launch_trace_ray(const RenderParams& p, const LaunchConfig& lc, hipStream_t stream);
 hipError_t launch_render_mega(const RenderParams& p, const LaunchConfig& lc, hipStream_t stream);
+hipError_t launch_signal_probe(uint32_t* word, uint32_t value, hipStream_t stream);
 hipError_t launch_resolve_reinhard(const float4* colors, float4* out, int64_t n, hipStream_t stream);
 hipError_t launch_filt_im(const float4* colors, float4* out, int32_t width, int32_t height, hipStream_t stream);
 hipError_t launch_wf_generate(const WfParams& p, hipStream_t stream);
diff --git a/opencl_path_tracer_amd/csrc/pt_kernels.hip b/opencl_path_tracer_amd/csrc/pt_kernels.hip
--- a/opencl_path_tracer_amd/csrc/pt_kernels.hip
+++ b/opencl_path_tracer_amd/csrc/pt_kernels.hip
@@ -183,11 +183,12 @@
 
 PT_DEV int wait_tile_pass(const RenderParams& p, int tile, int pass, bool lane0) {
     unsigned seen = 0, lost = 0, polls = 0;
+    const unsigned need = (unsigned)__builtin_amdgcn_readfirstlane((int)(p.done_base + (unsigned)pass));
     const unsigned long long w0 = __builtin_amdgcn_s_memrealtime();
     for (;;) {
         if (lane0) seen = __hip_atomic_load(&p.tile_done[tile], __ATOMIC_RELAXED, __HIP_MEMORY_SCOPE_AGENT);
         seen = (unsigned)__builtin_amdgcn_readfirstlane((int)seen);
-        if (seen >= (unsigned)pass) break;
+        if (seen >= need) break;
         if ((++polls & 63u) == 0) {
             if (lane0) lost = __hip_atomic_load(&p.tile_counter[kTileCounterError], __ATOMIC_RELAXED, __HIP_MEMORY_SCOPE_AGENT);
             lost = (unsigned)__builtin_amdgcn_readfirstlane((int)lost);
@@ -202,7 +203,16 @@
         }
         __builtin_amdgcn_s_sleep(8);
     }
-    return __builtin_amdgcn_readfirstlane((int)(seen >= (unsigned)pass));
+    return __builtin_amdgcn_readfirstlane((int)(seen >= need));
+}
+
+PT_DEV unsigned fresh_from_scalar(unsigned v) {
+    unsigned r;
+    asm volatile("v_mov_b32 %0, %1" : "=v"(r) : "s"(__builtin_amdgcn_readfirstlane((int)v)));
+    return r;
+}
+PT_DEV void signal_dry(const RenderParams& p, bool lane0) {
+    if (p.dry_word && lane0) __hip_atomic_store(p.dry_word, fresh_from_scalar(p.dry_value), __ATOMIC_RELAXED, __HIP_MEMORY_SCOPE_SYSTEM);
 }
 
 template <int MODE, bool COUNT, bool LEAN, bool SK>
@@ -211,6 +221,8 @@
     const bool lane0 = (threadIdx.x & 63) == 0;
     const bool chained = p.chunk_spp > 0;
     const int n_pass = chained ? (p.n_taper > 0 ? p.n_taper : (p.nsamples + p.chunk_spp - 1) / p.chunk_spp) : 1;
+    const int n_items = __builtin_amdgcn_readfirstlane(n_pass * p.n_tiles);
+    const bool publish = p.tile_done != nullptr;
     const int s_last = p.first_sample + p.nsamples;
     const int camX = (int)p.cam.XM;
     f3 rP = mk(0.f, 0.f, 0.f), rD = mk(0.f, 0.f, 1.f);
@@ -241,20 +253,20 @@
         int t = 0;
         if (lane0) t = (int)atomicAdd(p.tile_counter, 1u);
         t = __builtin_amdgcn_readfirstlane(t);
+        if (t == n_items) signal_dry(p, lane0);
         const bool ok = chained ? t / p.n_tiles < n_pass : t < p.n_tiles;
         return __builtin_amdgcn_readfirstlane(ok ? t : -1);
     };
+    auto waits = [&](int item) { return __builtin_amdgcn_readfirstlane((int)(pass_of(item) > 0 || p.wait_pass0 != 0)); };
     auto released = [&](int item) {
-        const int pass = pass_of(item);
-        if (pass == 0) return 1;
+        if (!waits(item)) return 1;
         unsigned seen = 0;
         if (lane0) seen = __hip_atomic_load(&p.tile_done[tile_of(item)], __ATOMIC_RELAXED, __HIP_MEMORY_SCOPE_AGENT);
         seen = (unsigned)__builtin_amdgcn_readfirstlane((int)seen);
-        return __builtin_amdgcn_readfirstlane((int)(seen >= (unsigned)pass));
+        return __builtin_amdgcn_readfirstlane((int)(seen >= p.done_base + (unsigned)pass_of(item)));
     };
     auto wait_released = [&](int item) {
-        const int pass = pass_of(item);
-        return pass == 0 ? 1 : wait_tile_pass(p, tile_of(item), pass, lane0);
+        return !waits(item) ? 1 : wait_tile_pass(p, tile_of(item), pass_of(item), lane0);
     };
     auto begin_of = [&](int item) { const int ps = pass_of(item); return p.first_sample + (p.n_taper > 0 ? (ps > 0 ? (int)p.taper_end[ps - 1] : 0) : ps * p.chunk_spp); };
     auto end_of = [&](int item) { return !chained ? s_last : p.n_taper > 0 ? p.first_sample + (int)p.taper_end[pass_of(item)] : min(p.first_sample + (pass_of(item) + 1) * p.chunk_spp, s_last); };
@@ -299,13 +311,13 @@
             parked = true;
         }
         if (__ballot(!parked && !on_next) == 0) {
-            if (cur_item >= 0 && chained) {
+            if (cur_item >= 0 && publish) {
                 __builtin_amdgcn_fence(__ATOMIC_RELEASE, "agent");
                 asm volatile("s_waitcnt vmcnt(0)" ::: "memory");
                 const int tile = tile_of(cur_item), pass = pass_of(cur_item);
                 if (lane0 && !(tile == p.debug_stall_tile && pass == 0)) {
                     unsigned handed;
-                    asm volatile("v_mov_b32 %0, %1" : "=v"(handed) : "s"(__builtin_amdgcn_readfirstlane(pass + 1)));
+                    asm volatile("v_mov_b32 %0, %1" : "=v"(handed) : "s"(__builtin_amdgcn_readfirstlane((int)p.done_base + pass + 1)));
                     __hip_atomic_store(&p.tile_done[tile], handed, __ATOMIC_RELAXED, __HIP_MEMORY_SCOPE_AGENT);
                 }
             }
@@ -318,7 +330,7 @@
             if (nxt_item < 0) break;
             if (!nxt_ready) {
                 if (!wait_released(nxt_item)) break;
-                if (pass_of(nxt_item) > 0) __builtin_amdgcn_fence(__ATOMIC_ACQUIRE, "agent");
+                if (waits(nxt_item)) __builtin_amdgcn_fence(__ATOMIC_ACQUIRE, "agent");
             }
             cur_item = __builtin_amdgcn_readfirstlane(nxt_item);
             cur_end = __builtin_amdgcn_readfirstlane(end_of(nxt_item));
@@ -334,7 +346,7 @@
                 nxt_end = __builtin_amdgcn_readfirstlane(end_of(nxt_item));
             }
             if (nxt_item >= 0 && !nxt_ready && released(nxt_item)) {
-                if (pass_of(nxt_item) > 0) __builtin_amdgcn_fence(__ATOMIC_ACQUIRE, "agent");
+                if (waits(nxt_item)) __builtin_amdgcn_fence(__ATOMIC_ACQUIRE, "agent");
                 nxt_ready = 1;
             }
             if (nxt_item >= 0 && nxt_ready && parked && !on_next) {
@@ -420,6 +432,7 @@
     const bool lane0 = (threadIdx.x & 63) == 0;
     const bool chained = p.tile_counter != nullptr && p.chunk_spp > 0;
     const int n_pass = chained ? (p.n_taper > 0 ? p.n_taper : (p.nsamples + p.chunk_spp - 1) / p.chunk_spp) : 1;
+    const int n_items = __builtin_amdgcn_readfirstlane(n_pass * p.n_tiles);
     unsigned long long segs_tot = 0, samples_tot = 0, item_lane_steps = 0;
     int tile = __builtin_amdgcn_readfirstlane((int)((blockIdx.x * blockDim.x + threadIdx.x) >> 6));
     int pass = 0;
@@ -435,10 +448,11 @@
 #else
             t = __builtin_amdgcn_readfirstlane(t);
 #endif
+            if (t == n_items) signal_dry(p, lane0);
             pass = chained ? t / p.n_tiles : 0;
             tile = t - pass * p.n_tiles;
             if (chained ? pass >= n_pass : tile >= p.n_tiles) break;
-            if (pass > 0) {
+            if (pass > 0 || p.wait_pass0) {
                 if (!wait_tile_pass(p, tile, pass, lane0)) break;
                 __builtin_amdgcn_fence(__ATOMIC_ACQUIRE, "agent");
             }
@@ -467,11 +481,11 @@
             item_lane_steps += (unsigned long long)mxs * 64ull;
             if (p.tile_cost && lane0) atomicAdd(&p.tile_cost[ftile], (unsigned)((__builtin_amdgcn_s_memtime() - item_t0) >> 6));
         }
-        if (chained) {
+        if (p.tile_done) {
             __builtin_amdgcn_fence(__ATOMIC_RELEASE, "agent");
             asm volatile("s_waitcnt vmcnt(0)" ::: "memory");
             if (lane0 && !(tile == p.debug_stall_tile && pass == 0))
-                __hip_atomic_store(&p.tile_done[tile], (unsigned)(pass + 1), __ATOMIC_RELAXED, __HIP_MEMORY_SCOPE_AGENT);
+                __hip_atomic_store(&p.tile_done[tile], fresh_from_scalar(p.done_base + (unsigned)(pass + 1)), __ATOMIC_RELAXED, __HIP_MEMORY_SCOPE_AGENT);
         }
         if (!p.tile_counter) break;
     }
@@ -482,6 +496,8 @@
         if (lane0 && gone + 1u == gridDim.x * (BLOCK / 64)) {
             __hip_atomic_store(p.tile_counter, 0u, __ATOMIC_RELAXED, __HIP_MEMORY_SCOPE_AGENT);
             __hip_atomic_store(p.tile_counter + 1, 0u, __ATOMIC_RELAXED, __HIP_MEMORY_SCOPE_AGENT);
+            if (p.dry_word && __hip_atomic_load(p.dry_word, __ATOMIC_RELAXED, __HIP_MEMORY_SCOPE_SYSTEM) < p.dry_value)
+                __hip_atomic_store(p.dry_word, fresh_from_scalar(p.dry_value), __ATOMIC_RELAXED, __HIP_MEMORY_SCOPE_SYSTEM);
         }
     }
     if (COUNT) {
@@ -639,6 +655,14 @@
     return lc.count_work ? launch_render_t<false, true, kSchedSuspend>(p, lc, stream) : launch_render_t<false, false, kSchedSuspend>(p, lc, stream);
 }
 
+__global__ void k_signal_probe(uint32_t* word, uint32_t value) {
+    if (threadIdx.x == 0) __hip_atomic_store(word, value, __ATOMIC_RELAXED, __HIP_MEMORY_SCOPE_SYSTEM);
+}
+hipError_t launch_signal_probe(uint32_t* word, uint32_t value, hipStream_t stream) {
+    hipLaunchKernelGGL(k_signal_probe, dim3(1), dim3(64), 0, stream, word, value);
+    return hipGetLastError();
+}
+
 hipError_t launch_resolve_reinhard(const float4* colors, float4* out, int64_t n, hipStream_t stream) {
     if (n == 0) return hipSuccess;
     hipLaunchKernelGGL(k_resolve_reinhard, dim3((unsigned)((n + 255) / 256)), dim3(256), 0, stream, colors, out, (long long)n);
diff --git a/opencl_path_tracer_amd/csrc/pt_launch.cpp b/opencl_path_tracer_amd/csrc/pt_launch.cpp
--- a/opencl_path_tracer_amd/csrc/pt_launch.cpp
+++ b/opencl_path_tracer_amd/csrc/pt_launch.cpp
@@ -82,12 +82,14 @@
 int alloc_stack_overflow(pt_context* ctx) {
     if (ctx->d_stack_ovf) { PT_HIP(ctx, hipFree(ctx->d_stack_ovf)); ctx->d_stack_ovf = nullptr; }
     ctx->stack_ovf_lanes = 0;
+    ctx->stack_ovf_words = 0;
     const int extra = ctx->nodes4.empty() ? 0 : wide_stack_entries(ctx->wide_pending) - ctx->wide_lds_entries;
     if (extra <= 0) return PT_OK;
     const size_t n_tiles = (size_t)((ctx->W + 7) / 8) * (size_t)((ctx->local_rows + 7) / 8);
     const size_t lanes = 256 * std::max<size_t>((size_t)ctx->cu_count * 12 * kWfDefaultChains, (n_tiles + 3) / 4);
-    PT_HIP(ctx, hipMalloc((void**)&ctx->d_stack_ovf, lanes * (size_t)extra * sizeof(uint32_t)));
+    PT_HIP(ctx, hipMalloc((void**)&ctx->d_stack_ovf, 2 * lanes * (size_t)extra * sizeof(uint32_t)));
     ctx->stack_ovf_lanes = lanes;
+    ctx->stack_ovf_words = lanes * (size_t)extra;
     return PT_OK;
 }
 
@@ -153,6 +155,10 @@
     p->chunk_spp = 0;
     p->n_taper = 0;
     p->tile_done = nullptr;
+    p->done_base = 0;
+    p->wait_pass0 = 0;
+    p->dry_word = nullptr;
+    p->dry_value = 0;
     p->n_tiles = ((ctx->W + 7) / 8) * ((ctx->local_rows + 7) / 8);
     p->suspend_lanes = ctx->suspend_lanes >= 0 ? ctx->suspend_lanes : (p->node_mode == kNodesLds ? 16 : 24);
     p->node_min_lanes = ctx->node_min_lanes >= 0 ? ctx->node_min_lanes : (p->node_mode == kNodesLds ? 3 : 6);
@@ -179,12 +185,12 @@
         ctx->events.push_back(e);
     }
     *ep = &ctx->events[ctx->events_used++];
-    PT_HIP(ctx, hipEventRecord((*ep)->a, ctx->stream));
+    PT_HIP(ctx, hipEventRecord((*ep)->a, ctx->time_stream ? ctx->time_stream : (hipStream_t)ctx->stream));
     return PT_OK;
 }
 int time_end(pt_context* ctx, EventPair* ep) {
     ctx->kernel_launches++;
-    if (ep) PT_HIP(ctx, hipEventRecord(ep->b, ctx->stream));
+    if (ep) PT_HIP(ctx, hipEventRecord(ep->b, ctx->time_stream ? ctx->time_stream : (hipStream_t)ctx->stream));
     return PT_OK;
 }
 int time_collect(pt_context* ctx) {
@@ -208,11 +214,12 @@
     }
     if (!ctx->launched_since_check || !ctx->d_tile_counter) return PT_OK;
     ctx->launched_since_check = false;
-    uint32_t words[kTileCounterWords] = {};
-    PT_HIP(ctx, hipMemcpy(words, ctx->d_tile_counter, sizeof words, hipMemcpyDeviceToHost));
+    uint32_t both[kTileCounters * kTileCounterWords] = {};
+    PT_HIP(ctx, hipMemcpy(both, ctx->d_tile_counter, sizeof both, hipMemcpyDeviceToHost));
+    const uint32_t* words = both[kTileCounterError] != 0 ? both : both + kTileCounterWords;
     if (words[kTileCounterError] != 0) {
         ctx->counters_suspect = true;
-        PT_HIP(ctx, hipMemset(ctx->d_tile_counter, 0, sizeof words));
+        PT_HIP(ctx, hipMemset(ctx->d_tile_counter, 0, sizeof both));
         ctx->counters_suspect = false;
         char msg[256];
         std::snprintf(msg, sizeof msg, "k_render: pass %u of tile %u waited more than %d ms for the tile's previous pass to be handed over (the "
@@ -223,13 +230,73 @@
     return PT_OK;
 }
 
+int setup_overlap(pt_context* ctx) {
+    auto drop = [&]() {
+        for (int k = 0; k < 2; ++k) {
+            if (ctx->ov_stream[k]) (void)hipStreamDestroy(ctx->ov_stream[k]);
+            if (ctx->ov_done[k]) (void)hipEventDestroy(ctx->ov_done[k]);
+            ctx->ov_stream[k] = nullptr;
+            ctx->ov_done[k] = nullptr;
+        }
+        if (ctx->ov_entry) (void)hipEventDestroy(ctx->ov_entry);
+        if (ctx->ov_signal) (void)hipFree(ctx->ov_signal);
+        ctx->ov_entry = nullptr;
+        ctx->ov_signal = nullptr;
+        ctx->overlap_ok = false;
+        (void)hipGetLastError();
+        return PT_OK;
+    };
+    static std::atomic<int> verdict[kMaxDevicesPerProcess];
+    const int dev = ctx->device;
+    if (dev < 0 || dev >= kMaxDevicesPerProcess || verdict[dev].load() == 2) return PT_OK;
+    int can = 0;
+    if (hipDeviceGetAttribute(&can, hipDeviceAttributeCanUseStreamWaitValue, dev) != hipSuccess || !can) return drop();
+    void* word = nullptr;
+    if (hipExtMallocWithFlags(&word, 8, hipMallocSignalMemory) != hipSuccess || !word) return drop();
+    ctx->ov_signal = (uint32_t*)word;
+    for (int k = 0; k < 2; ++k) {
+        if (hipStreamCreateWithFlags(&ctx->ov_stream[k], hipStreamNonBlocking) != hipSuccess) return drop();
+        if (hipEventCreateWithFlags(&ctx->ov_done[k], hipEventDisableTiming) != hipSuccess) return drop();
+    }
+    if (hipEventCreateWithFlags(&ctx->ov_entry, hipEventDisableTiming) != hipSuccess) return drop();
+    if (hipStreamWriteValue32(ctx->ov_stream[0], word, 0, 0) != hipSuccess || hipStreamSynchronize(ctx->ov_stream[0]) != hipSuccess) return drop();
+    if (verdict[dev].load() == 0) {
+        if (launch_signal_probe(ctx->ov_signal, 1u, ctx->ov_stream[0]) != hipSuccess) return drop();
+        if (hipStreamWaitValue32(ctx->ov_stream[1], word, 1u, hipStreamWaitValueGte, 0xffffffffu) != hipSuccess) {
+            (void)hipStreamSynchronize(ctx->ov_stream[0]);
+            verdict[dev].store(2);
+            return drop();
+        }
+        bool seen = hipEventRecord(ctx->ov_done[1], ctx->ov_stream[1]) == hipSuccess;
+        const auto t0 = std::chrono::steady_clock::now();
+        while (seen && hipEventQuery(ctx->ov_done[1]) != hipSuccess) {
+            if (std::chrono::steady_clock::now() - t0 > std::chrono::seconds(2)) seen = false;
+            else std::this_thread::sleep_for(std::chrono::microseconds(50));
+        }
+        if (!seen) {
+            (void)hipGetLastError();
+            (void)hipStreamWriteValue32(ctx->ov_stream[0], word, 1u, 0);
+            (void)hipStreamSynchronize(ctx->ov_stream[0]);
+            (void)hipStreamSynchronize(ctx->ov_stream[1]);
+            verdict[dev].store(2);
+            return drop();
+        }
+        (void)hipGetLastError();
+        if (hipStreamWriteValue32(ctx->ov_stream[0], word, 0, 0) != hipSuccess || hipStreamSynchronize(ctx->ov_stream[0]) != hipSuccess) return drop();
+        verdict[dev].store(1);
+    }
+    ctx->overlap_ok = true;
+    return PT_OK;
+}
+
 }
 
 extern "C" {
 
 static int prepare_work_counter(pt_context* ctx) {
     if (ctx->counters_suspect) {
-        PT_HIP(ctx, hipMemsetAsync(ctx->d_tile_counter, 0, sizeof(uint32_t) * kTileCounterWords, ctx->stream));
+        PT_HIP(ctx, hipStreamSynchronize(ctx->stream));
+        PT_HIP(ctx, hipMemset(ctx->d_tile_counter, 0, sizeof(uint32_t) * kTileCounterWords * kTileCounters));
         ctx->counters_suspect = false;
     }
     ctx->launched_since_check = true;
@@ -403,13 +470,16 @@
     const size_t frame_tiles = (size_t)local_tiles(ctx);
     LaunchConfig lc;
     launch_cfg(ctx, p, &lc);
+    const bool eligible = ctx->overlap_ok && ctx->overlap_launches != 0 && ctx->persistent && !tile_list && !ctx->adaptive_frame && !lc.count_work &&
+                          ctx->debug_stall_tile < 0 && p.n_tiles > 0;
+    int n_pass = 1;
     if (ctx->persistent) {
         if (int rc2 = prepare_work_counter(ctx)) return rc2;
         p.tile_counter = ctx->d_tile_counter;
         const int resident_waves = ptamd_resident_waves(ctx, lc);
         const int auto_chunk = auto_chunk_spp(p.n_tiles, resident_waves, nsamples, lc.schedule, p.node_mode);
         const int chunk = ctx->chunk_spp >= 0 ? ctx->chunk_spp : auto_chunk;
-        int n_pass = chunk > 0 ? (int)(((int64_t)nsamples + chunk - 1) / chunk) : 1;
+        n_pass = chunk > 0 ? (int)(((int64_t)nsamples + chunk - 1) / chunk) : 1;
         const int taper = ctx->chunk_taper >= 0 ? ctx->chunk_taper : auto_chunk_taper(nsamples, lc.schedule, p.node_mode);
         if (chunk > 0 && nsamples > chunk && taper > 0 && taper < chunk && nsamples < 65536) {
             std::vector<int> ends;
@@ -429,11 +499,23 @@
         const int64_t items = chunk > 0 ? (int64_t)n_pass * p.n_tiles : p.n_tiles;
         if (items + (int64_t)resident_waves + 64 >= ((int64_t)1 << 31))
             return fail(ctx, PT_EINVAL, "nsamples / chunk_spp x tiles does not fit the 31-bit work-item counter of one launch: render in several calls");
-        if (chunk > 0 && nsamples > chunk && p.n_tiles > 0) {
-            if (!ctx->d_tile_done) PT_HIP(ctx, hipMalloc((void**)&ctx->d_tile_done, sizeof(uint32_t) * frame_tiles));
-            PT_HIP(ctx, hipMemsetAsync(ctx->d_tile_done, 0, sizeof(uint32_t) * (size_t)p.n_tiles, ctx->stream));
+        const bool chained = chunk > 0 && nsamples > chunk && p.n_tiles > 0;
+        if (!chained) n_pass = 1;
+        if (chained || eligible) {
+            if (ctx->done_epoch + (uint64_t)n_pass >= (1ull << 31) || ctx->ov_serial >= (1u << 30)) {
+                PT_HIP(ctx, hipStreamSynchronize(ctx->stream));
+                PT_HIP(ctx, hipMemset(ctx->d_tile_done, 0, sizeof(uint32_t) * frame_tiles));
+                ctx->done_epoch = 0;
+                if (ctx->ov_signal) {
+                    PT_HIP(ctx, hipStreamWriteValue32(ctx->stream, ctx->ov_signal, 0, 0));
+                    PT_HIP(ctx, hipStreamSynchronize(ctx->stream));
+                    ctx->ov_serial = 0;
+                }
+            }
             p.tile_done = ctx->d_tile_done;
-            p.chunk_spp = chunk;
+            p.done_base = ctx->done_epoch;
+            ctx->done_epoch += (uint32_t)n_pass;
+            if (chained) p.chunk_spp = chunk;
         }
     }
     if (lc.count_work && p.n_tiles > 0) {
@@ -441,13 +523,54 @@
         PT_HIP(ctx, hipMemsetAsync(ctx->d_tile_cost, 0, sizeof(uint32_t) * frame_tiles, ctx->stream));
         p.tile_cost = ctx->d_tile_cost;
     }
+    hipStream_t run_on = nullptr;
+    if (eligible) {
+        const int par = ctx->ov_parity;
+        run_on = ctx->ov_stream[par];
+        OverlapKey key;
+        key.block = lc.block; key.schedule = lc.schedule; key.waves_per_simd = lc.waves_per_simd; key.persistent_blocks = lc.persistent_blocks;
+        key.n_tiles = p.n_tiles; key.lds_bytes = lc.lds_bytes; key.colors = ctx->d_colors; key.rnds = ctx->d_rnds;
+        if (!ctx->ov_chain || ctx->stream.touched) {
+            PT_HIP(ctx, hipEventRecord(ctx->ov_entry, ctx->stream.quiet()));
+            PT_HIP(ctx, hipStreamWaitEvent(run_on, ctx->ov_entry, 0));
+        } else if (!(key == ctx->ov_key)) {
+            PT_HIP(ctx, hipStreamWaitEvent(run_on, ctx->ov_done[par ^ 1], 0));
+        } else {
+            PT_HIP(ctx, hipStreamWaitValue32(run_on, ctx->ov_signal, ctx->ov_serial, hipStreamWaitValueGte, 0xffffffffu));
+            p.wait_pass0 = 1;
+            ctx->overlapped_launches++;
+        }
+        p.tile_counter = ctx->d_tile_counter + (size_t)par * kTileCounterWords;
+        if (p.stack_ovf) p.stack_ovf += (size_t)par * ctx->stack_ovf_words;
+        p.dry_word = ctx->ov_signal;
+        p.dry_value = ++ctx->ov_serial;
+        ctx->ov_key = key;
+        ctx->ov_parity = par ^ 1;
+    }
     EventPair* ep;
-    if ((rc = time_begin(ctx, &ep)) != PT_OK) return rc;
-    {
-        const hipError_t le = launch_render_mega(p, lc, ctx->stream);
-        if (le != hipSuccess) { ctx->counters_suspect = true; return fail(ctx, PT_EHIP, std::string("launch_render_mega: ") + hipGetErrorString(le)); }
-    }
-    if ((rc = time_end(ctx, ep)) != PT_OK) { ctx->counters_suspect = true; return rc; }
+    ctx->time_stream = run_on;
+    rc = time_begin(ctx, &ep);
+    if (rc == PT_OK) {
+        const hipError_t le = launch_render_mega(p, lc, run_on ? run_on : (hipStream_t)ctx->stream);
+        if (le != hipSuccess) rc = fail(ctx, PT_EHIP, std::string("launch_render_mega: ") + hipGetErrorString(le));
+    }
+    if (rc == PT_OK) rc = time_end(ctx, ep);
+    ctx->time_stream = nullptr;
+    if (rc == PT_OK && run_on) {
+        const hipError_t e1 = hipEventRecord(ctx->ov_done[ctx->ov_parity ^ 1], run_on);
+        const hipError_t e2 = e1 == hipSuccess ? hipStreamWaitEvent(ctx->stream.quiet(), ctx->ov_done[ctx->ov_parity ^ 1], 0) : e1;
+        if (e2 != hipSuccess) rc = fail(ctx, PT_EHIP, std::string("launch_megakernel: completion event: ") + hipGetErrorString(e2));
+    }
+    if (rc != PT_OK) {
+        ctx->counters_suspect = true;
+        ctx->stream.touched = true;
+        if (run_on) (void)hipStreamSynchronize(run_on);
+        return rc;
+    }
+    if (run_on) {
+        ctx->ov_chain = true;
+        ctx->stream.touched = false;
+    }
     return PT_OK;
 }
 
@@ -581,6 +704,7 @@
 int pt_set_current_sample(pt_context* ctx, int32_t s) {
     if (!ctx || s < 0) return PT_EINVAL;
     ctx->current_sample = s;
+    ctx->stream.touched = true;
     if (s == 0) ctx->adaptive_frame = false;
     return PT_OK;
 }
```

Result: slower. 2634 (-5.5%).
